# cuevhv/PMT_learning_for_semantic_segmentation_and_disparity

Measured on AMD Instinct MI355X. Metric: stereo-pairs/sec (train fwd+bwd) 512x256, higher is better.
Workload: dtype bf16; 1 GPU; minidsnetExt (densenet121, 1dcorr, aspp 0; the live PyTorch form of baseline_SDnet*) train step fwd+loss(CE+CE+Lovasz+L1)+bwd+Adam, 512x256 (WxH), batch 8 per GPU, hipGraph; global_batch=8, parallelism=dp1, world_size=1

## Files before the change

pmt_learning_for_semantic_segmentation_and_disparity_amd/_lib.py:

```python
import ctypes
import os
import re

import torch

_HERE = os.path.dirname(os.path.abspath(__file__))
LIB_PATH = os.path.join(_HERE, "libsdhip.so")
HEADER_PATH = os.path.join(_HERE, "..", "include", "sdhip.h")

NREP = int(os.environ.get("SDHIP_TUNE_NREP", "32"))


class SdhipError(RuntimeError):
    pass


_ARG_TYPES = {"*": ctypes.c_void_p, "int": ctypes.c_int, "long": ctypes.c_long, "int64_t": ctypes.c_long, "float": ctypes.c_float, "double": ctypes.c_double}
_RET_TYPES = {"int": ctypes.c_int, "long": ctypes.c_long, "void": None, "const char*": ctypes.c_char_p}


def parse_header(text):
    text = re.sub(r"/\*.*?\*/", " ", text, flags=re.S)
    consts = {n: int(v) for n, v in re.findall(r"^[ \t]*#define[ \t]+(SDHIP_\w+)[ \t]+\(?(-?\d+)\)?[ \t]*$", text, flags=re.M)}
    sigs = {}
    for ret, name, params in re.findall(r"^([\w \t*]+?)\s*\b(sdhip_\w+)\s*\(([^()]*)\)\s*;", text, flags=re.M):
        ret = re.sub(r"\s*\*\s*", "*", " ".join(ret.split()))
        if ret not in _RET_TYPES:
            raise SdhipError("sdhip.h: %s has return type '%s', which the binding cannot classify" % (name, ret))
        args = []
        for par in ([] if params.strip() == "void" else params.split(",")):
            ctype = "*" if "*" in par else " ".join(w for w in par.split()[:-1] if w != "const")
            if ctype not in _ARG_TYPES:
                raise SdhipError("sdhip.h: %s has parameter '%s', which the binding cannot classify" % (name, " ".join(par.split())))
            args.append(_ARG_TYPES[ctype])
        sigs[name] = (_RET_TYPES[ret], args)
    return sigs, consts


if not os.path.exists(LIB_PATH):
    raise ImportError(
        "libsdhip.so not found at %s — run `python -c 'import __graft_entry__ as g; g.build()'` "
        "(hipcc, gfx950). This package has no fallback path." % LIB_PATH)
if not os.path.exists(HEADER_PATH):
    raise ImportError(
        "sdhip.h not found at %s — the binding reads every signature and constant of libsdhip.so from it. "
        "This package has no fallback path." % HEADER_PATH)

_lib = ctypes.CDLL(LIB_PATH, mode=ctypes.RTLD_GLOBAL)

with open(HEADER_PATH) as _f:
    _SIGS, CONSTANTS = parse_header(_f.read())
SIGNATURES = {_name: _args for _name, (_ret, _args) in _SIGS.items()}
for _name, (_ret, _args) in _SIGS.items():
    _fn = getattr(_lib, _name)
    _fn.argtypes = _args
    _fn.restype = _ret

F32, BF16 = CONSTANTS["SDHIP_F32"], CONSTANTS["SDHIP_BF16"]
ERR_ARG, ERR_LAUNCH, ERR_UNSUPPORTED = CONSTANTS["SDHIP_ERR_ARG"], CONSTANTS["SDHIP_ERR_LAUNCH"], CONSTANTS["SDHIP_ERR_UNSUPPORTED"]
ACT_HSWISH, ACT_HSIGMOID = CONSTANTS["SDHIP_ACT_HSWISH"], CONSTANTS["SDHIP_ACT_HSIGMOID"]
SEG_TVERSKY, SEG_DICE, SEG_DICE_ENTROPY = CONSTANTS["SDHIP_SEG_TVERSKY"], CONSTANTS["SDHIP_SEG_DICE"], CONSTANTS["SDHIP_SEG_DICE_ENTROPY"]


class WgradItem(ctypes.Structure):
    _fields_ = [(n, ctypes.c_void_p) for n in ("x", "dy", "dw_packed", "dbias", "in_scale", "in_shift")] + \
               [(n, ctypes.c_int) for n in ("B", "H", "W", "Cin", "ldx", "Ho", "Wo", "Cout", "lddy", "kh", "kw", "stride", "dil", "pad_t",
                                            "pad_l", "D", "Do", "kd", "sd", "pad_d", "in_relu", "groups")]


class PyrMap(ctypes.Structure):
    _fields_ = [("p", ctypes.c_void_p)] + [(n, ctypes.c_int) for n in ("h", "w", "ld", "reserved")]


def pyr_maps(entries):
    t = (PyrMap * len(entries))()
    for e, (m, h, w, ld) in zip(t, entries):
        e.p, e.h, e.w, e.ld = m.data_ptr(), h, w, ld
    return ctypes.cast(t, ctypes.c_void_p), t


def lovasz_workspace_bytes(npix, C):
    return _lib.sdhip_lovasz_workspace_bytes(npix, C)


def seg_terms_workspace_bytes(B, hw, C):
    n = _lib.sdhip_seg_terms_workspace_bytes(B, hw, C)
    if n <= 0:
        raise SdhipError("sdhip_seg_terms_workspace_bytes: unsupported shape (B %d, %d pixels, C %d; C <= 32)" % (B, hw, C))
    return n


def disp_smooth_workspace_bytes(B, H, W):
    n = _lib.sdhip_disp_smooth_workspace_bytes(B, H, W)
    if n <= 0:
        raise SdhipError("sdhip_disp_smooth_workspace_bytes: unsupported shape (B %d, H %d, W %d)" % (B, H, W))
    return n


def edge_bce_workspace_bytes(n):
    nbytes = _lib.sdhip_edge_bce_workspace_bytes(n)
    if nbytes <= 0:
        raise SdhipError("sdhip_edge_bce_workspace_bytes: unsupported element count %d" % n)
    return nbytes


def photo_mse_workspace_bytes(npix):
    nbytes = _lib.sdhip_photo_mse_workspace_bytes(npix)
    if nbytes <= 0:
        raise SdhipError("sdhip_photo_mse_workspace_bytes: unsupported pixel count %d" % npix)
    return nbytes


def dw_pool_parts(H, W, C, k, stride, dt):
    n = _lib.sdhip_dw_pool_parts(H, W, C, k, stride, dt)
    if n <= 0:
        raise SdhipError("sdhip_dw_pool_parts: unsupported depthwise shape")
    return n


def dw_wgrad_parts(B, H, W, C, k, stride):
    n = _lib.sdhip_dw_wgrad_parts(B, H, W, C, k, stride)
    if n <= 0:
        raise SdhipError("sdhip_dw_wgrad_parts: unsupported depthwise shape")
    return n


def packed_elems(M, K, T, dt):
    return _lib.sdhip_conv_packed_elems(M, K, T, dt)


def graph_node_counts(graph):
    c = (ctypes.c_int * 4)()
    n = _lib.sdhip_graph_node_counts(ctypes.c_void_p(graph.raw_cuda_graph()), c)
    if n < 0:
        raise SdhipError("sdhip_graph_node_counts failed: %s" % _lib.sdhip_last_error().decode())
    return {"kernel": c[0], "memset": c[1], "memcpy": c[2], "other": c[3], "total": n}


def abort_capture(stream):
    rc = _lib.sdhip_abort_capture(ctypes.c_void_p(stream.cuda_stream))
    if rc < 0:
        raise SdhipError("sdhip_abort_capture failed: %s" % _lib.sdhip_last_error().decode())
    return rc


def reload_diag():
    _lib.sdhip_diag_reload()


def _diag_switch(name):
    v = os.environ.get(name)
    if v:
        import sys
        sys.stderr.write("[sdhip] diagnostic switch %s=%s is set: this is not the production path\n" % (name, v))
    return v


DIAG_NO_FUSED_BN = bool(_diag_switch("SDHIP_DIAG_NO_FUSED_BN"))
DIAG_NO_SIDE = bool(_diag_switch("SDHIP_DIAG_NO_SIDE"))
DIAG_NO_GRAD_SLOTS = bool(_diag_switch("SDHIP_DIAG_NO_GRAD_SLOTS"))
DIAG_NO_WGRAD_GROUP = bool(_diag_switch("SDHIP_DIAG_NO_WGRAD_GROUP"))
DIAG_NO_PHASE_DGRAD = bool(_diag_switch("SDHIP_DIAG_NO_PHASE_DGRAD"))
TUNE_WGRAD_OVERLAP = bool(_diag_switch("SDHIP_TUNE_WGRAD_OVERLAP"))
TUNE_OVERLAP_WG = int(_diag_switch("SDHIP_TUNE_OVERLAP_WG") or 128)
DIAG_NO_BN_SLOTS = bool(_diag_switch("SDHIP_DIAG_NO_BN_SLOTS"))
TUNE_FUSE1_MAX_PIX = int(_diag_switch("SDHIP_TUNE_FUSE1_MAX_PIX") or 32768)
TUNE_PRO_MAX_PIX = int(_diag_switch("SDHIP_TUNE_PRO_MAX_PIX") or 32768)
TUNE_BN_SLOT_MAX_MB = int(_diag_switch("SDHIP_TUNE_BN_SLOT_MAX_MB") or 40)
DIAG_NO_BNPRO = bool(_diag_switch("SDHIP_DIAG_NO_BNPRO"))
DIAG_NO_BNBWD_EPILOGUE = bool(_diag_switch("SDHIP_DIAG_NO_BNBWD_EPILOGUE"))
DIAG_STEM_S2D = _diag_switch("SDHIP_STEM_S2D")
DIAG_NO_PYRAMID_FUSE = bool(_diag_switch("SDHIP_DIAG_NO_PYRAMID_FUSE"))


def abi_version():
    return _lib.sdhip_abi_version()


def call(name, *args, unsupported_ok=False):
    if name not in SIGNATURES:
        raise SdhipError("%s is not declared in include/sdhip.h" % name)
    rc = getattr(_lib, name)(*args)
    if rc != 0 and not (unsupported_ok and rc == ERR_UNSUPPORTED):
        raise SdhipError("%s failed (%d): %s" % (name, rc, _lib.sdhip_last_error().decode()))
    return rc == 0


def try_call(name, *args):
    return call(name, *args, unsupported_ok=True)


def dtype_code(t):
    if t.dtype == torch.float32:
        return F32
    if t.dtype == torch.bfloat16:
        return BF16
    raise SdhipError("unsupported dtype %s (f32 and bf16 only)" % t.dtype)


def code_of(dtype):
    return BF16 if dtype == torch.bfloat16 else F32


def stream_ptr():
    return ctypes.c_void_p(torch.cuda.current_stream().cuda_stream)


def ptr(t):
    return ctypes.c_void_p(t.data_ptr()) if t is not None else ctypes.c_void_p(0)
```

pmt_learning_for_semantic_segmentation_and_disparity_amd/csrc/conv_band.h:

```cpp
#pragma once
#include <type_traits>
#include "conv_fast.h"

namespace {

struct BandArgs {
  const void* x; const void* wp; void* y;
  const float* bias; double* stats;
  int B, H, W, Ho, Wo, pad_t, pad_l;
  int Cin, ldx, Cout, Mpad, ldy;
  int bpg, act, stats_ld, nrep;
  const void* res; int ldres;
  long rep_stride;
  int tiles_w, tiles_hw, ntiles, tpw;
  unsigned magic_hw, magic_tw;
  int D, Do, pad_d;
  unsigned magic_do;
  int dbg;
};

template <int I, int N, typename F> __device__ __forceinline__ void band_static_for(F&& f) {
  if constexpr (I < N) { f(std::integral_constant<int, I>{}); band_static_for<I + 1, N>(f); }
}
template <int N> __device__ __forceinline__ void band_wait() { asm volatile("s_waitcnt vmcnt(%0) lgkmcnt(0)" ::"n"(N) : "memory"); }

template <int K, int BN, int NW = 8, int KD = 1>
struct BandCfg {
  static constexpr int RPR = NW * 16;
  static constexpr int RPW = 16 / NW;
  static constexpr int TH = 16, TW = 32;
  static constexpr int IH = TH + K - 1, IW = TW + K - 1, IWp = (IW + 7) & ~7;
  static constexpr int HROWS = IH * IWp;
  static constexpr int HR = (HROWS + RPR - 1) / RPR;
  static constexpr int HB = HROWS * 64;
  static constexpr int RS = K == 3 ? 3 : 1;
  static constexpr int NSTG = K / RS;
  static constexpr bool WRES = NSTG == 1 && KD == 1;
  static constexpr int TPS = RS * K;
  static constexpr int WROWS = TPS * BN;
  static constexpr int WR = (WROWS + RPR - 1) / RPR;
  static constexpr int WB = WROWS * 64;
  static constexpr int NWB = WRES ? 1 : 2;
  static constexpr int WRS = WRES ? 0 : WR;
  static constexpr int HPS = NSTG == 1 ? HR : (HR + NSTG - 2) / (NSTG - 1);
  static constexpr int RED = NW * 2 * BN * 4;
  static constexpr int SPT = (WRS + HPS + TPS - 1) / TPS;
  static constexpr size_t LDS = 2 * HB + NWB * WB + RED;
  static_assert(HROWS % 16 == 0 && WROWS % 16 == 0, "a wave's 16 rows of a DMA round are either all inside or all outside the image");
  static_assert(NSTG == 1 || HPS * (NSTG - 1) >= HR, "halo rounds must fit the stages of one chunk");
  static_assert(LDS <= 160 * 1024, "LDS budget");
};

typedef __attribute__((ext_vector_type(4))) int band_rsrc_t;
constexpr int kBandOob = 0x7fffff00;
#pragma clang diagnostic push
#pragma clang diagnostic ignored "-Winline-asm"
__device__ __forceinline__ void band_dma(int voff, band_rsrc_t rsrc, unsigned lds_wave_base, int soff) {
  asm volatile("s_mov_b32 m0, %2\n\ts_nop 0\n\tbuffer_load_dwordx4 %0, %1, %3 offen lds"
               : : "v"(voff), "s"(rsrc), "s"(lds_wave_base), "s"(soff) : "memory", "m0");
}
#pragma clang diagnostic pop
__device__ __forceinline__ band_rsrc_t band_rsrc(const void* base) {
  const unsigned long long a = (unsigned long long)base;
  band_rsrc_t r;
  r[0] = __builtin_amdgcn_readfirstlane((int)(a & 0xffffffffu));
  r[1] = __builtin_amdgcn_readfirstlane((int)((a >> 32) & 0xffffu));
  r[2] = kBandOob;
  r[3] = 0x00020000;
  return r;
}

template <int K, int BN, int VAR, int NW, int KD = 1>
__global__ __launch_bounds__(NW * 64) void conv_band_kernel(const BandArgs p) {
  constexpr bool DBG = (VAR & 128) != 0;
  const int dbg = DBG ? p.dbg : 0;
  using C = BandCfg<K, BN, NW, KD>;
  using T = bf16_t;
  constexpr int IWp = C::IWp, IW = C::IW, HB = C::HB, WB = C::WB, RPR = C::RPR, RPW = C::RPW;
  constexpr int NT_CO = BN / 16, NT_PIX = 2 * RPW;
  constexpr int NSTORE = NT_CO * NT_PIX / 2;
  extern __shared__ __attribute__((aligned(16))) unsigned char smem[];

  const int tid = threadIdx.x, lane = tid & 63;
  const int wave = __builtin_amdgcn_readfirstlane(tid >> 6);
  const int l15 = lane & 15, lg = lane >> 4;

  const int t_begin = blockIdx.x * p.tpw;
  const int t_end = min(p.ntiles, t_begin + p.tpw);
  if (t_begin >= t_end) return;
  const int nhalf = KD > 1 ? KD : (p.Cin > 32 ? 2 : 1);
  const int nchunks = (t_end - t_begin) * nhalf;

  const int rsub = tid >> 2;
  const int c_l = (tid & 3) ^ ((rsub >> 1) & 2);
  const unsigned wave_lds = __builtin_amdgcn_readfirstlane(lds_addr(smem) + wave * 1024);
  const band_rsrc_t xr = band_rsrc(p.x), wr = band_rsrc(p.wp);
  const int img_bytes = p.H * p.W * p.ldx * 2;

  int czt = 0;
  auto tile_of = [&](int t, int& b, int& oh0, int& ow0) {
    if constexpr (KD > 1) { const int q = fast_div(t, p.Do, p.magic_do); czt = t - q * p.Do; t = q; }
    b = fast_div(t, p.tiles_hw, p.magic_hw);
    const int r = t - b * p.tiles_hw;
    const int ty = fast_div(r, p.tiles_w, p.magic_tw);
    oh0 = ty * C::TH;
    ow0 = (r - ty * p.tiles_w) * C::TW;
  };
  int hv[C::HR];
  auto halo_offsets = [&](int oh0, int ow0) {
    const int ih0 = oh0 - p.pad_t, iw0 = ow0 - p.pad_l;
#pragma unroll
    for (int r = 0; r < C::HR; ++r) {
      const int row = r * RPR + rsub;
      const int ih = row / IWp, iw = row - ih * IWp;
      const int gh = ih0 + ih, gw = iw0 + iw;
      const bool in = iw < IW && (unsigned)gh < (unsigned)p.H && (unsigned)gw < (unsigned)p.W && c_l * 8 < p.Cin;
      hv[r] = in ? ((gh * p.W + gw) * p.ldx + c_l * 8) * 2 : kBandOob;
    }
  };
  auto halo_dma = [&](int r, int soff, int hsel) {
    if (r < C::HR && r * RPR + wave * 16 < C::HROWS) band_dma(soff >= 0 ? hv[r] : kBandOob, xr, hsel * HB + r * (RPR * 64) + wave_lds, soff >= 0 ? soff : 0);
  };
  auto chunk_src = [&](int b, int zt, int h) -> int {
    if constexpr (KD > 1) {
      const int zin = zt + h - p.pad_d;
      return (zin >= 0 && zin < p.D) ? (b * p.D + zin) * img_bytes : -1;
    } else {
      return b * img_bytes + h * 64;
    }
  };
  int wv[C::WR];
#pragma unroll
  for (int r = 0; r < C::WR; ++r) {
    const int row = r * RPR + rsub;
    const int tap = row / BN, m = min(row % BN, p.Mpad - 1);
    wv[r] = (tap * p.Mpad + m) * 128 + c_l * 16;
  }
  const int wrow_bytes = C::TPS * p.Mpad * 128;
  auto w_dma = [&](int r, int j, int h, int wsel) {
    if (r < C::WR && r * RPR + wave * 16 < C::WROWS)
      band_dma(wv[r], wr, 2 * HB + wsel * WB + r * (RPR * 64) + wave_lds, j * wrow_bytes + (KD > 1 ? h * wrow_bytes : h * 64));
  };

  int b_k[K];
#pragma unroll
  for (int kw = 0; kw < K; ++kw) b_k[kw] = LdsRow<1>::off(kw + l15, lg);
  const int a_base = LdsRow<1>::off(l15, lg);
  const int wave_row = wave * (RPW * IWp * 64);

  float bv[NT_CO][4];
#pragma unroll
  for (int mi = 0; mi < NT_CO; ++mi)
#pragma unroll
    for (int r = 0; r < 4; ++r) {
      const int co = mi * 16 + 4 * lg + r;
      bv[mi][r] = (p.bias && co < p.Cout) ? p.bias[co] : 0.f;
    }

  f32x4 acc[NT_CO][NT_PIX];
  float s1[NT_CO][4], s2[NT_CO][4];
#pragma unroll
  for (int mi = 0; mi < NT_CO; ++mi)
#pragma unroll
    for (int r = 0; r < 4; ++r) { s1[mi][r] = 0.f; s2[mi][r] = 0.f; }

  float* const red = reinterpret_cast<float*>(smem + 2 * HB + C::NWB * WB);
  auto flush_stats = [&](int grp) {
#pragma unroll
    for (int mi = 0; mi < NT_CO; ++mi) {
#pragma unroll
      for (int r = 0; r < 4; ++r) {
        const float a = row16_sum(s1[mi][r]), c2 = row16_sum(s2[mi][r]);
        if (l15 == 0) {
          const int m = mi * 16 + 4 * lg + r;
          red[(wave * 2 + 0) * BN + m] = a;
          red[(wave * 2 + 1) * BN + m] = c2;
        }
        s1[mi][r] = 0.f; s2[mi][r] = 0.f;
      }
    }
    asm volatile("s_waitcnt lgkmcnt(0)" ::: "memory");
    __builtin_amdgcn_s_barrier();
    if (tid < 2 * BN) {
      const int which = tid / BN, m = tid - which * BN;
      if (m < p.Cout) {
        float tot = 0.f;
#pragma unroll
        for (int w = 0; w < NW; ++w) tot += red[(w * 2 + which) * BN + m];
        atomicAdd(p.stats + (long)(blockIdx.x % p.nrep) * p.rep_stride + ((long)grp * 2 + which) * p.stats_ld + m, (double)tot);
      }
    }
  };

  if constexpr ((VAR & 2) != 0) { if (wave >= 4) __builtin_amdgcn_s_setprio(1); }
  int cb, coh0, cow0, ch_half = 0, ct = t_begin;
  tile_of(ct, cb, coh0, cow0);
  halo_offsets(coh0, cow0);
#pragma unroll
  for (int r = 0; r < C::WR; ++r) w_dma(r, 0, 0, 0);
#pragma unroll
  for (int r = 0; r < C::HR; ++r) halo_dma(r, chunk_src(cb, czt, 0), 0);
  int cz = czt;
  int wsel = 0;
  bool epi_counted = false;

  constexpr bool WREG = C::WRES && BN <= 32;
  u32x4 wreg[WREG ? C::TPS : 1][NT_CO];

  for (int c = 0; c < nchunks; ++c) {
    const int hsel = c & 1;
    const bool has_next = c + 1 < nchunks;
    int nb = cb, noh0 = coh0, now0 = cow0, nh = ch_half + 1, nt = ct, nz = cz;
    if (nh == nhalf) {
      nh = 0; nt = ct + 1;
      if (has_next) { tile_of(nt, nb, noh0, now0); halo_offsets(noh0, now0); nz = czt; }
    }
    const int nsoff = chunk_src(nb, nz, nh);
    if (ch_half == 0) {
#pragma unroll
      for (int mi = 0; mi < NT_CO; ++mi)
#pragma unroll
        for (int ni = 0; ni < NT_PIX; ++ni) acc[mi][ni] = f32x4{0.f, 0.f, 0.f, 0.f};
    }
    const unsigned char* const hb = smem + hsel * HB + wave_row;

    band_static_for<0, C::NSTG>([&](auto jc) {
      constexpr int j = decltype(jc)::value;
      constexpr int r_lo = (j - 1) * C::HPS, r_hi = j * C::HPS < C::HR ? j * C::HPS : C::HR;
      constexpr bool counted = j >= 1 && r_hi > r_lo && r_hi * RPR <= C::HROWS;
      if (j == 0 && epi_counted) band_wait<NSTORE>();
      else if (counted && has_next) band_wait<counted ? r_hi - r_lo : 0>();
      else band_wait<0>();
      if (!(dbg & 16)) __builtin_amdgcn_s_barrier();

      const unsigned char* const wl = smem + 2 * HB + wsel * WB + a_base;
      const unsigned char* const hj = hb + j * C::RS * (IWp * 64);
      if constexpr (WREG) {
        if (c == 0) {
#pragma unroll
          for (int t = 0; t < C::TPS; ++t)
#pragma unroll
            for (int mi = 0; mi < NT_CO; ++mi) wreg[t][mi] = *reinterpret_cast<const u32x4*>(wl + t * (BN * 64) + mi * 1024);
        }
      }
      u32x4 af[2][NT_CO], bf[2][NT_PIX];
      if constexpr (DBG) if (dbg & 32) {
#pragma unroll
        for (int i = 0; i < 2; ++i)
#pragma unroll
          for (int q = 0; q < 4; ++q) { if (q < NT_CO) af[i][q] = u32x4{0x3f803f80u, (unsigned)tid, 0x3f803f80u, 0x3f803f80u}; bf[i][q] = u32x4{0x3f803f80u, 0x3f803f80u, (unsigned)lane, 0x3f803f80u}; }
      }
      auto load = [&](int set, int t) {
        if (dbg & 32) return;
#pragma unroll
        for (int mi = 0; mi < NT_CO; ++mi) {
          if constexpr (WREG) af[set][mi] = wreg[t][mi];
          else af[set][mi] = *reinterpret_cast<const u32x4*>(wl + t * (BN * 64) + mi * 1024);
        }
#pragma unroll
        for (int ni = 0; ni < NT_PIX; ++ni)
          bf[set][ni] = *reinterpret_cast<const u32x4*>(hj + b_k[t % K] + ((t / K + (ni >> 1)) * IWp + (ni & 1) * 16) * 64);
      };
      auto dma_slot = [&](int sl) {
        if (sl < C::WRS) {
          if (dbg & 2) return;
          if (j + 1 < C::NSTG) w_dma(sl, j + 1, ch_half, wsel ^ 1);
          else if (has_next) w_dma(sl, 0, nh, wsel ^ 1);
        } else if (sl < C::WRS + C::HPS) {
          if (dbg & 1) return;
          if (has_next && (C::NSTG == 1 || j < C::NSTG - 1)) halo_dma(j * C::HPS + sl - C::WRS, nsoff, hsel ^ 1);
        }
      };
      load(0, 0);
#pragma unroll
      for (int kw = 0; kw < C::TPS; ++kw) {
        if constexpr ((VAR & 1) != 0) {
#pragma unroll
          for (int sl = kw * C::SPT; sl < (kw + 1) * C::SPT; ++sl) dma_slot(sl);
        }
        if (kw + 1 < C::TPS) load((kw + 1) & 1, kw + 1);
        if constexpr ((VAR & 1) == 0) {
#pragma unroll
          for (int sl = kw * C::SPT; sl < (kw + 1) * C::SPT; ++sl) dma_slot(sl);
        }
        if (!(dbg & 4)) {
#pragma unroll
          for (int mi = 0; mi < NT_CO; ++mi)
#pragma unroll
            for (int ni = 0; ni < NT_PIX; ++ni) Mma<T>::run(acc[mi][ni], af[kw & 1][mi], bf[kw & 1][ni]);
        }
        if constexpr ((VAR & 4) != 0) {
#pragma unroll
          for (int g = 0; g < NT_CO + NT_PIX; ++g) {
            __builtin_amdgcn_sched_group_barrier(0x100, 1, 0);
            __builtin_amdgcn_sched_group_barrier(0x008, (NT_CO * NT_PIX) / (NT_CO + NT_PIX), 0);
          }
        }
      }
      if constexpr (!C::WRES) wsel ^= 1;
    });

    epi_counted = false;
    if (ch_half == nhalf - 1) {
      const int oimg = KD > 1 ? cb * p.Do + cz : cb;
      const int grp = oimg < p.bpg ? 0 : oimg / p.bpg;
      if (p.bias) {
#pragma unroll
        for (int mi = 0; mi < NT_CO; ++mi)
#pragma unroll
          for (int ni = 0; ni < NT_PIX; ++ni)
#pragma unroll
            for (int r = 0; r < 4; ++r) acc[mi][ni][r] += bv[mi][r];
      }
      if (p.act == 1) {
#pragma unroll
        for (int mi = 0; mi < NT_CO; ++mi)
#pragma unroll
          for (int ni = 0; ni < NT_PIX; ++ni)
#pragma unroll
            for (int r = 0; r < 4; ++r) acc[mi][ni][r] = fmaxf(acc[mi][ni][r], 0.f);
      } else if (p.act == 2) {
#pragma unroll
        for (int mi = 0; mi < NT_CO; ++mi)
#pragma unroll
          for (int ni = 0; ni < NT_PIX; ++ni)
#pragma unroll
            for (int r = 0; r < 4; ++r) acc[mi][ni][r] = 1.f / (1.f + __expf(-acc[mi][ni][r]));
      }
      T* const yb = (T*)p.y + (long)oimg * p.Ho * p.Wo * p.ldy;
      const T* const rb = (const T*)p.res + (long)oimg * p.Ho * p.Wo * p.ldres;
      const bool interior = coh0 + C::TH <= p.Ho && cow0 + C::TW <= p.Wo && BN <= p.Cout;
      if (interior) {
        const long pix0 = (long)(coh0 + RPW * wave) * p.Wo + cow0 + (lg & 1) * 16 + l15;
        T* const d0 = yb + pix0 * p.ldy + 8 * (lg >> 1);
        const T* const r0 = rb + pix0 * p.ldres + 8 * (lg >> 1);
#pragma unroll
        for (int q = 0; q < NT_PIX / 2; ++q) {
          T* dst = d0 + (long)q * p.Wo * p.ldy;
          const T* rsrc = r0 + (long)q * p.Wo * p.ldres;
          u32x4 ov[NT_CO];
#pragma unroll
          for (int mi = 0; mi < NT_CO; ++mi) {
            const f32x4 v0 = acc[mi][2 * q], v1 = acc[mi][2 * q + 1];
            const u32x2 o0 = u32x2{pack2bf(v0[0], v0[1]), pack2bf(v0[2], v0[3])};
            const u32x2 o1 = u32x2{pack2bf(v1[0], v1[1]), pack2bf(v1[2], v1[3])};
            if (p.stats) {
              const f32x4 w0 = f32x4{bflo(o0[0]), bfhi(o0[0]), bflo(o0[1]), bfhi(o0[1])};
              const f32x4 w1 = f32x4{bflo(o1[0]), bfhi(o1[0]), bflo(o1[1]), bfhi(o1[1])};
#pragma unroll
              for (int r = 0; r < 4; ++r) {
                s1[mi][r] += w0[r] + w1[r];
                s2[mi][r] = fmaf(w1[r], w1[r], fmaf(w0[r], w0[r], s2[mi][r]));
              }
            }
            u32x4 o;
            if (p.res) {
              float f[8];
#pragma unroll
              for (int r = 0; r < 4; ++r) {
                const float a0 = v0[r], a1 = v1[r];
                const u32x2 e = __builtin_amdgcn_permlane16_swap(__float_as_uint(a0), __float_as_uint(a1), false, false);
                const unsigned e0 = e[0], e1 = e[1];
                f[r] = __uint_as_float(e0); f[4 + r] = __uint_as_float(e1);
              }
              const u32x4 old = *reinterpret_cast<const u32x4*>(rsrc + mi * 16);
#pragma unroll
              for (int e = 0; e < 4; ++e) o[e] = pack2bf(f[2 * e] + bflo(old[e]), f[2 * e + 1] + bfhi(old[e]));
            } else {
              const u32x2 e0 = __builtin_amdgcn_permlane16_swap(o0[0], o1[0], false, false);
              const u32x2 e1 = __builtin_amdgcn_permlane16_swap(o0[1], o1[1], false, false);
              o = u32x4{e0[0], e1[0], e0[1], e1[1]};
            }
            ov[mi] = o;
          }
          if (!(dbg & 8)) {
#pragma unroll
            for (int mi = 0; mi < NT_CO; ++mi) *reinterpret_cast<u32x4*>(dst + mi * 16) = ov[mi];
          }
        }
        epi_counted = !(dbg & 8) && !p.res;
      } else {
#pragma unroll
        for (int ni = 0; ni < NT_PIX; ++ni) {
          const int oh = coh0 + RPW * wave + (ni >> 1), ow = cow0 + (ni & 1) * 16 + l15;
          const bool valid = oh < p.Ho && ow < p.Wo;
          T* dst = yb + ((long)oh * p.Wo + ow) * p.ldy;
          const T* rsrc = rb + ((long)oh * p.Wo + ow) * p.ldres;
#pragma unroll
          for (int mi = 0; mi < NT_CO; ++mi) {
            const int co = mi * 16 + 4 * lg;
            float v[4];
#pragma unroll
            for (int r = 0; r < 4; ++r) v[r] = acc[mi][ni][r];
            if (valid && co + 3 < p.Cout) {
              if (p.res) {
                const u32x2 old = *reinterpret_cast<const u32x2*>(rsrc + co);
                v[0] += bflo(old[0]); v[1] += bfhi(old[0]); v[2] += bflo(old[1]); v[3] += bfhi(old[1]);
              }
              const u32x2 o = u32x2{pack2bf(v[0], v[1]), pack2bf(v[2], v[3])};
              *reinterpret_cast<u32x2*>(dst + co) = o;
              v[0] = bflo(o[0]); v[1] = bfhi(o[0]); v[2] = bflo(o[1]); v[3] = bfhi(o[1]);
            } else if (valid && co < p.Cout) {
#pragma unroll
              for (int r = 0; r < 4; ++r) {
                if (co + r < p.Cout) {
                  if (p.res) v[r] += Elem<T>::ld(rsrc + co + r);
                  Elem<T>::st(dst + co + r, v[r]); v[r] = Elem<T>::rnd(v[r]);
                }
                else v[r] = 0.f;
              }
            } else {
#pragma unroll
              for (int r = 0; r < 4; ++r) v[r] = 0.f;
            }
            if (p.stats) {
#pragma unroll
              for (int r = 0; r < 4; ++r) { s1[mi][r] += v[r]; s2[mi][r] = fmaf(v[r], v[r], s2[mi][r]); }
            }
          }
        }
      }
      if (p.stats) {
        const int nimg = KD > 1 ? nb * p.Do + nz : nb;
        const int ngrp = nimg < p.bpg ? 0 : nimg / p.bpg;
        if (!has_next || ngrp != grp) { flush_stats(grp); epi_counted = false; }
      }
    }
    cb = nb; coh0 = noh0; cow0 = now0; ch_half = nh; ct = nt; cz = nz;
  }
}

inline bool band_ok(int ntiles) { return ntiles >= 192 && ntiles < 65536; }

template <int K, int BN, int VAR, int NW = 8, int KD = 1>
int launch_band_bn(const BandArgs& a, int grid, hipStream_t s) {
  auto kern = conv_band_kernel<K, BN, VAR, NW, KD>;
  static bool attr_set = false;
  if (!attr_set) {
    if (hipFuncSetAttribute((const void*)kern, hipFuncAttributeMaxDynamicSharedMemorySize, 160 * 1024) != hipSuccess)
      SDHIP_FAIL(SDHIP_ERR_LAUNCH, "conv_band: cannot raise dynamic LDS limit");
    attr_set = true;
  }
  const size_t lds = BandCfg<K, BN, NW, KD>::LDS;
  hipLaunchKernelGGL(kern, dim3(grid), dim3(NW * 64), lds, s, a);
  SDHIP_LAUNCH_CHECK();
  return SDHIP_OK;
}

template <int K, int KD = 1>
int launch_band(BandArgs& a, hipStream_t s) {
  const int tiles_h = sdhip_cdiv(a.Ho, 16);
  a.tiles_w = sdhip_cdiv(a.Wo, 32);
  a.tiles_hw = tiles_h * a.tiles_w;
  a.ntiles = a.tiles_hw * a.B * (KD > 1 ? a.Do : 1);
  a.magic_do = (KD > 1 && a.Do > 1) ? (unsigned)(0x100000000ULL / (unsigned)a.Do) + 1u : 0u;
  a.magic_hw = a.tiles_hw > 1 ? (unsigned)(0x100000000ULL / (unsigned)a.tiles_hw) + 1u : 0u;
  a.magic_tw = a.tiles_w > 1 ? (unsigned)(0x100000000ULL / (unsigned)a.tiles_w) + 1u : 0u;
  a.tpw = sdhip_cdiv(a.ntiles, 256);
  a.dbg = sdhip_diag().tune_band_dbg;
  const int grid = sdhip_cdiv(a.ntiles, a.tpw);
  a.dbg &= 0xff;
  if constexpr (K == 5) {
    if (a.Mpad > 32) return a.dbg ? launch_band_bn<K, 64, 128 + 5>(a, grid, s) : launch_band_bn<K, 64, 5>(a, grid, s);
  } else if constexpr (KD > 1) {
    return launch_band_bn<K, 32, 5, 8, KD>(a, grid, s);
  } else {
    if (a.Mpad > 32) return launch_band_bn<K, 64, 5>(a, grid, s);
  }
  return launch_band_bn<K, 32, 5>(a, grid, s);
}

}
```

pmt_learning_for_semantic_segmentation_and_disparity_amd/csrc/conv_fwd.hip:

```cpp
#include "conv_common.h"
#include "conv_fast.h"
#include "conv_point.h"
#include "conv_grow.h"
#include "conv_mid.h"
#include "conv_band.h"
#include "conv_gemm.h"
#include "conv_thin.h"

namespace {

struct FwdArgs {
  const void* x; const void* wp; void* y;
  const float* bias; const float* in_scale; const float* in_shift; double* stats;
  ConvGeom g;
  int Cin, ldx, Cout, Mpad, ldy;
  int in_relu, groups, act, accumulate;
  int tg, vec_in, vec_out, stats_ld, nrep, pf_halo, sh, per_tap;
  long rep_stride;
};

template <typename T, int TH, int TW, int BN>
__global__ __launch_bounds__(256) void conv_fwd_kernel(const FwdArgs p) {
  constexpr int V = Chunk<T>::N;
  constexpr int CK = 8 * V;
// ... 209 lines not shown
      w_issue(q, t);
      w_commit(q, t, wl0);
      __syncthreads();
      compute(q, t, halo0, wl0);
    }
  } else {
  if (pf_halo) halo_issue(0); else halo_sync_stage(0, halo0);
  w_issue(0, 0);
  for (int st = 0; st < S; ++st) {
    const int q = st / ntg, t0 = (st - q * ntg) * p.tg;
    unsigned char* halo = halo0 + ((pf_halo && (q & 1)) ? halo_bytes : 0);
    unsigned char* wl = wl0 + (st & 1) * wbuf_bytes;
    if (pf_halo && t0 == 0) halo_commit(q, halo);
    w_commit(q, t0, wl);
    __syncthreads();
    const int sn = st + 1;
    int qn = 0, t0n = 0;
    if (sn < S) {
      qn = sn / ntg; t0n = (sn - qn * ntg) * p.tg;
      if (pf_halo && t0n == 0) halo_issue(qn);
      w_issue(qn, t0n);
    }
    compute(q, t0, halo, wl);
    if (!pf_halo && sn < S && t0n == 0) {
      __syncthreads();
      halo_sync_stage(qn, halo0);
    }
  }
  }

  float s1[NT_CO][4], s2[NT_CO][4];
#pragma unroll
  for (int mi = 0; mi < NT_CO; ++mi)
#pragma unroll
    for (int r = 0; r < 4; ++r) { s1[mi][r] = 0.f; s2[mi][r] = 0.f; }

  T* yb = (T*)p.y + (long)blockIdx.z * g.Ho * g.Wo * p.ldy;
#pragma unroll
  for (int ni = 0; ni < NT_PIX; ++ni) {
    const int pt = wave * NT_PIX + ni;
    const int oh = oh0 + pt / TWT, ow = ow0 + (pt % TWT) * 16 + l15;
    const bool valid = oh < g.Ho && ow < g.Wo;
    T* dst = yb + ((long)oh * g.Wo + ow) * p.ldy;
#pragma unroll
    for (int mi = 0; mi < NT_CO; ++mi) {
      if (mi * 16 >= mvalid) continue;
      const int co = n0 + mi * 16 + 4 * lg;
      float v[4];
#pragma unroll
      for (int r = 0; r < 4; ++r) {
        float x = acc[mi][ni][r];
        if (p.bias && co + r < p.Cout) x += p.bias[co + r];
        if (p.act == 1) x = fmaxf(x, 0.f);
        else if (p.act == 2) x = 1.f / (1.f + __expf(-x));
        v[r] = x;
      }
      if (!valid) continue;
      if (p.vec_out && co + 3 < p.Cout) {
        if constexpr (sizeof(T) == 4) {
          f32x4* d4 = reinterpret_cast<f32x4*>(dst + co);
          f32x4 o = f32x4{v[0], v[1], v[2], v[3]};
          if (p.accumulate) o += *d4;
          *d4 = o;
#pragma unroll
          for (int r = 0; r < 4; ++r) v[r] = o[r];
        } else {
          u32x2* d2 = reinterpret_cast<u32x2*>(dst + co);
          if (p.accumulate) {
            const u32x2 old = *d2;
            v[0] += bflo(old[0]); v[1] += bfhi(old[0]); v[2] += bflo(old[1]); v[3] += bfhi(old[1]);
          }
          const u32x2 o = u32x2{pack2bf(v[0], v[1]), pack2bf(v[2], v[3])};
          *d2 = o;
          v[0] = bflo(o[0]); v[1] = bfhi(o[0]); v[2] = bflo(o[1]); v[3] = bfhi(o[1]);
        }
      } else {
#pragma unroll
        for (int r = 0; r < 4; ++r) {
          if (co + r < p.Cout) {
            if (p.accumulate) v[r] += Elem<T>::ld(dst + co + r);
            Elem<T>::st(dst + co + r, v[r]);
            v[r] = Elem<T>::rnd(v[r]);
          } else {
            v[r] = 0.f;
          }
        }
      }
#pragma unroll
      for (int r = 0; r < 4; ++r) { s1[mi][r] += v[r]; s2[mi][r] = fmaf(v[r], v[r], s2[mi][r]); }
    }
  }

  if (p.stats) {
    __syncthreads();
    float* red = reinterpret_cast<float*>(smem);
#pragma unroll
    for (int mi = 0; mi < NT_CO; ++mi) {
#pragma unroll
      for (int r = 0; r < 4; ++r) {
        float a = s1[mi][r], c2 = s2[mi][r];
#pragma unroll
        for (int o = 8; o > 0; o >>= 1) { a += __shfl_xor(a, o, 64); c2 += __shfl_xor(c2, o, 64); }
        if (l15 == 0) {
          const int m = mi * 16 + 4 * lg + r;
          red[(wave * 2 + 0) * BN + m] = a;
          red[(wave * 2 + 1) * BN + m] = c2;
        }
      }
    }
    __syncthreads();
    if (tid < 2 * BN) {
      const int which = tid / BN, m = tid - which * BN;
      if (n0 + m < p.Cout) {
        const float tot = red[(0 * 2 + which) * BN + m] + red[(1 * 2 + which) * BN + m] +
                          red[(2 * 2 + which) * BN + m] + red[(3 * 2 + which) * BN + m];
        atomicAdd(p.stats + (long)((blockIdx.x + blockIdx.z) % p.nrep) * p.rep_stride + ((long)grp * 2 + which) * p.stats_ld + n0 + m, (double)tot);
      }
    }
  }
}

template <typename T, int TH, int TW, int BN>
int launch(const FwdArgs& a, size_t lds, hipStream_t s) {
  auto kern = conv_fwd_kernel<T, TH, TW, BN>;
  static size_t attr_set = 0;
  if (lds > 64 * 1024 && lds > attr_set) {
    if (hipFuncSetAttribute((const void*)kern, hipFuncAttributeMaxDynamicSharedMemorySize, 160 * 1024) != hipSuccess)
      SDHIP_FAIL(SDHIP_ERR_LAUNCH, "conv_fwd: cannot raise dynamic LDS limit");
    attr_set = 160 * 1024;
  }
  const ConvGeom& g = a.g;
  dim3 grid(sdhip_cdiv(g.Ho, TH) * sdhip_cdiv(g.Wo, TW), sdhip_cdiv(a.Mpad, BN), g.B * g.Do);
  hipLaunchKernelGGL(kern, grid, dim3(256), lds, s, a);
  SDHIP_LAUNCH_CHECK();
  return SDHIP_OK;
}

template <typename T, int TH, int TW>
int launch_bn(const FwdArgs& a, int bn, size_t lds, hipStream_t s) {
  switch (bn) {
    case 16: return launch<T, TH, TW, 16>(a, lds, s);
    case 32: return launch<T, TH, TW, 32>(a, lds, s);
    case 64: return launch<T, TH, TW, 64>(a, lds, s);
    default: return launch<T, TH, TW, 128>(a, lds, s);
  }
}

size_t halo_bytes_of(const ConvGeom& g, int th, int tw, int per_tap) {
  const int eh = per_tap ? 0 : (g.kh - 1) * g.dil, ew = per_tap ? 0 : (g.kw - 1) * g.dil;
  const int IH = (th - 1) * g.stride + eh + 1, IW = (tw - 1) * g.stride + ew + 1;
  return ((size_t)IH * IW * 128 + 15) & ~(size_t)15;
}


struct ProStats {
  const double* stats; int ld, nrep;
  const float* gamma; const float* beta;
  float* scale; float* shift; float* mean; float* invstd; float* rmean; float* rvar;
  float eps, momentum; double count;
  const double* pend; double* fold; int pend_ld, pend_nrep, pend_c0, pend_n;
};

struct ConvCall {
  const void* x = nullptr; const void* wp = nullptr; void* y = nullptr;
  const float* bias = nullptr; const float* in_scale = nullptr; const float* in_shift = nullptr;
  double* stats = nullptr; int stats_ld = 0, stats_nrep = 1;
  ConvGeom g{};
  int Cin = 0, ldx = 0, Cout = 0, ldy = 0;
  int in_relu = 0, groups = 1, act = 0, accumulate = 0;
  int dtype = SDHIP_F32;
  hipStream_t stream = nullptr;
  int omul = 1, ooz = 0, ooy = 0, oox = 0;
  const void* bx = nullptr; int ldbx = 0;
  const float* bsc = nullptr; const float* bsh = nullptr; int bx_mode = 0;
  const void* addend = nullptr; int ldadd = 0;
  const ProStats* ps = nullptr;
  bool plain() const { return !ps && !bx && !addend && omul == 1; }
  bool flat() const { return g.kd == 1 && g.D == 1 && g.Do == 1; }
};

ConvGeom geom2d(int B, int H, int W, int Ho, int Wo, int kh, int kw, int stride, int dil, int pad_t, int pad_l) {
  return ConvGeom{B, H, W, Ho, Wo, kh, kw, stride, dil, pad_t, pad_l, 1, 1, 1, 1, 0};
}

ConvCall conv_call(const void* x, const void* wpacked, void* y, const ConvGeom& g, int Cin, int ldx, int Cout, int ldy, int dtype, void* stream) {
  ConvCall c;
  c.x = x; c.wp = wpacked; c.y = y; c.g = g;
  c.Cin = Cin; c.ldx = ldx; c.Cout = Cout; c.ldy = ldy;
  c.dtype = dtype; c.stream = (hipStream_t)stream;
  return c;
}

struct ConvPlan {
  int V, es, Mpad;
  int stats_ld, nrep; long rep_stride;
  int vec_in, vec_out;
  int T, bn; bool big;
  int rows, chunks_per_row, per_tap_any;
};

constexpr size_t kLdsMax = 160 * 1024, kLdsSoft = 80 * 1024;

ConvPlan conv_plan(const ConvCall& c) {
  const ConvGeom& g = c.g;
  const SdhipDiag& dg = sdhip_diag();
  ConvPlan d;
  d.V = c.dtype == SDHIP_BF16 ? 8 : 4;
  d.es = conv_esize(c.dtype);
  d.Mpad = (c.Cout + 15) & ~15;
  d.stats_ld = c.stats_ld > 0 ? c.stats_ld : c.Cout;
  d.nrep = c.stats_nrep > 0 ? c.stats_nrep : 1;
  d.rep_stride = (long)c.groups * 2 * d.stats_ld;
  d.vec_in = (c.ldx % d.V == 0) && (((uintptr_t)c.x & 15) == 0);
  d.vec_out = (c.ldy % 4 == 0) && (((uintptr_t)c.y % (4 * d.es)) == 0);
  int bn = 16;
  for (int cand = 128; cand >= 32; cand >>= 1)
    if ((long)sdhip_cdiv(d.Mpad, cand) * cand * 4 <= (long)d.Mpad * 5) { bn = cand; break; }
  if ((long)g.kh * g.kw * g.kd * c.Cin <= 128 && d.Mpad <= 128) bn = d.Mpad > 64 ? 128 : (d.Mpad > 32 ? 64 : (d.Mpad > 16 ? 32 : 16));
  d.T = g.kh * g.kw;
  const long blocks_big = (long)sdhip_cdiv(g.Ho, 8) * sdhip_cdiv(g.Wo, 32) * g.B * g.Do * sdhip_cdiv(d.Mpad, bn);
  d.big = (blocks_big >= dg.tune_big && g.Wo >= 24) || dg.conv_big;
  if (g.stride == 2 && g.kd > 1 && !dg.conv_big && dg.tune_s2_small) d.big = false;
  if (!d.big) {
    const long px_blocks = (long)sdhip_cdiv(g.Ho, 4) * sdhip_cdiv(g.Wo, 16) * g.B * g.Do;
    while (bn > 32 && px_blocks * sdhip_cdiv(d.Mpad, bn) < dg.tune_split) bn >>= 1;
  }
  d.bn = bn;
  d.rows = d.Mpad < bn ? d.Mpad : bn;
  d.chunks_per_row = c.Cin <= 8 * d.V / 2 ? 4 : 8;
  d.per_tap_any = (g.kh > 1 || g.kw > 1) && g.dil >= 4 && g.kd == 1;
  return d;
}


int path_thin(const ConvCall& c, const ConvPlan& d) {
  const ConvGeom& g = c.g;
  if (!(c.plain() && c.Cout == 1 && c.Cin <= d.V && d.vec_in && g.stride == 1 && c.flat() && !c.in_scale && !c.accumulate &&
        d.T <= kThinMaxT && g.Ho == g.H + 2 * g.pad_t - g.dil * (g.kh - 1) && g.Wo == g.W + 2 * g.pad_l - g.dil * (g.kw - 1) &&
        g.pad_t >= 0 && g.pad_l >= 0 && !sdhip_diag().conv_no_thin))
    return kNotTaken;
  ThinArgs t{};
  t.x = c.x; t.wp = c.wp; t.y = c.y; t.bias = c.bias; t.stats = c.stats;
  set_extent(t, g);
  t.kh = g.kh; t.kw = g.kw; t.dil = g.dil;
  t.Cin = c.Cin; t.ldx = c.ldx; t.ldy = c.ldy; t.Mpad = d.Mpad; t.act = c.act; t.bpg = g.B / c.groups;
  t.stats_ld = d.stats_ld; t.nrep = d.nrep; t.rep_stride = d.rep_stride;
  dim3 grid(sdhip_cdiv(g.Wo, 256), g.Ho, g.B);
  if (c.dtype == SDHIP_BF16) hipLaunchKernelGGL(conv_thin_fwd_kernel<bf16_t>, grid, dim3(256), 0, c.stream, t);
  else hipLaunchKernelGGL(conv_thin_fwd_kernel<float>, grid, dim3(256), 0, c.stream, t);
  SDHIP_LAUNCH_CHECK_AS("conv2d_fwd_impl");
  return SDHIP_OK;
}

int path_fanin(const ConvCall& c, const ConvPlan& d) {
  const ConvGeom& g = c.g;
  if (!(c.plain() && c.dtype == SDHIP_BF16 && fanin_ok(c.Cin, c.Cout, g.kh, g.kw, g.stride, g.dil, g.kd, g.sd, c.ldx, c.x) && !c.in_scale &&
        !c.accumulate && !c.stats && (long)g.H * g.W * c.ldx < (1L << 31) && !sdhip_diag().conv_no_thin))
    return kNotTaken;
  FaninArgs t{};
  t.x = c.x; t.wp = c.wp; t.y = c.y; t.bias = c.bias;
  set_extent(t, g);
  t.kh = g.kh; t.kw = g.kw;
  t.D = g.D; t.Do = g.Do; t.pad_d = g.pad_d;
  t.Cin = c.Cin; t.ldx = c.ldx; t.ldy = c.ldy; t.Mpad = d.Mpad; t.act = c.act;
  t.dpw = 1; t.zsegs = g.Do; t.npxp = 0; t.pitch = 0;
  return launch_fanin(t, g.kd, c.stream);
}

int path_fanout(const ConvCall& c, const ConvPlan& d) {
  const ConvGeom& g = c.g;
  if (!(c.plain() && c.dtype == SDHIP_BF16 && fanout_ok(c.Cin, c.Cout, d.T, g.stride, g.kd, g.sd, c.ldy, c.y) && !c.in_scale &&
        !c.accumulate && !c.stats && !c.bias && c.act == 0 && (g.kh - 1) * g.dil <= 31 && (g.kw - 1) * g.dil <= 31 &&
        (long)sdhip_cdiv(g.Ho, 8) * sdhip_cdiv(g.Wo, 32) < (1L << 31) && g.B <= 65535 && !sdhip_diag().conv_no_thin))
    return kNotTaken;
  FanArgs t{};
  t.x = c.x; t.wp = c.wp; t.y = c.y;
  set_extent(t, g);
  t.kh = g.kh; t.kw = g.kw; t.dil = g.dil;
  t.ldx = c.ldx; t.Cout = c.Cout; t.Mpad = d.Mpad; t.ldy = c.ldy;
  t.D = g.D; t.Do = g.Do; t.kd = g.kd; t.pad_d = g.pad_d; t.dpw = 1; t.zsegs = g.Do;
  return launch_fanout(t, c.stream);
}

int path_gemm(const ConvCall& c, const ConvPlan& d) {
  const ConvGeom& g = c.g;
  const SdhipDiag& dg = sdhip_diag();
  if (!(c.plain() && c.dtype == SDHIP_BF16 && g.kh == 1 && g.kw == 1 && c.flat() && g.stride == 1 && g.pad_t == 0 && g.pad_l == 0 &&
        g.Ho == g.H && g.Wo == g.W && !c.accumulate && !dg.conv_generic && !dg.conv_no_gemm))
    return kNotTaken;
  GemmArgs a{};
  a.seg[0] = GemmSeg{c.x, c.ldx, c.Cin, 0};
  a.seg[1] = GemmSeg{nullptr, 0, 0, 0};
  a.nseg = 1;
  a.wp = c.wp; a.y = c.y; a.bias = c.bias; a.in_scale = c.in_scale; a.in_shift = c.in_shift; a.stats = c.stats;
  a.ldy = c.ldy; a.Cout = c.Cout; a.Mpad = d.Mpad; a.K = c.Cin; a.in_relu = c.in_relu; a.act = c.act;
  a.M = (long)g.B * g.H * g.W; a.H = g.H; a.W = g.W; a.ppg = a.M / c.groups;
  a.stats_ld = d.stats_ld; a.nrep = d.nrep; a.rep_stride = d.rep_stride;
  if (!gemm1x1_ok(a, (c.in_scale || c.stats) ? c.groups : 1)) return kNotTaken;
  return launch_gemm_any(a, c.stream);
}

bool band_common_ok(const ConvCall& c) {
  const ConvGeom& g = c.g;
  return !c.ps && !c.bx && c.omul == 1 && c.dtype == SDHIP_BF16 && g.stride == 1 && g.dil == 1 && !c.in_scale &&
         !((c.accumulate || c.addend) && c.stats) && !(c.accumulate && c.addend) &&
         (!c.addend || (c.ldadd % 8 == 0 && ((uintptr_t)c.addend & 15) == 0)) && c.Cin % 8 == 0 &&
         c.ldx % 8 == 0 && ((uintptr_t)c.x & 15) == 0 && c.ldy % 8 == 0 && ((uintptr_t)c.y & 15) == 0 &&
         (long)g.B * g.D * g.H * g.W * c.ldx * 2 < (long)kBandOob && band_ok(sdhip_cdiv(g.Ho, 16) * sdhip_cdiv(g.Wo, 32) * g.B * g.Do) &&
         !sdhip_diag().conv_generic && !sdhip_diag().conv_no_band;
}

BandArgs band_args(const ConvCall& c, const ConvPlan& d) {
  const ConvGeom& g = c.g;
  BandArgs f{};
  f.x = c.x; f.wp = c.wp; f.y = c.y; f.bias = c.bias; f.stats = c.stats;
  set_extent(f, g);
  f.D = g.D; f.Do = g.Do; f.pad_d = g.pad_d;
  f.Cin = c.Cin; f.ldx = c.ldx; f.Cout = c.Cout; f.Mpad = d.Mpad; f.ldy = c.ldy;
  f.bpg = (g.B / c.groups) * g.Do; f.act = c.act; f.stats_ld = d.stats_ld; f.nrep = d.nrep; f.rep_stride = d.rep_stride;
  f.res = c.addend ? c.addend : (c.accumulate ? c.y : nullptr); f.ldres = c.addend ? c.ldadd : c.ldy;
  return f;
}

int path_band2d(const ConvCall& c, const ConvPlan& d) {
  const ConvGeom& g = c.g;
  const bool band5 = g.kh == 5 && g.kw == 5 && (c.Cin <= 32 || c.Cin == 64);
  const bool band3 = g.kh == 3 && g.kw == 3 && c.Cin <= 32 && !sdhip_diag().conv_no_band3;
  if (!((band5 || band3) && c.flat() && d.Mpad <= 64 && d.Mpad >= 32 && band_common_ok(c))) return kNotTaken;
  BandArgs f = band_args(c, d);
  f.pad_d = 0;
  return band5 ? launch_band<5>(f, c.stream) : launch_band<3>(f, c.stream);
}

int path_band3d(const ConvCall& c, const ConvPlan& d) {
  const ConvGeom& g = c.g;
  if (!(g.kh == 3 && g.kw == 3 && g.kd == 3 && g.sd == 1 && c.Cin <= 32 && d.Mpad == 32 && band_common_ok(c) && !sdhip_diag().conv_no_band3))
    return kNotTaken;
  BandArgs f = band_args(c, d);
  return launch_band<3, 3>(f, c.stream);
}

int path_point(const ConvCall& c, const ConvPlan& d) {
  const ConvGeom& g = c.g;
  const SdhipDiag& dg = sdhip_diag();
  if (!(c.dtype == SDHIP_BF16 && !c.bx && !c.addend && c.omul == 1 && (c.ps || (c.in_scale && c.stats)) && !c.bias && c.act == 0 && !c.accumulate &&
        g.kh == 1 && g.kw == 1 && c.flat() && g.stride == 1 && g.pad_t == 0 && g.pad_l == 0 && g.Ho == g.H && g.Wo == g.W &&
        c.Cin >= 128 && c.Cin <= kPinMaxC && c.Cin % 8 == 0 && c.Cout % kPointBN == 0 && c.Cout <= 256 && (long)g.B * g.H * g.W <= 32768 && (long)g.H * g.W <= kPointMaxMap &&
        (long)g.B * sdhip_cdiv((long)g.H * g.W, kPointPix) * (c.Cout / kPointBN) <= kPointMaxWG &&
        d.vec_in && d.vec_out && (long)g.H * g.W * c.ldx < (1L << 31) && !dg.conv_generic && !dg.conv_no_point))
    return kNotTaken;
  const ProStats* ps = c.ps;
  PointArgs f{};
  f.x = c.x; f.wp = c.wp; f.y = c.y; f.in_scale = c.in_scale; f.in_shift = c.in_shift; f.stats = c.stats;
  f.HW = g.H * g.W; f.Cin = c.Cin; f.ldx = c.ldx; f.Cout = c.Cout; f.Mpad = d.Mpad; f.ldy = c.ldy;
  f.in_relu = c.in_relu; f.bpg = g.B / c.groups;
  f.stats_ld = d.stats_ld; f.nrep = d.nrep; f.rep_stride = d.rep_stride;
  if (ps) {
    f.pin_stats = ps->stats; f.pin_ld = ps->ld; f.pin_nrep = ps->nrep; f.pin_groups = c.groups; f.pin_gamma = ps->gamma; f.pin_beta = ps->beta;
    f.pin_scale = ps->scale; f.pin_shift = ps->shift; f.pin_mean = ps->mean; f.pin_invstd = ps->invstd; f.pin_rmean = ps->rmean; f.pin_rvar = ps->rvar;
    f.pin_eps = ps->eps; f.pin_momentum = ps->momentum; f.pin_count = ps->count;
    f.pend_stats = ps->pend; f.pin_fold = ps->fold; f.pend_ld = ps->pend_ld; f.pend_nrep = ps->pend_nrep; f.pend_c0 = ps->pend_c0; f.pend_n = ps->pend ? ps->pend_n : 0;
  }
  return launch_point(f, g.B, c.stream);
}

int path_grow(const ConvCall& c, const ConvPlan& d) {
  const ConvGeom& g = c.g;
  const SdhipDiag& dg = sdhip_diag();
  if (!(c.dtype == SDHIP_BF16 && !c.bx && !c.addend && c.omul == 1 && (c.ps || (c.in_scale && c.stats)) && !c.bias && c.act == 0 && !c.accumulate &&
        g.kh == 3 && g.kw == 3 && c.flat() && g.stride == 1 && g.dil == 1 && g.pad_t == 1 && g.pad_l == 1 && g.Ho == g.H && g.Wo == g.W &&
        c.Cin % 32 == 0 && c.Cin >= 64 && c.Cin <= 256 && c.Cout == kGrowBN && (long)g.H * g.W <= kGrowMaxMap &&
        (long)g.B * sdhip_cdiv(g.H, kGrowTH) * sdhip_cdiv(g.W, kGrowTW) <= kGrowMaxWG &&
        d.vec_in && d.vec_out && (long)g.H * g.W * c.ldx < (1L << 31) && !dg.conv_generic && !dg.conv_no_grow))
    return kNotTaken;
  const ProStats* ps = c.ps;
  GrowArgs f{};
  f.x = c.x; f.wp = c.wp; f.y = c.y; f.in_scale = c.in_scale; f.in_shift = c.in_shift; f.stats = c.stats;
  f.H = g.H; f.W = g.W; f.Cin = c.Cin; f.ldx = c.ldx; f.ldy = c.ldy; f.tiles_w = sdhip_cdiv(g.W, kGrowTW);
  f.in_relu = c.in_relu; f.bpg = g.B / c.groups;
  f.stats_ld = d.stats_ld; f.nrep = d.nrep; f.rep_stride = d.rep_stride;
  if (ps) {
    f.pin_stats = ps->stats; f.pin_ld = ps->ld; f.pin_nrep = ps->nrep; f.pin_groups = c.groups; f.pin_gamma = ps->gamma; f.pin_beta = ps->beta;
    f.pin_scale = ps->scale; f.pin_shift = ps->shift; f.pin_mean = ps->mean; f.pin_invstd = ps->invstd; f.pin_rmean = ps->rmean; f.pin_rvar = ps->rvar;
    f.pin_eps = ps->eps; f.pin_momentum = ps->momentum; f.pin_count = ps->count;
    f.pend_stats = ps->pend; f.pin_fold = ps->fold; f.pend_ld = ps->pend_ld; f.pend_nrep = ps->pend_nrep; f.pend_c0 = ps->pend_c0; f.pend_n = ps->pend ? ps->pend_n : 0;
  }
  return launch_grow(f, g.B, c.stream);
}

int path_mid(const ConvCall& c, const ConvPlan& d) {
  const ConvGeom& g = c.g;
  const SdhipDiag& dg = sdhip_diag();
  const long min_map = dg.tune_mid_min_map > 0 ? dg.tune_mid_min_map : kMidMinMap, max_map = dg.tune_mid_max_map > 0 ? dg.tune_mid_max_map : kMidMaxMap;
  const long max_wg = dg.tune_mid_max_wg > 0 ? dg.tune_mid_max_wg : kMidMaxWG;
  if (!(c.dtype == SDHIP_BF16 && g.kh == 3 && g.kw == 3 && c.flat() && g.stride == 1 && g.dil == 1 && g.pad_t == 1 && g.pad_l == 1 &&
        g.Ho == g.H && g.Wo == g.W && c.Cin == kMidBN && c.Cout == kMidBN && !c.in_scale && !c.ps && !c.bias && c.act == 0 && !c.accumulate &&
        c.omul == 1 && (c.bx ? c.bx_mode == 0 : !c.addend) && (long)g.H * g.W >= min_map && (long)g.H * g.W <= max_map &&
        (long)g.B * sdhip_cdiv(g.H, kMidTH) * sdhip_cdiv(g.W, kMidTW) <= max_wg &&
        d.vec_in && d.vec_out && (long)g.H * g.W * c.ldx < (1L << 31) && !dg.conv_generic && !dg.conv_no_mid))
    return kNotTaken;
  MidArgs f{};
  f.x = c.x; f.wp = c.wp; f.y = c.y; f.stats = c.stats;
  f.H = g.H; f.W = g.W; f.ldx = c.ldx; f.ldy = c.ldy; f.tiles_w = sdhip_cdiv(g.W, kMidTW);
  f.bpg = g.B / c.groups;
  f.stats_ld = d.stats_ld; f.nrep = d.nrep; f.rep_stride = d.rep_stride;
  f.bx = c.bx; f.bsc = c.bsc; f.bsh = c.bsh; f.ldbx = c.ldbx;
  f.res = c.bx ? c.addend : nullptr; f.ldres = c.ldadd;
  return launch_mid(f, g.B, c.stream);
}

int path_fast(const ConvCall& c, const ConvPlan& d) {
  const ConvGeom& g = c.g;
  if (!(!d.per_tap_any && d.vec_in && d.vec_out && (long)g.H * g.W * c.ldx < (1L << 31) && !sdhip_diag().conv_generic)) return kNotTaken;
  const int tune_ksoft_small = 80, tune_ksoft_big = 80;
  const int CKh = 8 * d.V, T = d.T, bn = d.bn;
  const int ks = d.chunks_per_row == 4 ? 1 : 2;
  const int rb = 64 * ks, px_per_round = 256 / (4 * ks);
  const ProStats* ps = c.ps;
  FastArgs f{};
  f.x = c.x; f.wp = c.wp; f.y = c.y; f.bias = c.bias; f.in_scale = c.in_scale; f.in_shift = c.in_shift; f.stats = c.stats;
  set_extent(f, g);
  f.kh = g.kh; f.kw = g.kw; f.stride = g.stride; f.dil = g.dil;
  f.D = g.D; f.Do = g.Do; f.kd = g.kd; f.sd = g.sd; f.pad_d = g.pad_d;
  f.Cin = c.Cin; f.ldx = c.ldx; f.Cout = c.Cout; f.Mpad = d.Mpad; f.ldy = c.ldy;
  f.in_relu = c.in_relu; f.bpg = g.B / c.groups; f.act = c.act; f.accumulate = c.accumulate;
  f.stats_ld = d.stats_ld; f.nrep = d.nrep; f.rep_stride = d.rep_stride; f.tail = (c.Cin % d.V) != 0;
  f.omul = c.omul; f.ooz = c.ooz; f.ooy = c.ooy; f.oox = c.oox;
  f.bx = c.bx; f.ldbx = c.ldbx; f.bsc = c.bsc; f.bsh = c.bsh;
  f.res = c.bx ? c.addend : nullptr; f.ldres = c.ldadd; f.bx_mode = c.bx_mode; f.bx_groups = c.groups;
  f.dma = !c.in_scale && !f.tail && !ps;
  if (ps) {
    f.pin_stats = ps->stats; f.pin_ld = ps->ld; f.pin_nrep = ps->nrep; f.pin_groups = c.groups; f.pin_gamma = ps->gamma; f.pin_beta = ps->beta;
    f.pin_scale = ps->scale; f.pin_shift = ps->shift; f.pin_mean = ps->mean; f.pin_invstd = ps->invstd; f.pin_rmean = ps->rmean; f.pin_rvar = ps->rvar;
    f.pin_eps = ps->eps; f.pin_momentum = ps->momentum; f.pin_count = ps->count;
    f.pend_stats = ps->pend; f.pin_fold = ps->fold; f.pend_ld = ps->pend_ld; f.pend_nrep = ps->pend_nrep; f.pend_c0 = ps->pend_c0; f.pend_n = ps->pend ? ps->pend_n : 0;
  }
  bool fbig = d.big;
  for (int attempt = 0; attempt < 2; ++attempt) {
    const int th = fbig ? 8 : 4, tw = fbig ? 32 : 16;
    const int IH = (th - 1) * g.stride + (g.kh - 1) * g.dil + 1, IW = (tw - 1) * g.stride + (g.kw - 1) * g.dil + 1;
    const int IWp = (IW + 7) & ~7;
    const int hrows = ((IH * IWp + px_per_round - 1) / px_per_round) * px_per_round;
    const int nqq_f = g.kd * (ks == 2 ? sdhip_cdiv(c.Cin, CKh) : 1);
    const size_t hb = (size_t)hrows * rb * ((fbig || nqq_f == 1) ? 1 : 2);
    if (!fbig && hrows > ((f.dma && ks == 1) ? 6 : 5) * px_per_round) { fbig = true; continue; }
    auto wbuf = [&](int tgv) { return (size_t)(((tgv * bn + px_per_round - 1) / px_per_round) * px_per_round) * rb; };
    int tg = T;
    const size_t ksoft_f = (size_t)(fbig ? tune_ksoft_big : tune_ksoft_small) * 1024;
    size_t lds;
    if (nqq_f == 1 && hb + wbuf(T) <= ksoft_f) {
      lds = hb + wbuf(T);
    } else {
      while (tg > 1 && hb + 2 * wbuf(tg) > ksoft_f) --tg;
      lds = hb + 2 * wbuf(tg);
    }
    if (lds < 4096) lds = 4096;
    f.pin_off = 0; f.pin_cs = 0;
    if (ps) { f.pin_off = (int)lds; f.pin_cs = (c.Cin + 63) & ~63; lds += 2 * (size_t)f.pin_cs * sizeof(float); }
    if (lds > kLdsMax) { if (!fbig) break; fbig = false; continue; }
    f.tg = tg;
    f.magic_iwp = IWp > 1 ? (unsigned)(0x100000000ULL / (unsigned)IWp) + 1u : 0u;
    f.tiles_w = sdhip_cdiv(g.Wo, tw);
    f.magic_tw = f.tiles_w > 1 ? (unsigned)(0x100000000ULL / (unsigned)f.tiles_w) + 1u : 0u;
    f.ntg = sdhip_cdiv(T, tg);
    if ((long)f.tiles_w * sdhip_cdiv(g.Ho, th) >= 65536) break;
    return c.dtype == SDHIP_BF16 ? launch_fast_any<bf16_t>(f, fbig, ks, bn, lds, c.stream) : launch_fast_any<float>(f, fbig, ks, bn, lds, c.stream);
  }
  return kNotTaken;
}

int path_generic(const ConvCall& c, const ConvPlan& d) {
  const ConvGeom& g = c.g;
  const int bn = d.bn;
  FwdArgs a{};
  a.x = c.x; a.wp = c.wp; a.y = c.y; a.bias = c.bias; a.in_scale = c.in_scale; a.in_shift = c.in_shift; a.stats = c.stats;
  a.g = g;
  a.Cin = c.Cin; a.ldx = c.ldx; a.Cout = c.Cout; a.Mpad = d.Mpad; a.ldy = c.ldy;
  a.in_relu = c.in_relu; a.groups = c.groups; a.act = c.act; a.accumulate = c.accumulate;
  a.vec_in = d.vec_in; a.vec_out = d.vec_out;
  a.stats_ld = d.stats_ld; a.nrep = d.nrep; a.rep_stride = d.rep_stride;
  bool big = d.big;
  for (int attempt = 0; attempt < 2; ++attempt) {
    const int th = big ? 8 : 4, tw = big ? 32 : 16;
    const int per_tap = d.per_tap_any;
    const size_t halo = halo_bytes_of(g, th, tw, per_tap);
    const long halo_loads = (long)(halo / 128) * d.chunks_per_row;
    const int pf = !per_tap && !big && d.vec_in && (c.Cin % d.V == 0) && halo_loads <= 4 * 256 && 2 * halo + 2 * (size_t)bn * 128 <= kLdsSoft;
    int tg = per_tap ? 1 : 1024 / (d.rows * d.chunks_per_row);
    if (tg < 1) tg = 1;
    if (tg > d.T) tg = d.T;
    const size_t hb = halo * (pf ? 2 : 1);
    while (tg > 1 && hb + 2 * (size_t)tg * bn * 128 > kLdsSoft) --tg;
    size_t lds = hb + 2 * (size_t)tg * bn * 128;
    if (lds < 4096) lds = 4096;
    if (lds > kLdsMax) {
      if (big) { big = false; continue; }
      SDHIP_FAIL(SDHIP_ERR_UNSUPPORTED, "conv2d_fwd: halo tile of a %dx%d kernel with dilation %d does not fit LDS", g.kh, g.kw, g.dil);
    }
    a.tg = tg; a.pf_halo = pf; a.sh = d.chunks_per_row == 4 ? 2 : 3; a.per_tap = per_tap;
    if (c.dtype == SDHIP_BF16)
      return big ? launch_bn<bf16_t, 8, 32>(a, bn, lds, c.stream) : launch_bn<bf16_t, 4, 16>(a, bn, lds, c.stream);
    return big ? launch_bn<float, 8, 32>(a, bn, lds, c.stream) : launch_bn<float, 4, 16>(a, bn, lds, c.stream);
  }
  SDHIP_FAIL(SDHIP_ERR_UNSUPPORTED, "conv2d_fwd: no tile configuration fits");
}

int conv2d_fwd_impl(const ConvCall& c) {
  const ConvGeom& g = c.g;
  SDHIP_CHECK_ARG(c.x && c.wp && c.y, "conv2d_fwd: null pointer");
  SDHIP_CHECK_ARG(c.dtype == SDHIP_F32 || c.dtype == SDHIP_BF16, "conv2d_fwd: unknown dtype %d", c.dtype);
  SDHIP_CHECK_ARG(g.B > 0 && g.H > 0 && g.W > 0 && c.Cin > 0 && c.Cout > 0 && g.Ho > 0 && g.Wo > 0, "conv2d_fwd: empty tensor");
  SDHIP_CHECK_ARG(c.ldx >= c.Cin && c.ldy >= c.Cout, "conv2d_fwd: pixel stride smaller than channel count");
  SDHIP_CHECK_ARG(g.kh >= 1 && g.kw >= 1 && g.stride >= 1 && g.dil >= 1, "conv2d_fwd: bad kernel geometry");
  SDHIP_CHECK_ARG(c.groups >= 1 && g.B % c.groups == 0, "conv2d_fwd: batch %d not divisible by %d stat groups", g.B, c.groups);
  SDHIP_CHECK_ARG((c.in_scale == nullptr) == (c.in_shift == nullptr), "conv2d_fwd: in_scale/in_shift must come together");
  SDHIP_CHECK_ARG(((uintptr_t)c.wp & 15) == 0, "conv2d_fwd: packed weights must be 16-byte aligned");
  SDHIP_CHECK_ARG(g.D >= 1 && g.Do >= 1 && g.kd >= 1 && g.sd >= 1 && (long)g.B * g.Do <= 65535, "conv2d_fwd: bad depth geometry");
  const ConvPlan d = conv_plan(c);
  int rc;
  for (auto path : {path_thin, path_fanin, path_fanout, path_gemm, path_band2d, path_band3d})
    if ((rc = path(c, d)) != kNotTaken) return rc;
  if (c.addend && !c.bx) SDHIP_FAIL(SDHIP_ERR_UNSUPPORTED, "conv2d_fwd_add: only the persistent 5x5 kernel adds a second tensor in its epilogue (bf16, <= 64 channels, >= 192 tiles of 16x32)");
  if ((rc = path_point(c, d)) != kNotTaken) return rc;
  if ((rc = path_grow(c, d)) != kNotTaken) return rc;
  if ((rc = path_mid(c, d)) != kNotTaken) return rc;
  if ((rc = path_fast(c, d)) != kNotTaken) return rc;
  if (c.omul != 1) SDHIP_FAIL(SDHIP_ERR_UNSUPPORTED, "conv2d_fwd_phase: interleaved output needs the aligned fast path (ldx %% 8, ldy %% 4)");
  if (c.ps) SDHIP_FAIL(SDHIP_ERR_UNSUPPORTED, "conv2d_fwd_bnpro: needs the aligned fast path (ldx %% 8, ldy %% 4, halo tile within LDS)");
  if (c.bx) SDHIP_FAIL(SDHIP_ERR_UNSUPPORTED, "conv2d_fwd_bnbwd: needs the aligned fast path (ldx %% 8, ldy %% 4, halo tile within LDS)");
  return path_generic(c, d);
}

}

extern "C" int sdhip_conv1x1_cat_fwd(const void* x0, int ld0, int c0, int us0, const void* x1, int ld1, int c1, int us1,
                                     const void* wpacked, void* y, int ldy, const float* bias,
                                     int B, int H, int W, int Cout, int act, int dtype, void* stream) {
  SDHIP_CHECK_ARG(x0 && wpacked && y && c0 > 0 && B > 0 && H > 0 && W > 0 && Cout > 0, "conv1x1_cat_fwd: bad arguments");
  SDHIP_CHECK_ARG(dtype == SDHIP_BF16, "conv1x1_cat_fwd: bf16 only");
  SDHIP_CHECK_ARG((x1 == nullptr) == (c1 == 0) && us0 >= 0 && us1 >= 0 && us0 < 8 && us1 < 8, "conv1x1_cat_fwd: bad second segment");
  GemmArgs g{};
  g.seg[0] = GemmSeg{x0, ld0, c0, us0};
  g.seg[1] = GemmSeg{x1, ld1, c1, us1};
  g.nseg = x1 ? 2 : 1;
  g.wp = wpacked; g.y = y; g.bias = bias;
  g.ldy = ldy; g.Cout = Cout; g.Mpad = (Cout + 15) & ~15; g.K = c0 + c1; g.act = act;
  g.M = (long)B * H * W; g.H = H; g.W = W; g.ppg = g.M;
  g.stats_ld = Cout; g.nrep = 1; g.rep_stride = 0;
  if (!gemm1x1_ok(g, 1, true)) SDHIP_FAIL(SDHIP_ERR_UNSUPPORTED, "conv1x1_cat_fwd: operands not 16-byte aligned / grid not divisible by the upsampling factor");
  return launch_gemm_any(g, (hipStream_t)stream);
}

extern "C" int sdhip_conv2d_fwd(const void* x, const void* wpacked, void* y,
                                const float* bias, const float* in_scale, const float* in_shift,
                                double* stats, int stats_ld, int stats_nrep,
                                int B, int H, int W, int Cin, int ldx,
                                int Ho, int Wo, int Cout, int ldy,
                                int kh, int kw, int stride, int dil, int pad_t, int pad_l,
                                int D, int Do, int kd, int sd, int pad_d,
                                int in_relu, int groups, int act, int accumulate,
                                int dtype, void* stream) {
  ConvCall c = conv_call(x, wpacked, y, ConvGeom{B, H, W, Ho, Wo, kh, kw, stride, dil, pad_t, pad_l, D, Do, kd, sd, pad_d},
                         Cin, ldx, Cout, ldy, dtype, stream);
  c.bias = bias; c.in_scale = in_scale; c.in_shift = in_shift;
  c.stats = stats; c.stats_ld = stats_ld; c.stats_nrep = stats_nrep;
  c.in_relu = in_relu; c.groups = groups; c.act = act; c.accumulate = accumulate;
  return conv2d_fwd_impl(c);
}

extern "C" int sdhip_conv2d_fwd_bnpro(const void* x, const void* wpacked, void* y, double* out_stats, int out_stats_ld, int out_stats_nrep,
                                      double* in_stats, int in_stats_ld, int in_stats_nrep,
                                      const double* pend_stats, int pend_ld, int pend_nrep, int pend_c0, int pend_n,
                                      const float* gamma, const float* beta,
                                      float* running_mean, float* running_var, float* scale_out, float* shift_out, float* mean_out,
                                      float* invstd_out, double count, float eps, float momentum,
                                      int B, int H, int W, int Cin, int ldx, int Ho, int Wo, int Cout, int ldy,
                                      int kh, int kw, int pad_t, int pad_l, int groups, int dtype, void* stream) {
  SDHIP_CHECK_ARG(in_stats && scale_out && shift_out && mean_out && invstd_out && count >= 1. && in_stats_nrep >= 1 && in_stats_ld >= Cin,
                  "conv2d_fwd_bnpro: statistics / output vectors missing");
  SDHIP_CHECK_ARG((running_mean == nullptr) == (running_var == nullptr), "conv2d_fwd_bnpro: running_mean / running_var come together");
  if (Cin > kPinMaxC || in_stats_nrep > 4 || (pend_stats && pend_nrep > 4))
    SDHIP_FAIL(SDHIP_ERR_UNSUPPORTED, "conv2d_fwd_bnpro: at most %d input channels and 4 statistics replicas", kPinMaxC);
  SDHIP_CHECK_ARG(!pend_stats || (pend_n > 0 && pend_c0 >= 0 && pend_c0 + pend_n <= Cin && pend_ld >= pend_n && pend_nrep >= 1 && in_stats_nrep == 1),
                  "conv2d_fwd_bnpro: bad pending-statistics slice (folding needs single-replica slab statistics)");
  ProStats ps{in_stats, in_stats_ld, in_stats_nrep, gamma, beta, scale_out, shift_out, mean_out, invstd_out, running_mean, running_var,
              eps, momentum, count, pend_stats, in_stats, pend_ld, pend_nrep, pend_c0, pend_n};
  ConvCall c = conv_call(x, wpacked, y, geom2d(B, H, W, Ho, Wo, kh, kw, 1, 1, pad_t, pad_l), Cin, ldx, Cout, ldy, dtype, stream);
  c.stats = out_stats; c.stats_ld = out_stats_ld; c.stats_nrep = out_stats_nrep;
  c.in_relu = 1; c.groups = groups;
  c.ps = &ps;
  return conv2d_fwd_impl(c);
}

extern "C" int sdhip_conv2d_fwd_add(const void* x, const void* wpacked, void* y, const void* addend, int ldadd,
                                    int B, int H, int W, int Cin, int ldx, int Ho, int Wo, int Cout, int ldy,
                                    int kh, int kw, int pad_t, int pad_l, int dtype, void* stream) {
  SDHIP_CHECK_ARG(addend && ldadd >= Cout, "conv2d_fwd_add: addend missing / pixel stride smaller than Cout");
  ConvCall c = conv_call(x, wpacked, y, geom2d(B, H, W, Ho, Wo, kh, kw, 1, 1, pad_t, pad_l), Cin, ldx, Cout, ldy, dtype, stream);
  c.addend = addend; c.ldadd = ldadd;
  return conv2d_fwd_impl(c);
}

extern "C" int sdhip_conv2d_fwd_bnbwd(const void* x, const void* wpacked, void* y, double* sums, int sums_ld, int sums_nrep,
                                      const void* u, int ldu, const float* scale, const float* shift, const void* addend, int ldadd,
                                      int B, int H, int W, int Cin, int ldx, int Ho, int Wo, int Cout, int ldy,
                                      int kh, int kw, int dil, int pad_t, int pad_l, int groups, int mode, int dtype, void* stream) {
  SDHIP_CHECK_ARG(mode == 0 || (mode == 1 && addend), "conv2d_fwd_bnbwd: mode 1 (apply) needs the tensor the result is added to");
  SDHIP_CHECK_ARG(dtype == SDHIP_BF16, "conv2d_fwd_bnbwd: bf16 only");
  SDHIP_CHECK_ARG(sums && u && scale && shift && ldu >= Cout && Cout % 4 == 0 && ldu % 4 == 0 && ((uintptr_t)u & 7) == 0 &&
                  ((uintptr_t)scale & 15) == 0 && ((uintptr_t)shift & 15) == 0,
                  "conv2d_fwd_bnbwd: sums / u / scale / shift missing or misaligned (Cout %% 4, ldu %% 4)");
  SDHIP_CHECK_ARG(!addend || (ldadd >= Cout && ldadd % 4 == 0 && ((uintptr_t)addend & 7) == 0), "conv2d_fwd_bnbwd: addend misaligned");
  ConvCall c = conv_call(x, wpacked, y, geom2d(B, H, W, Ho, Wo, kh, kw, 1, dil, pad_t, pad_l), Cin, ldx, Cout, ldy, dtype, stream);
  c.stats = sums; c.stats_ld = sums_ld; c.stats_nrep = sums_nrep;
  c.groups = groups;
  c.bx = u; c.ldbx = ldu; c.bsc = scale; c.bsh = shift; c.bx_mode = mode;
  c.addend = addend; c.ldadd = ldadd;
  return conv2d_fwd_impl(c);
}

extern "C" int sdhip_conv2d_fwd_phase(const void* x, const void* wpacked, void* y, double* stats, int stats_ld, int stats_nrep,
                                      int B, int H, int W, int Cin, int ldx, int Cout, int ldy, int kh, int kw,
                                      int D, int kd, int groups, int off_d, int off_h, int off_w, int dtype, void* stream) {
  SDHIP_CHECK_ARG(off_d >= 0 && off_d < 2 && off_h >= 0 && off_h < 2 && off_w >= 0 && off_w < 2, "conv2d_fwd_phase: phase offsets are 0 or 1");
  ConvCall c = conv_call(x, wpacked, y, ConvGeom{B, H, W, H, W, kh, kw, 1, 1, 0, 0, D, D, kd, 1, 0}, Cin, ldx, Cout, ldy, dtype, stream);
  c.stats = stats; c.stats_ld = stats_ld; c.stats_nrep = stats_nrep;
  c.groups = groups;
  c.omul = 2; c.ooz = off_d; c.ooy = off_h; c.oox = off_w;
  return conv2d_fwd_impl(c);
}
```

pmt_learning_for_semantic_segmentation_and_disparity_amd/csrc/runtime.hip:

```cpp
#include "sdhip_common.h"
#include <vector>

#define SDHIP_ABI_VERSION 2

static thread_local char g_err[512] = "";

void sdhip_set_error(const char* fmt, ...) {
  va_list ap;
  va_start(ap, fmt);
  vsnprintf(g_err, sizeof(g_err), fmt, ap);
  va_end(ap);
}

extern "C" int sdhip_abi_version(void) { return SDHIP_ABI_VERSION; }
extern "C" const char* sdhip_last_error(void) { return g_err; }

static SdhipDiag g_diag;
static bool g_diag_init = false;

static int env_int(const char* name, int dflt) { const char* v = getenv(name); return v ? atoi(v) : dflt; }
static bool env_set(const char* name) {
  const char* v = getenv(name);
  if (v && *v) { fprintf(stderr, "[libsdhip] diagnostic switch %s=%s is set: kernels / launch heuristics differ from production\n", name, v); return true; }
  return false;
}
static void diag_fill() {
  g_diag.conv_generic = env_set("SDHIP_CONV_GENERIC");
  g_diag.conv_big = env_set("SDHIP_CONV_BIG");
  g_diag.conv_no_thin = env_set("SDHIP_CONV_NO_THIN");
  g_diag.conv_no_gemm = env_set("SDHIP_CONV_NO_GEMM");
  g_diag.conv_no_band = env_set("SDHIP_CONV_NO_BAND");
  g_diag.conv_no_band3 = env_set("SDHIP_CONV_NO_BAND3");
  g_diag.conv_no_point = env_set("SDHIP_CONV_NO_POINT");
  g_diag.conv_no_grow = env_set("SDHIP_CONV_NO_GROW");
  g_diag.conv_no_mid = env_set("SDHIP_CONV_NO_MID");
  g_diag.wgrad_generic = env_set("SDHIP_WGRAD_GENERIC");
  g_diag.wgrad_no_pack = env_set("SDHIP_WGRAD_NO_PACK");
  g_diag.wgrad_force_pack = env_set("SDHIP_WGRAD_FORCE_PACK");
  g_diag.wgrad_no_gemm = env_set("SDHIP_WGRAD_NO_GEMM");
  g_diag.wgrad_no_half = env_set("SDHIP_WGRAD_NO_HALF");
  g_diag.thin_wgrad_reg = env_set("SDHIP_THIN_WGRAD_REG");
  g_diag.corr_no_tiled = env_set("SDHIP_CORR_NO_TILED");
  g_diag.wgrad_no_half32 = env_set("SDHIP_WGRAD_NO_HALF32");
  g_diag.wgrad_split2d = env_set("SDHIP_WGRAD_SPLIT2D");
  g_diag.tune_s2_small = env_int("SDHIP_TUNE_S2_SMALL", 1);
  g_diag.tune_big = env_int("SDHIP_TUNE_BIG", 512);
  g_diag.tune_split = env_int("SDHIP_TUNE_SPLIT", 1024);
  g_diag.tune_thin_blocks = env_int("SDHIP_TUNE_THIN_BLOCKS", 1024);
  g_diag.tune_fused_blocks = env_int("SDHIP_TUNE_FUSED_BLOCKS", 768);
  g_diag.tune_gemm_dbg = env_int("SDHIP_TUNE_GEMM_DBG", 0);
  g_diag.tune_band_dbg = env_int("SDHIP_TUNE_BAND_DBG", 0);
  g_diag.tune_mid_min_map = env_int("SDHIP_TUNE_MID_MIN_MAP", 0);
  g_diag.tune_mid_max_map = env_int("SDHIP_TUNE_MID_MAX_MAP", 0);
  g_diag.tune_mid_max_wg = env_int("SDHIP_TUNE_MID_MAX_WG", 0);
  g_diag.tune_atomic_tbs = getenv("SDHIP_TUNE_ATOMIC_TBS") ? atof(getenv("SDHIP_TUNE_ATOMIC_TBS")) : 1.3;
  g_diag.tune_wg1_tile = getenv("SDHIP_TUNE_WG1_TILE") ? atof(getenv("SDHIP_TUNE_WG1_TILE")) : 1.0;
  g_diag_init = true;
}
const SdhipDiag& sdhip_diag() {
  if (!g_diag_init) diag_fill();
  return g_diag;
}
__attribute__((constructor)) static void diag_at_load() { diag_fill(); }
extern "C" void sdhip_diag_reload(void) { diag_fill(); }

extern "C" int sdhip_abort_capture(void* stream) {
  hipStream_t s = (hipStream_t)stream;
  hipStreamCaptureStatus st = hipStreamCaptureStatusNone;
  hipError_t e = hipStreamIsCapturing(s, &st);
  (void)hipGetLastError();
  int was_open = 0;
  if (e != hipSuccess || st != hipStreamCaptureStatusNone) {
    hipGraph_t g = nullptr;
    (void)hipStreamEndCapture(s, &g);
    (void)hipGetLastError();
    if (g) (void)hipGraphDestroy(g);
    was_open = 1;
  }
  st = hipStreamCaptureStatusNone;
  e = hipStreamIsCapturing(s, &st);
  (void)hipGetLastError();
  if (e == hipSuccess && st == hipStreamCaptureStatusActive) SDHIP_FAIL(SDHIP_ERR_LAUNCH, "abort_capture: the stream is still capturing");
  return was_open;
}

extern "C" int sdhip_graph_node_counts(void* graph, int* counts) {
  SDHIP_CHECK_ARG(graph && counts, "graph_node_counts: null pointer");
  size_t n = 0;
  if (hipGraphGetNodes((hipGraph_t)graph, nullptr, &n) != hipSuccess) SDHIP_FAIL(SDHIP_ERR_LAUNCH, "graph_node_counts: hipGraphGetNodes failed");
  std::vector<hipGraphNode_t> nodes(n);
  if (n && hipGraphGetNodes((hipGraph_t)graph, nodes.data(), &n) != hipSuccess) SDHIP_FAIL(SDHIP_ERR_LAUNCH, "graph_node_counts: hipGraphGetNodes failed");
  counts[0] = counts[1] = counts[2] = counts[3] = 0;
  for (size_t i = 0; i < n; ++i) {
    hipGraphNodeType t;
    if (hipGraphNodeGetType(nodes[i], &t) != hipSuccess) SDHIP_FAIL(SDHIP_ERR_LAUNCH, "graph_node_counts: hipGraphNodeGetType failed");
    if (t == hipGraphNodeTypeKernel) ++counts[0];
    else if (t == hipGraphNodeTypeMemset) ++counts[1];
    else if (t == hipGraphNodeTypeMemcpy) ++counts[2];
    else ++counts[3];
  }
  return (int)n;
}
```

pmt_learning_for_semantic_segmentation_and_disparity_amd/csrc/sdhip_common.h:

```cpp
#pragma once
#include <hip/hip_runtime.h>
#include <stdint.h>
#include <stdio.h>
#include <stdarg.h>
#include <stdlib.h>
#include <initializer_list>
#include <type_traits>

#include "../../include/sdhip.h"

#define SDHIP_WAVE 64

typedef unsigned short bf16_t;

typedef __attribute__((ext_vector_type(4))) float f32x4;
typedef __attribute__((ext_vector_type(2))) float f32x2;
typedef __attribute__((ext_vector_type(8))) __bf16 bf16x8_t;
typedef __attribute__((ext_vector_type(4))) __bf16 bf16x4_t;
typedef __attribute__((ext_vector_type(4))) unsigned int u32x4;
typedef __attribute__((ext_vector_type(2))) unsigned int u32x2;

void sdhip_set_error(const char* fmt, ...);
#define SDHIP_FAIL(code, ...) do { sdhip_set_error(__VA_ARGS__); return (code); } while (0)
#define SDHIP_CHECK_ARG(cond, ...) do { if (!(cond)) SDHIP_FAIL(SDHIP_ERR_ARG, __VA_ARGS__); } while (0)
#define SDHIP_LAUNCH_CHECK_AS(who) do { hipError_t e__ = hipGetLastError(); \
    if (e__ != hipSuccess) SDHIP_FAIL(SDHIP_ERR_LAUNCH, "%s: launch failed: %s", (who), hipGetErrorString(e__)); } while (0)
#define SDHIP_LAUNCH_CHECK() SDHIP_LAUNCH_CHECK_AS(__func__)

struct SdhipDiag {
  bool conv_generic, conv_big, conv_no_thin, conv_no_gemm, conv_no_band, conv_no_band3, wgrad_generic, wgrad_no_pack, wgrad_force_pack, wgrad_no_half, thin_wgrad_reg, corr_no_tiled, wgrad_no_half32, wgrad_split2d, wgrad_no_gemm, conv_no_point, conv_no_grow, conv_no_mid;
  int tune_s2_small;
  int tune_big, tune_split, tune_thin_blocks, tune_fused_blocks, tune_gemm_dbg, tune_band_dbg;
  int tune_mid_min_map, tune_mid_max_map, tune_mid_max_wg;
  double tune_atomic_tbs, tune_wg1_tile;
};
const SdhipDiag& sdhip_diag();

__device__ __forceinline__ float bf2f(bf16_t v) { return __builtin_bit_cast(float, ((unsigned int)v) << 16); }
__device__ __forceinline__ bf16_t f2bf(float f) { return __builtin_bit_cast(bf16_t, (__bf16)f); }
__device__ __forceinline__ unsigned int pack2bf(float lo, float hi) {
  return (unsigned int)f2bf(lo) | ((unsigned int)f2bf(hi) << 16);
}
__device__ __forceinline__ float bflo(unsigned int u) { return __builtin_bit_cast(float, u << 16); }
__device__ __forceinline__ float bfhi(unsigned int u) { return __builtin_bit_cast(float, u & 0xffff0000u); }

template <typename T> struct Elem;
template <> struct Elem<float> {
  static constexpr int kPer16B = 4;
  static __device__ __forceinline__ float ld(const float* p) { return *p; }
  static __device__ __forceinline__ void st(float* p, float v) { *p = v; }
  static __device__ __forceinline__ float rnd(float v) { return v; }
};
template <> struct Elem<bf16_t> {
  static constexpr int kPer16B = 8;
  static __device__ __forceinline__ float ld(const bf16_t* p) { return bf2f(*p); }
  static __device__ __forceinline__ void st(bf16_t* p, float v) { *p = f2bf(v); }
  static __device__ __forceinline__ float rnd(float v) { return bf2f(f2bf(v)); }
};

template <typename T> struct Chunk;
template <> struct Chunk<float> {
  static constexpr int N = 4;
  static __device__ __forceinline__ void unpack(const u32x4& u, float* f) {
    const f32x4 v = __builtin_bit_cast(f32x4, u);
#pragma unroll
    for (int i = 0; i < 4; ++i) f[i] = v[i];
  }
  static __device__ __forceinline__ u32x4 pack(const float* f) {
    f32x4 v;
#pragma unroll
    for (int i = 0; i < 4; ++i) v[i] = f[i];
    return __builtin_bit_cast(u32x4, v);
  }
};
template <> struct Chunk<bf16_t> {
  static constexpr int N = 8;
  static __device__ __forceinline__ void unpack(const u32x4& u, float* f) {
#pragma unroll
    for (int i = 0; i < 4; ++i) { f[2 * i] = bflo(u[i]); f[2 * i + 1] = bfhi(u[i]); }
  }
  static __device__ __forceinline__ u32x4 pack(const float* f) {
    u32x4 u;
#pragma unroll
    for (int i = 0; i < 4; ++i) u[i] = pack2bf(f[2 * i], f[2 * i + 1]);
    return u;
  }
};

template <typename T> __device__ __forceinline__ T wave_sum(T v) {
#pragma unroll
  for (int o = 32; o > 0; o >>= 1) v += __shfl_xor(v, o, 64);
  return v;
}
__device__ __forceinline__ float wave_max(float v) {
#pragma unroll
  for (int o = 32; o > 0; o >>= 1) v = fmaxf(v, __shfl_xor(v, o, 64));
  return v;
}

__device__ __forceinline__ float block_sum(float v, float* sh) {
  v = wave_sum(v);
  if ((threadIdx.x & 63) == 0) sh[threadIdx.x >> 6] = v;
  __syncthreads();
  float r = 0.f;
  if (threadIdx.x == 0) for (int i = 0; i < (int)(blockDim.x >> 6); ++i) r += sh[i];
  return r;
}
template <typename T> __device__ __forceinline__ T block_tail(T v, T* red) {
  const int tid = threadIdx.x;
#pragma unroll
  for (int o = 32; o > 0; o >>= 1) v += __shfl_xor(v, o, 64);
  if ((tid & 63) == 0) red[tid >> 6] = v;
  __syncthreads();
  return ((red[0] + red[1]) + red[2]) + red[3];
}

template <typename T, bool VEC> struct Unit {
  static constexpr int N = VEC ? Chunk<T>::N : 1;
  static __device__ __forceinline__ void load(const T* p, float* f) {
    if constexpr (VEC) Chunk<T>::unpack(*reinterpret_cast<const u32x4*>(p), f);
    else f[0] = Elem<T>::ld(p);
  }
  static __device__ __forceinline__ void store(T* p, const float* f) {
    if constexpr (VEC) *reinterpret_cast<u32x4*>(p) = Chunk<T>::pack(f);
    else Elem<T>::st(p, f[0]);
  }
  using Raw = std::conditional_t<VEC, u32x4, T>;
  static __device__ __forceinline__ Raw raw(const T* p) {
    if constexpr (VEC) return *reinterpret_cast<const u32x4*>(p);
    else return *p;
  }
  static __device__ __forceinline__ void unpack(const Raw& r, float* f) {
    if constexpr (VEC) Chunk<T>::unpack(r, f);
    else f[0] = Elem<T>::ld(&r);
  }
};

__device__ __forceinline__ float hsig_f(float v) { return fminf(fmaxf(v + 3.f, 0.f), 6.f) / 6.f; }
__device__ __forceinline__ float act_hs(float v, int act) { return act == SDHIP_ACT_HSWISH ? v * hsig_f(v) : hsig_f(v); }
__device__ __forceinline__ float act_hs_d(float v, int act) {
  const float t = v + 3.f;
  const float m = (t > 0.f && t < 6.f) ? 1.f / 6.f : 0.f;
  return act == SDHIP_ACT_HSWISH ? hsig_f(v) + v * m : m;
}

static inline int sdhip_cdiv(long a, long b) { return (int)((a + b - 1) / b); }

template <typename T> struct SdhipType { using type = T; };
template <typename F> inline auto sdhip_by_dtype(int dtype, F&& f) {
  return dtype == SDHIP_F32 ? f(SdhipType<float>{}) : f(SdhipType<bf16_t>{});
}
template <typename F> inline auto sdhip_by_flag(bool b, F&& f) { return b ? f(std::true_type{}) : f(std::false_type{}); }

#define SDHIP_CHECK_DTYPE(who, dtype) \
  SDHIP_CHECK_ARG((dtype) == SDHIP_F32 || (dtype) == SDHIP_BF16, "%s: unknown dtype %d", who, (int)(dtype))

template <typename T>
inline bool sdhip_vec_ok(int C, std::initializer_list<int> lds, std::initializer_list<const void*> ptrs) {
  const int n = Chunk<T>::N;
  if (C % n) return false;
  for (int l : lds) if (l % n) return false;
  for (const void* p : ptrs) if (p && ((uintptr_t)p & 15)) return false;
  return true;
}

namespace {
__global__ __launch_bounds__(256) void sdhip_zero_kernel(unsigned char* __restrict__ p, size_t bytes) {
  const size_t stride = (size_t)gridDim.x * 256;
  const size_t i = (size_t)blockIdx.x * 256 + threadIdx.x;
  size_t head = (size_t)((16 - (((uintptr_t)p) & 15)) & 15);
  if (head > bytes) head = bytes;
  const size_t n16 = (bytes - head) >> 4;
  const size_t tail0 = head + (n16 << 4);
  u32x4* p16 = reinterpret_cast<u32x4*>(p + head);
  for (size_t j = i; j < n16; j += stride) p16[j] = u32x4{0u, 0u, 0u, 0u};
  if (i < head) p[i] = 0;
  if (tail0 + i < bytes && i < 16) p[tail0 + i] = 0;
}
inline hipError_t sdhip_zero_async(void* ptr, size_t bytes, hipStream_t s) {
  if (bytes == 0) return hipSuccess;
  size_t blocks = (bytes / 16 + 255) / 256;
  if (blocks > 2048) blocks = 2048;
  if (blocks < 1) blocks = 1;
  hipLaunchKernelGGL(sdhip_zero_kernel, dim3((unsigned)blocks), dim3(256), 0, s, (unsigned char*)ptr, bytes);
  return hipGetLastError();
}
}
```

pmt_learning_for_semantic_segmentation_and_disparity_amd/ops.py:

```python
import os
import torch

from . import _lib
from ._lib import call, dtype_code, ptr, stream_ptr, try_call


def _require_gpu(*ts):
    for t in ts:
        if t is not None and not t.is_cuda:
            raise _lib.SdhipError("sdhip ops need GPU tensors (got %s); there is no CPU path" % t.device)


def nhwc_view(x):
    B, C, H, W = x.shape
    sb, sc, sh, sw = x.stride()
    ld = sw
    ok = (sc == 1 or C == 1) and ld >= C and (sh == W * ld or H == 1) and (sb == H * W * ld or B == 1)
    if W == 1:
        ok = False if (sc != 1 and C != 1) else (sh >= C and (sb == H * sh or B == 1))
        ld = sh if ok else ld
    if not ok:
        x = x.contiguous(memory_format=torch.channels_last)
        if x.stride(1) != 1 and C != 1:
            x = x.permute(0, 2, 3, 1).contiguous().permute(0, 3, 1, 2)
# ... 384 lines not shown

    def finish(self):
        self.measuring = False
        slot = lambda bn, g: (g * bn.num_features + 3) & ~3
        n = sum(2 * slot(bn, g) for bn, g, _, _ in self.tables.values())
        self.table_buf = torch.empty(max(n, 4), dtype=torch.float32, device=self.device)
        off = 0
        for rec in self.tables.values():
            bn, g = rec[0], rec[1]
            k, step = g * bn.num_features, slot(bn, g)
            rec[2] = self.table_buf[off:off + k].view(g, bn.num_features)
            rec[3] = self.table_buf[off + step:off + step + k].view(g, bn.num_features)
            off += 2 * step

    def rows(self):
        rows = [fold_row(r.weight.detach(), r.kind, r.bn, None, r.pack, r.bias_out) for r in self.layers.values() if r.ok]
        rows += [table_row(bn, g, sc, sh) for bn, g, sc, sh in self.tables.values()]
        return rows


def bn_frozen(bn):
    return not bn.training and not _wants_grad(bn.weight, bn.bias)


def _wants_grad(gamma, beta):
    return (gamma is not None and gamma.requires_grad) or (beta is not None and beta.requires_grad)


def _fold_state(bn=None):
    c = _ctx[0]
    if c is None or c.fold is None or (bn is not None and bn.training):
        return None
    if c.fold.train:
        return c.fold if c.fold.live and bn is not None and bn_frozen(bn) else None
    return None if torch.is_grad_enabled() else c.fold


def _folded_conv_bn_act(fold, x, weight, bn, spec, act, residual, groups, views=None):
    if act not in FOLD_ACTS or spec.D != 1 or spec.Do != 1 or weight.dim() != 4 or bn.running_mean is None or x.dtype != fold.dtype:
        return None
    rec = fold.layer(weight, bn, spec.kind)
    if rec is None or not rec.ok:
        return None
    _require_gpu(x, weight)
    B, Cin, H, W = x.shape
    xv, ldx = aligned_view(x)
    Cout = spec.cout(weight)
    y, ldy = alloc_nhwc(B, Cout, spec.Ho, spec.Wo, x.dtype, x.device)
    if residual is not None:
        if residual.shape != y.shape or residual.dtype != y.dtype:
            raise _lib.SdhipError("conv_bn_act: residual does not match the output")
        rv, ldres = nhwc_view(residual)
        call("sdhip_affine_act", ptr(rv), ldres, ptr(y), ldy, None, 0, None, None, B * spec.Ho * spec.Wo, Cout, 1, 0, dtype_code(x),
             stream_ptr())
    ran = try_call("sdhip_conv2d_fwd", ptr(xv), ptr(rec.pack), ptr(y), ptr(rec.bias_out), None, None, None, 0, 1,
                   B, H, W, Cin, ldx, spec.Ho, spec.Wo, Cout, ldy, spec.kh, spec.kw, spec.stride, spec.dil, spec.pad_t, spec.pad_l,
                   *spec.depth(), 0, groups, act, int(residual is not None), dtype_code(x), stream_ptr())
    if not ran:
        rec.ok = False
        return None
    fold.calls += 1
    if views is not None:
        views.append((xv, ldx, ldy))
    return y


class _NoFold(Exception):
    """The folded kernel does not take this layer's shape: conv_bn_act runs the table form instead (once; the record remembers)."""


class _FoldedConvBNActFn(torch.autograd.Function):

    @staticmethod
    def forward(ctx, x, weight, fold, spec, bn, act, groups, in_slot, in_bn):
        views = []
        y = _folded_conv_bn_act(fold, x, weight, bn, spec, act, None, groups, views)
        if y is None:
            raise _NoFold()
        (xv, ldx, ldy), = views
        scale = _bn_finalize(None, 1, bn, 0, 1)[0]
        ctx.spec, ctx.act, ctx.ldx, ctx.ldy, ctx.in_slot, ctx.in_bn = spec, act, ldx, ldy, in_slot, in_bn
        ctx.save_for_backward(xv, weight, y, scale)
        return y

    @staticmethod
    def backward(ctx, gy):
        xv, weight, y, scale = ctx.saved_tensors
        spec = ctx.spec
        B, Cout = y.shape[0], y.shape[1]
        g, ldg = nhwc_view(gy)
        graw, ldgr = alloc_nhwc(B, Cout, spec.Ho, spec.Wo, y.dtype, y.device)
        call("sdhip_act_out_bwd", ptr(g), ldg, ptr(y), ctx.ldy, ptr(graw), ldgr, ptr(scale), B * spec.Ho * spec.Wo, Cout, 1, ctx.act,
             dtype_code(y), stream_ptr())
        acc, addend = _take_parked(ctx.in_slot, xv, ctx.needs_input_grad[0])
        gx, gw, _ = _conv_backward(spec, xv, ctx.ldx, weight, graw, ldgr, None, None, False, 1, ctx.needs_input_grad[0],
                                   ctx.needs_input_grad[1], acc_into=acc, addend=addend, bn_slot=ctx.in_bn)
        return gx, gw, None, None, None, None, None, None, None


class ConvSpec:
    __slots__ = ("kind", "kh", "kw", "stride", "dil", "pad_t", "pad_l", "Ho", "Wo", "D", "Do", "kd", "sd", "pad_d")

    def __init__(self, kind, kh, kw, stride, dil, pad_t, pad_l, Ho, Wo, D=1, Do=1, kd=1, sd=1, pad_d=0):
        self.kind, self.kh, self.kw, self.stride, self.dil = kind, kh, kw, stride, dil
        self.pad_t, self.pad_l, self.Ho, self.Wo = pad_t, pad_l, Ho, Wo
        self.D, self.Do, self.kd, self.sd, self.pad_d = D, Do, kd, sd, pad_d

    def depth(self):
        return (self.D, self.Do, self.kd, self.sd, self.pad_d)

    def cout(self, weight):
        return weight.shape[0 if self.kind == 'conv' else 1]


def _conv_launch(x, ldx, wp, y, ldy, bias, in_scale, in_shift, stats, B, H, W, Cin, Ho, Wo, Cout,
                 kh, kw, stride, dil, pad_t, pad_l, in_relu, groups, act, accumulate, nrep=1, depth=(1, 1, 1, 1, 0)):
    sld = stats.stride(-2) if stats is not None else 0
    call("sdhip_conv2d_fwd", ptr(x), ptr(wp), ptr(y), ptr(bias), ptr(in_scale), ptr(in_shift), ptr(stats), sld, nrep,
         B, H, W, Cin, ldx, Ho, Wo, Cout, ldy, kh, kw, stride, dil, pad_t, pad_l, *depth,
         int(in_relu), groups, act, int(accumulate), dtype_code(x), stream_ptr())


NREP = _lib.NREP

from . import parallel


def _sync_stats(stats, nrep):
    if stats is None or parallel.world_size() == 1:
        return stats, nrep
    if stats.is_contiguous():
        parallel.all_reduce_sum_(stats)
        return stats, nrep
    G, _, C = stats.shape[-3:]
    compact, pz = _zeros((G, 2, C), torch.float64, stats.device)
    if not pz:
        compact.zero_()
    call("sdhip_stats_replica_sum", ptr(stats), ptr(compact), nrep, G, C, stats.stride(-2), C, stream_ptr())
    parallel.all_reduce_sum_(compact)
    return compact, 1


def _bn_finalize(stats, nrep, bn, count, groups, synced=False):
    C = bn.num_features
    dev = bn.weight.device
    if stats is None:
        fold = _fold_state(bn)
        t = fold.table(bn, groups) if fold is not None else None
        if t is not None:
            return [t[0], t[1], None, None]
    if not synced:
        stats, nrep = _sync_stats(stats, nrep)
    count = parallel.global_count(count)
    out = [torch.empty((groups, C), dtype=torch.float32, device=dev) for _ in range(4)]
    if stats is not None:
        _bn_track(bn, groups)
        call("sdhip_bn_finalize", ptr(stats), stats.stride(-2), nrep, ptr(bn.weight), ptr(bn.bias), ptr(bn.running_mean),
             ptr(bn.running_var), ptr(out[0]), ptr(out[1]), ptr(out[2]), ptr(out[3]), C, groups, float(count),
             float(bn.eps), float(_bn_momentum(bn)), stream_ptr())
    else:
        call("sdhip_bn_finalize", None, 0, 1, ptr(bn.weight), ptr(bn.bias), ptr(bn.running_mean), ptr(bn.running_var),
             ptr(out[0]), ptr(out[1]), ptr(out[2]), ptr(out[3]), C, groups, float(count), float(bn.eps), 0.0, stream_ptr())
    return out


def _fused_bn():
    return not _lib.DIAG_NO_FUSED_BN


def _bn_momentum(bn):
    return 0.1 if bn.momentum is None else bn.momentum


def _bn_track(bn, groups):
    if bn.num_batches_tracked is None:
        return
    c = _ctx[0]
    if c is not None and c.nbt is not None and c.arena is not None:
        return
    if c is not None and c.nbt is not None:
        c.nbt.append((bn.num_batches_tracked, groups))
    bn.num_batches_tracked += groups


def _bn_param_grads(gamma, beta, C, device):
    tg, tb = _grad_target(gamma), _grad_target(beta)
    if tg is not None and tb is not None:
        return tg, tb, True, (None, None)
    dgamma, dbeta = (torch.empty(C, dtype=torch.float32, device=device) for _ in range(2))
    return dgamma, dbeta, False, (dgamma, dbeta)


def bn_backward_two_phase(gy, ldg, x, ldx, gx, ldgx, scale, shift, mean, invstd, gamma, beta, npix, C, groups, act, count, dt):
    dev = scale.device
    both, pz = _zeros((2, NREP, groups, C), torch.float32, dev)
    dsc, dsh = both[0], both[1]
    call("sdhip_affine_act_bwd", ptr(gy), ldg, ptr(x), ldx, None, 0, ptr(scale), ptr(shift), ptr(dsc), ptr(dsh), NREP,
         npix, C, groups, act, 0, int(pz), dt, stream_ptr())
    parallel.all_reduce_sum_(both)
    dgamma, dbeta, direct, returned = _bn_param_grads(gamma, beta, C, dev)
    call("sdhip_bn_bwd_apply_fin", ptr(gy), ldg, ptr(x), ldx, ptr(gx), ldgx, ptr(scale), ptr(shift), ptr(dsc), ptr(dsh), NREP,
         ptr(gamma), ptr(mean), ptr(invstd), ptr(dgamma), ptr(dbeta), int(direct), parallel.param_scale(), npix, C, groups,
         float(count), act, dt, stream_ptr())
    return returned


def _bn_backward(gy, ldg, x, ldx, gx, ldgx, scale, shift, mean, invstd, gamma, npix, C, groups, act, count, train,
                 dt, accumulate_gx=False, dstats=None, accumulate_dstats=False, beta=None):
    dev = scale.device
    if not train and not _wants_grad(gamma, beta):
        call("sdhip_affine_act_bwd", ptr(gy), ldg, ptr(x), ldx, ptr(gx), ldgx, ptr(scale), ptr(shift), None, None, 1,
             npix, C, groups, act, int(accumulate_gx), 0, dt, stream_ptr())
        return None, None, None
    both, pz = _zeros((2, NREP, groups, C), torch.float32, dev)
    dsc, dsh = both[0], both[1]
    call("sdhip_affine_act_bwd", ptr(gy), ldg, ptr(x), ldx, ptr(gx), ldgx, ptr(scale), ptr(shift), ptr(dsc), ptr(dsh), NREP,
         npix, C, groups, act, int(accumulate_gx), int(pz), dt, stream_ptr())
    dgamma, dbeta, direct, returned = _bn_param_grads(gamma, beta, C, dev)
    par_flag = 2 if direct else 0
    if dstats is None:
        dstats = torch.empty((groups, 2, C), dtype=torch.float64, device=dev)
        accumulate_dstats = False
    if parallel.world_size() > 1 and train:
        call("sdhip_bn_finalize_bwd", ptr(dsc), ptr(dsh), NREP, ptr(gamma), ptr(mean), ptr(invstd), ptr(dgamma), ptr(dbeta),
             None, C, par_flag, C, groups, float(count), 1, stream_ptr())
        parallel.all_reduce_sum_(both)
        call("sdhip_bn_finalize_bwd", ptr(dsc), ptr(dsh), NREP, ptr(gamma), ptr(mean), ptr(invstd), None, None,
             ptr(dstats), dstats.stride(-2), int(accumulate_dstats), C, groups, float(parallel.global_count(count)), 1,
             stream_ptr())
    else:
        call("sdhip_bn_finalize_bwd", ptr(dsc), ptr(dsh), NREP, ptr(gamma), ptr(mean), ptr(invstd), ptr(dgamma), ptr(dbeta),
             ptr(dstats), dstats.stride(-2), int(accumulate_dstats) | par_flag, C, groups, float(count), int(train), stream_ptr())
    return (*returned, dstats)


_BN_ACTS = (0, 1, 2, _lib.ACT_HSWISH, _lib.ACT_HSIGMOID)


def _bn_act_forward(yraw, ldr, bn, ws, count, groups, act, residual=None):
    B, C, Ho, Wo = yraw.shape
    npix, dt = B * Ho * Wo, dtype_code(yraw)
    rv, ldres = nhwc_view(residual) if residual is not None else (None, 0)
    y, ldy = alloc_nhwc(B, C, Ho, Wo, yraw.dtype, yraw.device)
    if ws is not None and _fused_bn():
        scale, shift, mean, invstd = [torch.empty((groups, C), dtype=torch.float32, device=yraw.device) for _ in range(4)]
        _bn_track(bn, groups)
        parallel.all_reduce_sum_(ws)
        call("sdhip_affine_act_bn", ptr(yraw), ldr, ptr(y), ldy, ptr(rv), ldres, ptr(ws), ws.stride(-2), NREP, ptr(bn.weight),
             ptr(bn.bias), ptr(bn.running_mean), ptr(bn.running_var), ptr(scale), ptr(shift), ptr(mean), ptr(invstd),
             npix, C, groups, float(parallel.global_count(count)), float(bn.eps), float(_bn_momentum(bn)), act, dt, stream_ptr())
    else:
        scale, shift, mean, invstd = _bn_finalize(ws, NREP, bn, count, groups)
        call("sdhip_affine_act", ptr(yraw), ldr, ptr(y), ldy, ptr(rv), ldres, ptr(scale), ptr(shift), npix, C, groups, act, dt,
             stream_ptr())
    return y, scale, shift, mean, invstd


def _bn_act_backward(g, ldg, yraw, ldraw, scale, shift, mean, invstd, gamma, beta, groups, act, count, train, presummed=None,
                     out=None):
    B, C, Ho, Wo = yraw.shape
    npix, dt = B * Ho * Wo, dtype_code(yraw)
    graw, ldgr = out if out is not None else alloc_nhwc(B, C, Ho, Wo, yraw.dtype, yraw.device)
    if presummed is not None:
        dgamma, dbeta, direct, returned = _bn_param_grads(gamma, beta, C, yraw.device)
        parallel.all_reduce_sum_(presummed)
        call("sdhip_bn_bwd_apply_fin_d", ptr(g), ldg, ptr(yraw), ldraw, ptr(graw), ldgr, ptr(scale), ptr(shift), ptr(presummed), NREP,
             ptr(gamma), ptr(mean), ptr(invstd), ptr(dgamma), ptr(dbeta), int(direct), parallel.param_scale(), npix, C, groups,
             float(parallel.global_count(count)), act, dt, stream_ptr())
        return graw, ldgr, *returned
    if train and act not in _BN_ACTS:
        raise _lib.SdhipError("train-mode BatchNorm backward: activation %d is not one the two-phase kernels take" % act)
    if train and _fused_bn():
        dgamma, dbeta = bn_backward_two_phase(g, ldg, yraw, ldraw, graw, ldgr, scale, shift, mean, invstd, gamma, beta, npix, C,
                                              groups, act, parallel.global_count(count), dt)
    elif train:
        dgamma, dbeta, dS = _bn_backward(g, ldg, yraw, ldraw, None, 0, scale, shift, mean, invstd, gamma, npix, C, groups, act,
                                         count, True, dt, beta=beta)
        call("sdhip_bn_bwd_apply", ptr(g), ldg, ptr(yraw), ldraw, ptr(graw), ldgr, ptr(scale), ptr(shift), ptr(dS), C, npix, C,
             groups, act, dt, stream_ptr())
    else:
        dgamma, dbeta, _ = _bn_backward(g, ldg, yraw, ldraw, graw, ldgr, scale, shift, mean, invstd, gamma, npix, C, groups, act,
                                        count, False, dt, beta=beta)
    return graw, ldgr, dgamma, dbeta


class GradSlot:
    __slots__ = ("g", "exclusive")

    def __init__(self, exclusive):
        self.g = None
        self.exclusive = exclusive


def _take_parked(slot, xv, need_x):
    if slot is None or slot.g is None or not need_x:
        return None, None
    parked, slot.g = slot.g, None
    if parked.shape != xv.shape or parked.dtype != xv.dtype:
        raise _lib.SdhipError("GradSlot: parked gradient does not match the input it belongs to")
    return (parked, None) if slot.exclusive else (None, parked)


BN_SLOT_MAX_BYTES = _lib.TUNE_BN_SLOT_MAX_MB << 20


class BNSlot:
    __slots__ = ("u", "ldu", "scale", "shift", "groups", "C", "sums", "gptr")

    def __init__(self):
        self.u = self.scale = self.shift = self.sums = None
        self.ldu = self.groups = self.C = 0
        self.gptr = 0


def _conv_backward(ctx_spec, xv, ldx, weight, g, ldg, in_scale, in_shift, in_relu, groups, need_x, need_w, bias=None, acc_into=None,
                   addend=None, bn_slot=None):
    spec = ctx_spec
    Bimg, Cin, H, W = xv.shape
    B = Bimg // spec.D
    Cout = spec.cout(weight)
    dt = dtype_code(xv)
    gpost = gw = gb = None
    if need_x:
        wd = packed_weight(weight, spec.kind, 'dgrad', xv.dtype)
        fused_bn = False
        if (bn_slot is not None and bn_slot.u is not None and bn_slot.C == Cin and xv.dtype == torch.bfloat16 and spec.stride == 1
                and spec.sd == 1 and spec.kd == 1 and spec.D == 1 and tuple(bn_slot.u.shape) == (Bimg, Cin, H, W)
                and spec.kh * spec.kw <= 9 and Bimg * H * W * Cin * 2 <= BN_SLOT_MAX_BYTES):
            other = acc_into if acc_into is not None else addend
            gpost, ldgp = alloc_nhwc(Bimg, Cin, H, W, xv.dtype, xv.device)
            sums = _zeros((NREP, bn_slot.groups, 2, Cin), torch.float64, xv.device)[0]
            ov, ldo = nhwc_view(other) if other is not None else (None, 0)
            fused_bn = try_call("sdhip_conv2d_fwd_bnbwd", ptr(g), ptr(wd), ptr(gpost), ptr(sums), Cin, NREP, ptr(bn_slot.u), bn_slot.ldu,
                                ptr(bn_slot.scale), ptr(bn_slot.shift), ptr(ov), ldo, B, spec.Ho, spec.Wo, Cout, ldg, H, W, Cin, ldgp,
                                spec.kh, spec.kw, spec.dil, spec.dil * (spec.kh - 1) - spec.pad_t,
                                spec.dil * (spec.kw - 1) - spec.pad_l, bn_slot.groups, 0, dt, stream_ptr())
            if fused_bn:
                bn_slot.sums, bn_slot.gptr = sums, gpost.data_ptr()
        if (not fused_bn and acc_into is None and addend is None and spec.kind == 'conv' and spec.stride == 2 and spec.sd == 2
                and spec.kd == 3 and spec.kh == 3 and spec.kw == 3 and spec.dil == 1 and spec.pad_t == 1 and spec.pad_l == 1
                and spec.pad_d == 1 and spec.D == 2 * spec.Do and H == 2 * spec.Ho and W == 2 * spec.Wo and not _lib.DIAG_NO_PHASE_DGRAD):
            gpost, ldgp = alloc_nhwc(Bimg, Cin, H, W, xv.dtype, xv.device)
            packs, _keep = _phase_packs(weight, xv.dtype)
            for (pd, ph, pw), wpk in zip(_PHASES, packs):
                call("sdhip_conv2d_fwd_phase", ptr(g), ptr(wpk), ptr(gpost), None, 0, 1, B, spec.Ho, spec.Wo, Cout, ldg, Cin, ldgp,
                     1 + ph, 1 + pw, spec.Do, 1 + pd, 1, pd, ph, pw, dt, stream_ptr())
            if need_w:
                gw, gb = wgrad(xv, ldx, g, ldg, weight, bias, spec, in_scale, in_shift, in_relu, groups)
            return gpost, gw, gb
        if fused_bn:
            pass
        elif acc_into is not None:
            gpost, ldgp = nhwc_view(acc_into)
        else:
            gpost, ldgp = alloc_nhwc(Bimg, Cin, H, W, xv.dtype, xv.device)
        pt = spec.dil * (spec.kh - 1) - spec.pad_t
        pl = spec.dil * (spec.kw - 1) - spec.pad_l
        pd = (spec.kd - 1) - spec.pad_d
        gsrc, ldsrc, Dg, Hg, Wg = g, ldg, spec.Do, spec.Ho, spec.Wo
        if spec.stride != 1 or spec.sd != 1:
            Dg, Hg, Wg = (spec.Do - 1) * spec.sd + 1, (spec.Ho - 1) * spec.stride + 1, (spec.Wo - 1) * spec.stride + 1
            gsrc = empty_nhwc(B * Dg, Cout, Hg, Wg, xv.dtype, xv.device)
            call("sdhip_stuff", ptr(g), ldg, ptr(gsrc), Cout, B, spec.Do, spec.Ho, spec.Wo, Cout, spec.sd, spec.stride, 1, dt,
                 stream_ptr())
            ldsrc = Cout
        fused_add = fused_bn
        if not fused_bn and addend is not None and spec.kd == 1 and spec.D == 1 and spec.dil == 1 and gsrc is g:
            av, lda = nhwc_view(addend)
            fused_add = try_call("sdhip_conv2d_fwd_add", ptr(gsrc), ptr(wd), ptr(gpost), ptr(av), lda, B, Hg, Wg, Cout, ldsrc, H, W, Cin,
                                 ldgp, spec.kh, spec.kw, pt, pl, dt, stream_ptr())
        if not fused_add:
            _conv_launch(gsrc, ldsrc, wd, gpost, ldgp, None, None, None, None, B, Hg, Wg, Cout, H, W, Cin,
                         spec.kh, spec.kw, 1, spec.dil, pt, pl, False, 1, 0, acc_into is not None, 1, (Dg, spec.D, spec.kd, 1, pd))
            if addend is not None:
                gpost = add(gpost, addend)

    if need_w:
        gw, gb = wgrad(xv, ldx, g, ldg, weight, bias, spec, in_scale, in_shift, in_relu, groups)
    return gpost, gw, gb


def wgrad(xv, ldx, g, ldg, weight, bias, spec, in_scale=None, in_shift=None, in_relu=False, groups=1):
    c = _ctx[0]
    if c is not None and c.side is not None and c.direct_grads and not c.defer_wgrad:
        main = torch.cuda.current_stream()
        c.side.wait_stream(main)
        c.keep.append((xv, g, in_scale, in_shift))
        with torch.cuda.stream(c.side):
            return _wgrad_impl(xv, ldx, g, ldg, weight, bias, spec, in_scale, in_shift, in_relu, groups)
    return _wgrad_impl(xv, ldx, g, ldg, weight, bias, spec, in_scale, in_shift, in_relu, groups)


def _wgrad_impl(xv, ldx, g, ldg, weight, bias, spec, in_scale, in_shift, in_relu, groups):
    Bimg, Cin, H, W = xv.shape
    B = Bimg // spec.D
    Cout = spec.cout(weight)
    dt = dtype_code(xv)
    T = spec.kh * spec.kw
    per = _lib.packed_elems(Cout, Cin, T, dt)
    acc, pz = _zeros((per * spec.kd,), torch.float32, xv.device)
    tw = _grad_target(weight)
    tb = _grad_target(bias) if bias is not None else None
    gb = None
    if bias is not None:
        if tb is not None:
            dbias, dbias_pz = tb, True
        else:
            dbias, dbias_pz = _zeros((Cout,), torch.float32, xv.device)
            gb = dbias
    else:
        dbias, dbias_pz = None, True
    if bias is not None and pz != dbias_pz:
        if not pz:
            acc.zero_()
        elif tb is None:
            dbias.zero_()
        pz = True
    c = _ctx[0]
    if (c is not None and c.defer_wgrad and c.direct_grads and c.arena is not None and tw is not None and pz
            and (bias is None or tb is not None)):
        dpt = lambda t: t.data_ptr() if t is not None else None
        c.wq.append((dpt(xv), dpt(g), dpt(acc), dpt(dbias), dpt(in_scale), dpt(in_shift), B, H, W, Cin, ldx, spec.Ho, spec.Wo, Cout, ldg,
                     spec.kh, spec.kw, spec.stride, spec.dil, spec.pad_t, spec.pad_l) + tuple(spec.depth()) + (int(in_relu), groups))
        c.wq_keep.append((xv, g, in_scale, in_shift))
        c.wq_dt = dt
        if not c.overlap:
            c.flush_to_side()
    else:
        call("sdhip_conv2d_wgrad", ptr(xv), ptr(g), ptr(acc), ptr(dbias), ptr(in_scale), ptr(in_shift),
             B, H, W, Cin, ldx, spec.Ho, spec.Wo, Cout, ldg, spec.kh, spec.kw, spec.stride, spec.dil,
             spec.pad_t, spec.pad_l, *spec.depth(), int(in_relu), groups, int(pz), dt, stream_ptr())
    gw = None
    target = tw
    if target is None:
        gw = target = torch.empty_like(weight, memory_format=torch.contiguous_format)
    c = _ctx[0]
    defer = c is not None and c.direct_grads and tw is not None and pz and c.arena is not None
    for src_off, blk, M, K, T_, sm, sk, flip in _pack_rows(weight, spec.kind, 'fwd', dt):
        if defer:
            c.unpacks.append((acc.data_ptr() + 4 * per * blk, target.data_ptr() + 4 * src_off, M, K, T_, sm, sk, flip))
            c.unpack_dt = dt
        else:
            call("sdhip_conv_unpack_wgrad", ctypes_ptr(acc.data_ptr() + 4 * per * blk), ctypes_ptr(target.data_ptr() + 4 * src_off),
                 M, K, T_, sm, sk, flip, 1 if tw is not None else 0, dt, stream_ptr())
    return gw, gb


class _ConvFn(torch.autograd.Function):

    @staticmethod
    def forward(ctx, x, weight, bias, spec, act):
        _require_gpu(x, weight)
        Bimg, Cin, H, W = x.shape
        B = Bimg // spec.D
        xv, ldx = aligned_view(x)
        Cout = spec.cout(weight)
        wp = packed_weight(weight, spec.kind, 'fwd', x.dtype)
        y, ldy = alloc_nhwc(B * spec.Do, Cout, spec.Ho, spec.Wo, x.dtype, x.device)
        _conv_launch(xv, ldx, wp, y, ldy, bias.detach() if bias is not None else None, None, None, None, B, H, W, Cin,
                     spec.Ho, spec.Wo, Cout, spec.kh, spec.kw, spec.stride, spec.dil, spec.pad_t, spec.pad_l, False, 1, act, False,
                     1, spec.depth())
        ctx.spec, ctx.act, ctx.ldx = spec, act, ldx
        ctx.save_for_backward(xv, weight, bias, y if act else None)
        return y

    @staticmethod
    def backward(ctx, gy):
        xv, weight, bias, ysaved = ctx.saved_tensors
        spec, act = ctx.spec, ctx.act
        B = xv.shape[0] // spec.D * spec.Do
        Cout = spec.cout(weight)
        g, ldg = aligned_view(gy)
        if act:
            g2, ldg2 = alloc_nhwc(B, Cout, spec.Ho, spec.Wo, xv.dtype, xv.device)
            call("sdhip_affine_act_bwd", ptr(g), ldg, ptr(ysaved), nhwc_view(ysaved)[1], ptr(g2), ldg2, None, None, None, None, 1,
                 B * spec.Ho * spec.Wo, Cout, 1, 1 if act == 1 else 4, 0, 0, dtype_code(xv), stream_ptr())
            g, ldg = g2, ldg2
        gx, gw, gb = _conv_backward(spec, xv, ctx.ldx, weight, g, ldg, None, None, False, 1, ctx.needs_input_grad[0],
                                    ctx.needs_input_grad[1] or (bias is not None and ctx.needs_input_grad[2]), bias)
        return gx, gw, gb, None, None


class _ConvBNActFn(torch.autograd.Function):

    @staticmethod
    def forward(ctx, x, weight, gamma, beta, residual, spec, bn, act, groups, in_slot=None, res_slot=None, in_bn=None, out_bn=None):
        _require_gpu(x, weight)
        ctx.in_slot, ctx.res_slot, ctx.in_bn, ctx.out_bn = in_slot, res_slot, in_bn, out_bn
        Bimg, Cin, H, W = x.shape
        Btrue = Bimg // spec.D
        B = Btrue * spec.Do
        xv, ldx = aligned_view(x)
        Cout = spec.cout(weight)
        wp = packed_weight(weight, spec.kind, 'fwd', x.dtype)
        yraw, ldr_ = alloc_nhwc(B, Cout, spec.Ho, spec.Wo, x.dtype, x.device)
        train = bn.training
        ws = _zeros((NREP, groups, 2, Cout), torch.float64, x.device)[0] if train else None
        _conv_launch(xv, ldx, wp, yraw, ldr_, None, None, None, ws, Btrue, H, W, Cin, spec.Ho, spec.Wo, Cout,
                     spec.kh, spec.kw, spec.stride, spec.dil, spec.pad_t, spec.pad_l, False, groups, 0, False, NREP, spec.depth())
        count = (B // groups) * spec.Ho * spec.Wo
        y, scale, shift, mean, invstd = _bn_act_forward(yraw, ldr_, bn, ws, count, groups, act, residual)
        ctx.spec, ctx.act, ctx.groups, ctx.ldx, ctx.count, ctx.train = spec, act, groups, ldx, count, train
        ctx.ldraw = ldr_
        ctx.has_res = residual is not None
        if out_bn is not None and train and act == 1 and _fused_bn() and spec.D == 1 and spec.Do == 1:
            out_bn.u, out_bn.ldu, out_bn.scale, out_bn.shift, out_bn.groups, out_bn.C = yraw, ldr_, scale, shift, groups, Cout
        ctx.save_for_backward(xv, weight, gamma, beta, yraw, scale, shift, mean, invstd)
        return y

    @staticmethod
    def backward(ctx, gy):
        xv, weight, gamma, beta, yraw, scale, shift, mean, invstd = ctx.saved_tensors
        spec, groups = ctx.spec, ctx.groups
        g, ldg = nhwc_view(gy)
        ob, sums = ctx.out_bn, None
        if ob is not None and ob.sums is not None and ob.gptr == g.data_ptr() and ctx.train and _fused_bn():
            sums, ob.sums, ob.gptr = ob.sums, None, 0
        graw, ldgr, dgamma, dbeta = _bn_act_backward(g, ldg, yraw, ctx.ldraw, scale, shift, mean, invstd, gamma, beta, groups,
                                                     ctx.act, ctx.count, ctx.train, presummed=sums)
        acc, addend = _take_parked(ctx.in_slot, xv, ctx.needs_input_grad[0])
        gx, gw, _ = _conv_backward(spec, xv, ctx.ldx, weight, graw, ldgr, None, None, False, 1, ctx.needs_input_grad[0],
                                   ctx.needs_input_grad[1], acc_into=acc, addend=addend, bn_slot=ctx.in_bn)
        gres = gy if ctx.has_res else None
        if gres is not None and ctx.res_slot is not None:
            ctx.res_slot.g, gres = gy, None
        return gx, gw, dgamma, dbeta, gres, None, None, None, None, None, None, None, None


class _BNConvFn(torch.autograd.Function):

    @staticmethod
    def forward(ctx, x, stats, weight, gamma, beta, spec, bn, groups):
        _require_gpu(x, weight)
        B, Cin, H, W = x.shape
        xv, ldx = nhwc_view(x)
        Cout = weight.shape[0]
        train = bn.training
        count = (B // groups) * H * W
        scale, shift, mean, invstd = _bn_finalize(stats if train else None, 1, bn, count, groups, synced=True)
        wp = packed_weight(weight, spec.kind, 'fwd', x.dtype)
        y = empty_nhwc(B, Cout, spec.Ho, spec.Wo, x.dtype, x.device)
        _conv_launch(xv, ldx, wp, y, Cout, None, scale, shift, None, B, H, W, Cin, spec.Ho, spec.Wo, Cout,
                     spec.kh, spec.kw, spec.stride, spec.dil, spec.pad_t, spec.pad_l, True, groups, 0, False)
        ctx.spec, ctx.groups, ctx.ldx, ctx.count, ctx.train = spec, groups, ldx, count, train
        ctx.save_for_backward(xv, weight, gamma, beta, scale, shift, mean, invstd)
        return y

    @staticmethod
    def backward(ctx, gy):
        xv, weight, gamma, beta, scale, shift, mean, invstd = ctx.saved_tensors
        spec, groups = ctx.spec, ctx.groups
        B, Cin, H, W = xv.shape
        dt = dtype_code(xv)
        g, ldg = nhwc_view(gy)
        gpost, gw, _ = _conv_backward(spec, xv, ctx.ldx, weight, g, ldg, scale, shift, True, groups, True, True)
        gx = empty_nhwc(B, Cin, H, W, xv.dtype, xv.device)
        dgamma, dbeta, dS = _bn_backward(gpost, nhwc_view(gpost)[1], xv, ctx.ldx, gx, Cin, scale, shift, mean, invstd, gamma,
                                         B * H * W, Cin, groups, 1, ctx.count, ctx.train, dt, beta=beta)
        return gx, (dS if ctx.train else None), gw, dgamma, dbeta, None, None, None


class _BNActFn(torch.autograd.Function):

    @staticmethod
    def forward(ctx, x, stats, gamma, beta, bn, act, groups):
        _require_gpu(x)
        B, C, H, W = x.shape
        xv, ldx = nhwc_view(x)
        train = bn.training
        count = (B // groups) * H * W
        scale, shift, mean, invstd = _bn_finalize(stats if train else None, 1, bn, count, groups, synced=True)
        y = empty_nhwc(B, C, H, W, x.dtype, x.device)
        call("sdhip_affine_act", ptr(xv), ldx, ptr(y), C, None, 0, ptr(scale), ptr(shift), B * H * W, C, groups, act,
             dtype_code(x), stream_ptr())
        ctx.cfg = (ldx, act, groups, count, train)
        ctx.save_for_backward(xv, gamma, beta, scale, shift, mean, invstd)
        return y

    @staticmethod
    def backward(ctx, gy):
        xv, gamma, beta, scale, shift, mean, invstd = ctx.saved_tensors
        ldx, act, groups, count, train = ctx.cfg
        B, C, H, W = xv.shape
        g, ldg = nhwc_view(gy)
        gx = empty_nhwc(B, C, H, W, xv.dtype, xv.device)
        dgamma, dbeta, dS = _bn_backward(g, ldg, xv, ldx, gx, C, scale, shift, mean, invstd, gamma, B * H * W, C, groups, act,
                                         count, train, dtype_code(xv), beta=beta)
        return gx, (dS if train else None), dgamma, dbeta, None, None, None


def conv1x1_cat_forward(segs, weight, bias, act):
    (x0, us0) = segs[0]
    x1, us1 = segs[1] if len(segs) > 1 else (None, 0)
    B, c0 = x0.shape[0], x0.shape[1]
    H, W = x0.shape[2] << us0, x0.shape[3] << us0
    v0, ld0 = aligned_view(x0)
    v1, ld1 = aligned_view(x1) if x1 is not None else (None, 0)
    c1 = x1.shape[1] if x1 is not None else 0
    Cout = weight.shape[0]
    wp = packed_weight(weight, 'conv', 'fwd', x0.dtype)
    y, ldy = alloc_nhwc(B, Cout, H, W, x0.dtype, x0.device)
    call("sdhip_conv1x1_cat_fwd", ptr(v0), ld0, c0, us0, ptr(v1), ld1, c1, us1, ptr(wp), ptr(y), ldy,
         ptr(bias.detach()) if bias is not None else None, B, H, W, Cout, act, dtype_code(x0), stream_ptr())
    return y


class _UpCatConv1x1Fn(torch.autograd.Function):

    @staticmethod
    def forward(ctx, xs, xf, weight, us, act):
        _require_gpu(xs, xf, weight)
        y = conv1x1_cat_forward([(xs, us), (xf, 0)], weight, None, act)
        ctx.save_for_backward(xs, xf, weight, y if act else None)
        ctx.cfg = (us, act)
        return y

    @staticmethod
    def backward(ctx, gy):
        xs, xf, weight, ysaved = ctx.saved_tensors
        us, act = ctx.cfg
        B, Cout, H, W = gy.shape
        c0, c1 = xs.shape[1], xf.shape[1]
        h, w = xs.shape[2], xs.shape[3]
        dt = dtype_code(gy)
        g, ldg = aligned_view(gy)
        if act:
            g2, ldg2 = alloc_nhwc(B, Cout, H, W, gy.dtype, gy.device)
            call("sdhip_affine_act_bwd", ptr(g), ldg, ptr(ysaved), nhwc_view(ysaved)[1], ptr(g2), ldg2, None, None, None, None, 1,
                 B * H * W, Cout, 1, 1 if act == 1 else 4, 0, 0, dt, stream_ptr())
            g, ldg = g2, ldg2
        k = 1 << us
# ... 1688 lines not shown
```

Before: 434.6 stereo-pairs/s.

## Fuse BatchNorm-backward epilogue into band conv dgrad kernel for 3x3/5x5

Adds a band-convolution kernel variant whose epilogue computes the BatchNorm-backward reductions (ReLU mask and per-channel sum of grad·u and grad) from the saved pre-activation. The kernel body moves into a shared include so the plain and BN-fused variants share one source. The Python side now routes 3x3 and 5x5 data-gradient convolutions with a BN slot onto the fused path, including 5x5 kernels and tensors above the old slot-size cap. The goal is to skip a separate pass that rereads the gradient and activation for BN statistics. The cost is more epilogue work and register pressure in the band kernel.

```diff
diff --git a/pmt_learning_for_semantic_segmentation_and_disparity_amd/_lib.py b/pmt_learning_for_semantic_segmentation_and_disparity_amd/_lib.py
--- a/pmt_learning_for_semantic_segmentation_and_disparity_amd/_lib.py
+++ b/pmt_learning_for_semantic_segmentation_and_disparity_amd/_lib.py
@@ -167,6 +167,9 @@
 TUNE_FUSE1_MAX_PIX = int(_diag_switch("SDHIP_TUNE_FUSE1_MAX_PIX") or 32768)
 TUNE_PRO_MAX_PIX = int(_diag_switch("SDHIP_TUNE_PRO_MAX_PIX") or 32768)
 TUNE_BN_SLOT_MAX_MB = int(_diag_switch("SDHIP_TUNE_BN_SLOT_MAX_MB") or 40)
+_forms = _diag_switch("SDHIP_TUNE_BAND_BX_FORMS")
+TUNE_BAND_BX_FORMS = "5x5,3x3" if _forms is None else ("" if _forms == "none" else _forms)
+del _forms
 DIAG_NO_BNPRO = bool(_diag_switch("SDHIP_DIAG_NO_BNPRO"))
 DIAG_NO_BNBWD_EPILOGUE = bool(_diag_switch("SDHIP_DIAG_NO_BNBWD_EPILOGUE"))
 DIAG_STEM_S2D = _diag_switch("SDHIP_STEM_S2D")
diff --git a/pmt_learning_for_semantic_segmentation_and_disparity_amd/csrc/conv_band.h b/pmt_learning_for_semantic_segmentation_and_disparity_amd/csrc/conv_band.h
--- a/pmt_learning_for_semantic_segmentation_and_disparity_amd/csrc/conv_band.h
+++ b/pmt_learning_for_semantic_segmentation_and_disparity_amd/csrc/conv_band.h
@@ -17,6 +17,9 @@
   int D, Do, pad_d;
   unsigned magic_do;
   int dbg;
+};
+struct BandBxArgs : BandArgs {
+  const void* bx; const float* bsc; const float* bsh; int ldbx;
 };
 
 template <int I, int N, typename F> __device__ __forceinline__ void band_static_for(F&& f) {
@@ -72,365 +75,17 @@
 
 template <int K, int BN, int VAR, int NW, int KD = 1>
 __global__ __launch_bounds__(NW * 64) void conv_band_kernel(const BandArgs p) {
-  constexpr bool DBG = (VAR & 128) != 0;
-  const int dbg = DBG ? p.dbg : 0;
-  using C = BandCfg<K, BN, NW, KD>;
-  using T = bf16_t;
-  constexpr int IWp = C::IWp, IW = C::IW, HB = C::HB, WB = C::WB, RPR = C::RPR, RPW = C::RPW;
-  constexpr int NT_CO = BN / 16, NT_PIX = 2 * RPW;
-  constexpr int NSTORE = NT_CO * NT_PIX / 2;
-  extern __shared__ __attribute__((aligned(16))) unsigned char smem[];
+#include "conv_band_body.h"
+}
 
-  const int tid = threadIdx.x, lane = tid & 63;
-  const int wave = __builtin_amdgcn_readfirstlane(tid >> 6);
-  const int l15 = lane & 15, lg = lane >> 4;
-
-  const int t_begin = blockIdx.x * p.tpw;
-  const int t_end = min(p.ntiles, t_begin + p.tpw);
-  if (t_begin >= t_end) return;
-  const int nhalf = KD > 1 ? KD : (p.Cin > 32 ? 2 : 1);
-  const int nchunks = (t_end - t_begin) * nhalf;
-
-  const int rsub = tid >> 2;
-  const int c_l = (tid & 3) ^ ((rsub >> 1) & 2);
-  const unsigned wave_lds = __builtin_amdgcn_readfirstlane(lds_addr(smem) + wave * 1024);
-  const band_rsrc_t xr = band_rsrc(p.x), wr = band_rsrc(p.wp);
-  const int img_bytes = p.H * p.W * p.ldx * 2;
-
-  int czt = 0;
-  auto tile_of = [&](int t, int& b, int& oh0, int& ow0) {
-    if constexpr (KD > 1) { const int q = fast_div(t, p.Do, p.magic_do); czt = t - q * p.Do; t = q; }
-    b = fast_div(t, p.tiles_hw, p.magic_hw);
-    const int r = t - b * p.tiles_hw;
-    const int ty = fast_div(r, p.tiles_w, p.magic_tw);
-    oh0 = ty * C::TH;
-    ow0 = (r - ty * p.tiles_w) * C::TW;
-  };
-  int hv[C::HR];
-  auto halo_offsets = [&](int oh0, int ow0) {
-    const int ih0 = oh0 - p.pad_t, iw0 = ow0 - p.pad_l;
-#pragma unroll
-    for (int r = 0; r < C::HR; ++r) {
-      const int row = r * RPR + rsub;
-      const int ih = row / IWp, iw = row - ih * IWp;
-      const int gh = ih0 + ih, gw = iw0 + iw;
-      const bool in = iw < IW && (unsigned)gh < (unsigned)p.H && (unsigned)gw < (unsigned)p.W && c_l * 8 < p.Cin;
-      hv[r] = in ? ((gh * p.W + gw) * p.ldx + c_l * 8) * 2 : kBandOob;
-    }
-  };
-  auto halo_dma = [&](int r, int soff, int hsel) {
-    if (r < C::HR && r * RPR + wave * 16 < C::HROWS) band_dma(soff >= 0 ? hv[r] : kBandOob, xr, hsel * HB + r * (RPR * 64) + wave_lds, soff >= 0 ? soff : 0);
-  };
-  auto chunk_src = [&](int b, int zt, int h) -> int {
-    if constexpr (KD > 1) {
-      const int zin = zt + h - p.pad_d;
-      return (zin >= 0 && zin < p.D) ? (b * p.D + zin) * img_bytes : -1;
-    } else {
-      return b * img_bytes + h * 64;
-    }
-  };
-  int wv[C::WR];
-#pragma unroll
-  for (int r = 0; r < C::WR; ++r) {
-    const int row = r * RPR + rsub;
-    const int tap = row / BN, m = min(row % BN, p.Mpad - 1);
-    wv[r] = (tap * p.Mpad + m) * 128 + c_l * 16;
-  }
-  const int wrow_bytes = C::TPS * p.Mpad * 128;
-  auto w_dma = [&](int r, int j, int h, int wsel) {
-    if (r < C::WR && r * RPR + wave * 16 < C::WROWS)
-      band_dma(wv[r], wr, 2 * HB + wsel * WB + r * (RPR * 64) + wave_lds, j * wrow_bytes + (KD > 1 ? h * wrow_bytes : h * 64));
-  };
-
-  int b_k[K];
-#pragma unroll
-  for (int kw = 0; kw < K; ++kw) b_k[kw] = LdsRow<1>::off(kw + l15, lg);
-  const int a_base = LdsRow<1>::off(l15, lg);
-  const int wave_row = wave * (RPW * IWp * 64);
-
-  float bv[NT_CO][4];
-#pragma unroll
-  for (int mi = 0; mi < NT_CO; ++mi)
-#pragma unroll
-    for (int r = 0; r < 4; ++r) {
-      const int co = mi * 16 + 4 * lg + r;
-      bv[mi][r] = (p.bias && co < p.Cout) ? p.bias[co] : 0.f;
-    }
-
-  f32x4 acc[NT_CO][NT_PIX];
-  float s1[NT_CO][4], s2[NT_CO][4];
-#pragma unroll
-  for (int mi = 0; mi < NT_CO; ++mi)
-#pragma unroll
-    for (int r = 0; r < 4; ++r) { s1[mi][r] = 0.f; s2[mi][r] = 0.f; }
-
-  float* const red = reinterpret_cast<float*>(smem + 2 * HB + C::NWB * WB);
-  auto flush_stats = [&](int grp) {
-#pragma unroll
-    for (int mi = 0; mi < NT_CO; ++mi) {
-#pragma unroll
-      for (int r = 0; r < 4; ++r) {
-        const float a = row16_sum(s1[mi][r]), c2 = row16_sum(s2[mi][r]);
-        if (l15 == 0) {
-          const int m = mi * 16 + 4 * lg + r;
-          red[(wave * 2 + 0) * BN + m] = a;
-          red[(wave * 2 + 1) * BN + m] = c2;
-        }
-        s1[mi][r] = 0.f; s2[mi][r] = 0.f;
-      }
-    }
-    asm volatile("s_waitcnt lgkmcnt(0)" ::: "memory");
-    __builtin_amdgcn_s_barrier();
-    if (tid < 2 * BN) {
-      const int which = tid / BN, m = tid - which * BN;
-      if (m < p.Cout) {
-        float tot = 0.f;
-#pragma unroll
-        for (int w = 0; w < NW; ++w) tot += red[(w * 2 + which) * BN + m];
-        atomicAdd(p.stats + (long)(blockIdx.x % p.nrep) * p.rep_stride + ((long)grp * 2 + which) * p.stats_ld + m, (double)tot);
-      }
-    }
-  };
-
-  if constexpr ((VAR & 2) != 0) { if (wave >= 4) __builtin_amdgcn_s_setprio(1); }
-  int cb, coh0, cow0, ch_half = 0, ct = t_begin;
-  tile_of(ct, cb, coh0, cow0);
-  halo_offsets(coh0, cow0);
-#pragma unroll
-  for (int r = 0; r < C::WR; ++r) w_dma(r, 0, 0, 0);
-#pragma unroll
-  for (int r = 0; r < C::HR; ++r) halo_dma(r, chunk_src(cb, czt, 0), 0);
-  int cz = czt;
-  int wsel = 0;
-  bool epi_counted = false;
-
-  constexpr bool WREG = C::WRES && BN <= 32;
-  u32x4 wreg[WREG ? C::TPS : 1][NT_CO];
-
-  for (int c = 0; c < nchunks; ++c) {
-    const int hsel = c & 1;
-    const bool has_next = c + 1 < nchunks;
-    int nb = cb, noh0 = coh0, now0 = cow0, nh = ch_half + 1, nt = ct, nz = cz;
-    if (nh == nhalf) {
-      nh = 0; nt = ct + 1;
-      if (has_next) { tile_of(nt, nb, noh0, now0); halo_offsets(noh0, now0); nz = czt; }
-    }
-    const int nsoff = chunk_src(nb, nz, nh);
-    if (ch_half == 0) {
-#pragma unroll
-      for (int mi = 0; mi < NT_CO; ++mi)
-#pragma unroll
-        for (int ni = 0; ni < NT_PIX; ++ni) acc[mi][ni] = f32x4{0.f, 0.f, 0.f, 0.f};
-    }
-    const unsigned char* const hb = smem + hsel * HB + wave_row;
-
-    band_static_for<0, C::NSTG>([&](auto jc) {
-      constexpr int j = decltype(jc)::value;
-      constexpr int r_lo = (j - 1) * C::HPS, r_hi = j * C::HPS < C::HR ? j * C::HPS : C::HR;
-      constexpr bool counted = j >= 1 && r_hi > r_lo && r_hi * RPR <= C::HROWS;
-      if (j == 0 && epi_counted) band_wait<NSTORE>();
-      else if (counted && has_next) band_wait<counted ? r_hi - r_lo : 0>();
-      else band_wait<0>();
-      if (!(dbg & 16)) __builtin_amdgcn_s_barrier();
-
-      const unsigned char* const wl = smem + 2 * HB + wsel * WB + a_base;
-      const unsigned char* const hj = hb + j * C::RS * (IWp * 64);
-      if constexpr (WREG) {
-        if (c == 0) {
-#pragma unroll
-          for (int t = 0; t < C::TPS; ++t)
-#pragma unroll
-            for (int mi = 0; mi < NT_CO; ++mi) wreg[t][mi] = *reinterpret_cast<const u32x4*>(wl + t * (BN * 64) + mi * 1024);
-        }
-      }
-      u32x4 af[2][NT_CO], bf[2][NT_PIX];
-      if constexpr (DBG) if (dbg & 32) {
-#pragma unroll
-        for (int i = 0; i < 2; ++i)
-#pragma unroll
-          for (int q = 0; q < 4; ++q) { if (q < NT_CO) af[i][q] = u32x4{0x3f803f80u, (unsigned)tid, 0x3f803f80u, 0x3f803f80u}; bf[i][q] = u32x4{0x3f803f80u, 0x3f803f80u, (unsigned)lane, 0x3f803f80u}; }
-      }
-      auto load = [&](int set, int t) {
-        if (dbg & 32) return;
-#pragma unroll
-        for (int mi = 0; mi < NT_CO; ++mi) {
-          if constexpr (WREG) af[set][mi] = wreg[t][mi];
-          else af[set][mi] = *reinterpret_cast<const u32x4*>(wl + t * (BN * 64) + mi * 1024);
-        }
-#pragma unroll
-        for (int ni = 0; ni < NT_PIX; ++ni)
-          bf[set][ni] = *reinterpret_cast<const u32x4*>(hj + b_k[t % K] + ((t / K + (ni >> 1)) * IWp + (ni & 1) * 16) * 64);
-      };
-      auto dma_slot = [&](int sl) {
-        if (sl < C::WRS) {
-          if (dbg & 2) return;
-          if (j + 1 < C::NSTG) w_dma(sl, j + 1, ch_half, wsel ^ 1);
-          else if (has_next) w_dma(sl, 0, nh, wsel ^ 1);
-        } else if (sl < C::WRS + C::HPS) {
-          if (dbg & 1) return;
-          if (has_next && (C::NSTG == 1 || j < C::NSTG - 1)) halo_dma(j * C::HPS + sl - C::WRS, nsoff, hsel ^ 1);
-        }
-      };
-      load(0, 0);
-#pragma unroll
-      for (int kw = 0; kw < C::TPS; ++kw) {
-        if constexpr ((VAR & 1) != 0) {
-#pragma unroll
-          for (int sl = kw * C::SPT; sl < (kw + 1) * C::SPT; ++sl) dma_slot(sl);
-        }
-        if (kw + 1 < C::TPS) load((kw + 1) & 1, kw + 1);
-        if constexpr ((VAR & 1) == 0) {
-#pragma unroll
-          for (int sl = kw * C::SPT; sl < (kw + 1) * C::SPT; ++sl) dma_slot(sl);
-        }
-        if (!(dbg & 4)) {
-#pragma unroll
-          for (int mi = 0; mi < NT_CO; ++mi)
-#pragma unroll
-            for (int ni = 0; ni < NT_PIX; ++ni) Mma<T>::run(acc[mi][ni], af[kw & 1][mi], bf[kw & 1][ni]);
-        }
-        if constexpr ((VAR & 4) != 0) {
-#pragma unroll
-          for (int g = 0; g < NT_CO + NT_PIX; ++g) {
-            __builtin_amdgcn_sched_group_barrier(0x100, 1, 0);
-            __builtin_amdgcn_sched_group_barrier(0x008, (NT_CO * NT_PIX) / (NT_CO + NT_PIX), 0);
-          }
-        }
-      }
-      if constexpr (!C::WRES) wsel ^= 1;
-    });
-
-    epi_counted = false;
-    if (ch_half == nhalf - 1) {
-      const int oimg = KD > 1 ? cb * p.Do + cz : cb;
-      const int grp = oimg < p.bpg ? 0 : oimg / p.bpg;
-      if (p.bias) {
-#pragma unroll
-        for (int mi = 0; mi < NT_CO; ++mi)
-#pragma unroll
-          for (int ni = 0; ni < NT_PIX; ++ni)
-#pragma unroll
-            for (int r = 0; r < 4; ++r) acc[mi][ni][r] += bv[mi][r];
-      }
-      if (p.act == 1) {
-#pragma unroll
-        for (int mi = 0; mi < NT_CO; ++mi)
-#pragma unroll
-          for (int ni = 0; ni < NT_PIX; ++ni)
-#pragma unroll
-            for (int r = 0; r < 4; ++r) acc[mi][ni][r] = fmaxf(acc[mi][ni][r], 0.f);
-      } else if (p.act == 2) {
-#pragma unroll
-        for (int mi = 0; mi < NT_CO; ++mi)
-#pragma unroll
-          for (int ni = 0; ni < NT_PIX; ++ni)
-#pragma unroll
-            for (int r = 0; r < 4; ++r) acc[mi][ni][r] = 1.f / (1.f + __expf(-acc[mi][ni][r]));
-      }
-      T* const yb = (T*)p.y + (long)oimg * p.Ho * p.Wo * p.ldy;
-      const T* const rb = (const T*)p.res + (long)oimg * p.Ho * p.Wo * p.ldres;
-      const bool interior = coh0 + C::TH <= p.Ho && cow0 + C::TW <= p.Wo && BN <= p.Cout;
-      if (interior) {
-        const long pix0 = (long)(coh0 + RPW * wave) * p.Wo + cow0 + (lg & 1) * 16 + l15;
-        T* const d0 = yb + pix0 * p.ldy + 8 * (lg >> 1);
-        const T* const r0 = rb + pix0 * p.ldres + 8 * (lg >> 1);
-#pragma unroll
-        for (int q = 0; q < NT_PIX / 2; ++q) {
-          T* dst = d0 + (long)q * p.Wo * p.ldy;
-          const T* rsrc = r0 + (long)q * p.Wo * p.ldres;
-          u32x4 ov[NT_CO];
-#pragma unroll
-          for (int mi = 0; mi < NT_CO; ++mi) {
-            const f32x4 v0 = acc[mi][2 * q], v1 = acc[mi][2 * q + 1];
-            const u32x2 o0 = u32x2{pack2bf(v0[0], v0[1]), pack2bf(v0[2], v0[3])};
-            const u32x2 o1 = u32x2{pack2bf(v1[0], v1[1]), pack2bf(v1[2], v1[3])};
-            if (p.stats) {
-              const f32x4 w0 = f32x4{bflo(o0[0]), bfhi(o0[0]), bflo(o0[1]), bfhi(o0[1])};
-              const f32x4 w1 = f32x4{bflo(o1[0]), bfhi(o1[0]), bflo(o1[1]), bfhi(o1[1])};
-#pragma unroll
-              for (int r = 0; r < 4; ++r) {
-                s1[mi][r] += w0[r] + w1[r];
-                s2[mi][r] = fmaf(w1[r], w1[r], fmaf(w0[r], w0[r], s2[mi][r]));
-              }
-            }
-            u32x4 o;
-            if (p.res) {
-              float f[8];
-#pragma unroll
-              for (int r = 0; r < 4; ++r) {
-                const float a0 = v0[r], a1 = v1[r];
-                const u32x2 e = __builtin_amdgcn_permlane16_swap(__float_as_uint(a0), __float_as_uint(a1), false, false);
-                const unsigned e0 = e[0], e1 = e[1];
-                f[r] = __uint_as_float(e0); f[4 + r] = __uint_as_float(e1);
-              }
-              const u32x4 old = *reinterpret_cast<const u32x4*>(rsrc + mi * 16);
-#pragma unroll
-              for (int e = 0; e < 4; ++e) o[e] = pack2bf(f[2 * e] + bflo(old[e]), f[2 * e + 1] + bfhi(old[e]));
-            } else {
-              const u32x2 e0 = __builtin_amdgcn_permlane16_swap(o0[0], o1[0], false, false);
-              const u32x2 e1 = __builtin_amdgcn_permlane16_swap(o0[1], o1[1], false, false);
-              o = u32x4{e0[0], e1[0], e0[1], e1[1]};
-            }
-            ov[mi] = o;
-          }
-          if (!(dbg & 8)) {
-#pragma unroll
-            for (int mi = 0; mi < NT_CO; ++mi) *reinterpret_cast<u32x4*>(dst + mi * 16) = ov[mi];
-          }
-        }
-        epi_counted = !(dbg & 8) && !p.res;
-      } else {
-#pragma unroll
-        for (int ni = 0; ni < NT_PIX; ++ni) {
-          const int oh = coh0 + RPW * wave + (ni >> 1), ow = cow0 + (ni & 1) * 16 + l15;
-          const bool valid = oh < p.Ho && ow < p.Wo;
-          T* dst = yb + ((long)oh * p.Wo + ow) * p.ldy;
-          const T* rsrc = rb + ((long)oh * p.Wo + ow) * p.ldres;
-#pragma unroll
-          for (int mi = 0; mi < NT_CO; ++mi) {
-            const int co = mi * 16 + 4 * lg;
-            float v[4];
-#pragma unroll
-            for (int r = 0; r < 4; ++r) v[r] = acc[mi][ni][r];
-            if (valid && co + 3 < p.Cout) {
-              if (p.res) {
-                const u32x2 old = *reinterpret_cast<const u32x2*>(rsrc + co);
-                v[0] += bflo(old[0]); v[1] += bfhi(old[0]); v[2] += bflo(old[1]); v[3] += bfhi(old[1]);
-              }
-              const u32x2 o = u32x2{pack2bf(v[0], v[1]), pack2bf(v[2], v[3])};
-              *reinterpret_cast<u32x2*>(dst + co) = o;
-              v[0] = bflo(o[0]); v[1] = bfhi(o[0]); v[2] = bflo(o[1]); v[3] = bfhi(o[1]);
-            } else if (valid && co < p.Cout) {
-#pragma unroll
-              for (int r = 0; r < 4; ++r) {
-                if (co + r < p.Cout) {
-                  if (p.res) v[r] += Elem<T>::ld(rsrc + co + r);
-                  Elem<T>::st(dst + co + r, v[r]); v[r] = Elem<T>::rnd(v[r]);
-                }
-                else v[r] = 0.f;
-              }
-            } else {
-#pragma unroll
-              for (int r = 0; r < 4; ++r) v[r] = 0.f;
-            }
-            if (p.stats) {
-#pragma unroll
-              for (int r = 0; r < 4; ++r) { s1[mi][r] += v[r]; s2[mi][r] = fmaf(v[r], v[r], s2[mi][r]); }
-            }
-          }
-        }
-      }
-      if (p.stats) {
-        const int nimg = KD > 1 ? nb * p.Do + nz : nb;
-        const int ngrp = nimg < p.bpg ? 0 : nimg / p.bpg;
-        if (!has_next || ngrp != grp) { flush_stats(grp); epi_counted = false; }
-      }
-    }
-    cb = nb; coh0 = noh0; cow0 = now0; ch_half = nh; ct = nt; cz = nz;
-  }
+template <int K, int BN, int VAR, int NW, int KD = 1>
+__global__ __launch_bounds__(NW * 64) void conv_band_bx_kernel(const BandBxArgs p) {
+  static_assert((VAR & 8) != 0 && KD == 1, "the BatchNorm-backward epilogue: 2-D form only");
+#include "conv_band_body.h"
 }
 
 inline bool band_ok(int ntiles) { return ntiles >= 192 && ntiles < 65536; }
+inline bool band_bx_form_ok(int k, int Mpad, bool addend) { return !(k == 5 && Mpad > 32 && addend); }
 
 template <int K, int BN, int VAR, int NW = 8, int KD = 1>
 int launch_band_bn(const BandArgs& a, int grid, hipStream_t s) {
@@ -447,8 +102,24 @@
   return SDHIP_OK;
 }
 
-template <int K, int KD = 1>
-int launch_band(BandArgs& a, hipStream_t s) {
+template <int K, int BN, int VAR, int NW = 8>
+int launch_band_bx_bn(const BandBxArgs& a, int grid, hipStream_t s) {
+  auto kern = conv_band_bx_kernel<K, BN, VAR, NW>;
+  static bool attr_set = false;
+  if (!attr_set) {
+    if (hipFuncSetAttribute((const void*)kern, hipFuncAttributeMaxDynamicSharedMemorySize, 160 * 1024) != hipSuccess)
+      SDHIP_FAIL(SDHIP_ERR_LAUNCH, "conv_band: cannot raise dynamic LDS limit");
+    attr_set = true;
+  }
+  constexpr size_t lds = BandCfg<K, BN, NW, 1>::LDS + 2 * BN * sizeof(float);
+  static_assert(lds <= 160 * 1024, "LDS budget of the BatchNorm-backward form");
+  hipLaunchKernelGGL(kern, dim3(grid), dim3(NW * 64), lds, s, a);
+  SDHIP_LAUNCH_CHECK();
+  return SDHIP_OK;
+}
+
+template <int KD>
+int band_tiling(BandArgs& a) {
   const int tiles_h = sdhip_cdiv(a.Ho, 16);
   a.tiles_w = sdhip_cdiv(a.Wo, 32);
   a.tiles_hw = tiles_h * a.tiles_w;
@@ -457,8 +128,13 @@
   a.magic_hw = a.tiles_hw > 1 ? (unsigned)(0x100000000ULL / (unsigned)a.tiles_hw) + 1u : 0u;
   a.magic_tw = a.tiles_w > 1 ? (unsigned)(0x100000000ULL / (unsigned)a.tiles_w) + 1u : 0u;
   a.tpw = sdhip_cdiv(a.ntiles, 256);
+  return sdhip_cdiv(a.ntiles, a.tpw);
+}
+
+template <int K, int KD = 1>
+int launch_band(BandArgs& a, hipStream_t s) {
+  const int grid = band_tiling<KD>(a);
   a.dbg = sdhip_diag().tune_band_dbg;
-  const int grid = sdhip_cdiv(a.ntiles, a.tpw);
   a.dbg &= 0xff;
   if constexpr (K == 5) {
     if (a.Mpad > 32) return a.dbg ? launch_band_bn<K, 64, 128 + 5>(a, grid, s) : launch_band_bn<K, 64, 5>(a, grid, s);
@@ -470,4 +146,18 @@
   return launch_band_bn<K, 32, 5>(a, grid, s);
 }
 
+template <int K>
+int launch_band_bx(BandBxArgs& a, hipStream_t s) {
+  const int grid = band_tiling<1>(a);
+  a.dbg = 0;
+  if (!band_bx_form_ok(K, a.Mpad, a.res != nullptr))
+    SDHIP_FAIL(SDHIP_ERR_UNSUPPORTED, "conv_band: the BatchNorm-backward form with an addend is not built for %dx%d with more than 32 output channels", K, K);
+  if constexpr (K == 5) {
+    if (a.Mpad > 32) return launch_band_bx_bn<K, 64, 5 + 8>(a, grid, s);
+  } else {
+    if (a.Mpad > 32) return a.res ? launch_band_bx_bn<K, 64, 5 + 8 + 16>(a, grid, s) : launch_band_bx_bn<K, 64, 5 + 8>(a, grid, s);
+  }
+  return a.res ? launch_band_bx_bn<K, 32, 5 + 8 + 16>(a, grid, s) : launch_band_bx_bn<K, 32, 5 + 8>(a, grid, s);
 }
+
+}
diff --git a/pmt_learning_for_semantic_segmentation_and_disparity_amd/csrc/conv_band_body.h b/pmt_learning_for_semantic_segmentation_and_disparity_amd/csrc/conv_band_body.h
--- /dev/null
+++ b/pmt_learning_for_semantic_segmentation_and_disparity_amd/csrc/conv_band_body.h
@@ -0,0 +1,496 @@
+  constexpr bool DBG = (VAR & 128) != 0;
+  constexpr bool BX = (VAR & 8) != 0;
+  static_assert(!BX || (KD == 1 && !DBG), "the BatchNorm-backward epilogue: 2-D form only");
+  const std::conditional_t<BX, BandBxArgs, BandArgs>& pbx = p;
+  const int dbg = DBG ? p.dbg : 0;
+  using C = BandCfg<K, BN, NW, KD>;
+  using T = bf16_t;
+  constexpr int IWp = C::IWp, IW = C::IW, HB = C::HB, WB = C::WB, RPR = C::RPR, RPW = C::RPW;
+  constexpr int NT_CO = BN / 16, NT_PIX = 2 * RPW;
+  constexpr int NSTORE = NT_CO * NT_PIX / 2;
+  extern __shared__ __attribute__((aligned(16))) unsigned char smem[];
+
+  const int tid = threadIdx.x, lane = tid & 63;
+  const int wave = __builtin_amdgcn_readfirstlane(tid >> 6);
+  const int l15 = lane & 15, lg = lane >> 4;
+
+  const int t_begin = blockIdx.x * p.tpw;
+  const int t_end = min(p.ntiles, t_begin + p.tpw);
+  if (t_begin >= t_end) return;
+  const int nhalf = KD > 1 ? KD : (p.Cin > 32 ? 2 : 1);
+  const int nchunks = (t_end - t_begin) * nhalf;
+
+  const int rsub = tid >> 2;
+  const int c_l = (tid & 3) ^ ((rsub >> 1) & 2);
+  const unsigned wave_lds = __builtin_amdgcn_readfirstlane(lds_addr(smem) + wave * 1024);
+  const band_rsrc_t xr = band_rsrc(p.x), wr = band_rsrc(p.wp);
+  const int img_bytes = p.H * p.W * p.ldx * 2;
+
+  int czt = 0;
+  auto tile_of = [&](int t, int& b, int& oh0, int& ow0) {
+    if constexpr (KD > 1) { const int q = fast_div(t, p.Do, p.magic_do); czt = t - q * p.Do; t = q; }
+    b = fast_div(t, p.tiles_hw, p.magic_hw);
+    const int r = t - b * p.tiles_hw;
+    const int ty = fast_div(r, p.tiles_w, p.magic_tw);
+    oh0 = ty * C::TH;
+    ow0 = (r - ty * p.tiles_w) * C::TW;
+  };
+  int hv[C::HR];
+  auto halo_offsets = [&](int oh0, int ow0) {
+    const int ih0 = oh0 - p.pad_t, iw0 = ow0 - p.pad_l;
+#pragma unroll
+    for (int r = 0; r < C::HR; ++r) {
+      const int row = r * RPR + rsub;
+      const int ih = row / IWp, iw = row - ih * IWp;
+      const int gh = ih0 + ih, gw = iw0 + iw;
+      const bool in = iw < IW && (unsigned)gh < (unsigned)p.H && (unsigned)gw < (unsigned)p.W && c_l * 8 < p.Cin;
+      hv[r] = in ? ((gh * p.W + gw) * p.ldx + c_l * 8) * 2 : kBandOob;
+    }
+  };
+  auto halo_dma = [&](int r, int soff, int hsel) {
+    if (r < C::HR && r * RPR + wave * 16 < C::HROWS) band_dma(soff >= 0 ? hv[r] : kBandOob, xr, hsel * HB + r * (RPR * 64) + wave_lds, soff >= 0 ? soff : 0);
+  };
+  auto chunk_src = [&](int b, int zt, int h) -> int {
+    if constexpr (KD > 1) {
+      const int zin = zt + h - p.pad_d;
+      return (zin >= 0 && zin < p.D) ? (b * p.D + zin) * img_bytes : -1;
+    } else {
+      return b * img_bytes + h * 64;
+    }
+  };
+  int wv[C::WR];
+#pragma unroll
+  for (int r = 0; r < C::WR; ++r) {
+    const int row = r * RPR + rsub;
+    const int tap = row / BN, m = min(row % BN, p.Mpad - 1);
+    wv[r] = (tap * p.Mpad + m) * 128 + c_l * 16;
+  }
+  const int wrow_bytes = C::TPS * p.Mpad * 128;
+  auto w_dma = [&](int r, int j, int h, int wsel) {
+    if (r < C::WR && r * RPR + wave * 16 < C::WROWS)
+      band_dma(wv[r], wr, 2 * HB + wsel * WB + r * (RPR * 64) + wave_lds, j * wrow_bytes + (KD > 1 ? h * wrow_bytes : h * 64));
+  };
+
+  int b_k[K];
+#pragma unroll
+  for (int kw = 0; kw < K; ++kw) b_k[kw] = LdsRow<1>::off(kw + l15, lg);
+  const int a_base = LdsRow<1>::off(l15, lg);
+  const int wave_row = wave * (RPW * IWp * 64);
+
+  float bv[NT_CO][4];
+#pragma unroll
+  for (int mi = 0; mi < NT_CO; ++mi)
+#pragma unroll
+    for (int r = 0; r < 4; ++r) {
+      const int co = mi * 16 + 4 * lg + r;
+      bv[mi][r] = (!BX && p.bias && co < p.Cout) ? p.bias[co] : 0.f;
+    }
+
+  f32x4 acc[NT_CO][NT_PIX];
+  float s1[NT_CO][4], s2[NT_CO][4];
+#pragma unroll
+  for (int mi = 0; mi < NT_CO; ++mi)
+#pragma unroll
+    for (int r = 0; r < 4; ++r) { s1[mi][r] = 0.f; s2[mi][r] = 0.f; }
+
+  float* const red = reinterpret_cast<float*>(smem + 2 * HB + C::NWB * WB);
+  float* const bxs = red + NW * 2 * BN;
+  auto bx_scale = [&](int grp) {
+    if constexpr (BX) {
+      if (tid < 2 * BN) {
+        const int which = tid / BN, m = tid - which * BN;
+        bxs[tid] = m < p.Cout ? (which ? pbx.bsh : pbx.bsc)[(long)grp * p.Cout + m] : 0.f;
+      }
+    }
+  };
+  auto bx_fold = [&]() {
+#pragma unroll
+    for (int mi = 0; mi < NT_CO; ++mi)
+#pragma unroll
+      for (int r = 0; r < 4; ++r) {
+        const float a = row16_sum(s1[mi][r]), c2 = row16_sum(s2[mi][r]);
+        if (l15 == 0) {
+          const int m = mi * 16 + 4 * lg + r;
+          red[(wave * 2 + 0) * BN + m] += a;
+          red[(wave * 2 + 1) * BN + m] += c2;
+        }
+      }
+  };
+  auto flush_stats = [&](int grp) {
+    if constexpr (!BX) {
+#pragma unroll
+      for (int mi = 0; mi < NT_CO; ++mi) {
+#pragma unroll
+        for (int r = 0; r < 4; ++r) {
+          const float a = row16_sum(s1[mi][r]), c2 = row16_sum(s2[mi][r]);
+          if (l15 == 0) {
+            const int m = mi * 16 + 4 * lg + r;
+            red[(wave * 2 + 0) * BN + m] = a;
+            red[(wave * 2 + 1) * BN + m] = c2;
+          }
+          s1[mi][r] = 0.f; s2[mi][r] = 0.f;
+        }
+      }
+    }
+    asm volatile("s_waitcnt lgkmcnt(0)" ::: "memory");
+    __builtin_amdgcn_s_barrier();
+    if (tid < 2 * BN) {
+      const int which = tid / BN, m = tid - which * BN;
+      if (m < p.Cout) {
+        float tot = 0.f;
+#pragma unroll
+        for (int w = 0; w < NW; ++w) tot += red[(w * 2 + which) * BN + m];
+        if constexpr (BX) {
+#pragma unroll
+          for (int w = 0; w < NW; ++w) red[(w * 2 + which) * BN + m] = 0.f;
+        }
+        atomicAdd(p.stats + (long)(blockIdx.x % p.nrep) * p.rep_stride + ((long)grp * 2 + which) * p.stats_ld + m, (double)tot);
+      }
+    }
+  };
+
+  if constexpr ((VAR & 2) != 0) { if (wave >= 4) __builtin_amdgcn_s_setprio(1); }
+  int cb, coh0, cow0, ch_half = 0, ct = t_begin;
+  tile_of(ct, cb, coh0, cow0);
+  if constexpr (BX) {
+    for (int i = lane; i < 2 * BN; i += 64) red[wave * 2 * BN + i] = 0.f;
+    bx_scale(cb < p.bpg ? 0 : cb / p.bpg);
+  }
+  halo_offsets(coh0, cow0);
+#pragma unroll
+  for (int r = 0; r < C::WR; ++r) w_dma(r, 0, 0, 0);
+#pragma unroll
+  for (int r = 0; r < C::HR; ++r) halo_dma(r, chunk_src(cb, czt, 0), 0);
+  int cz = czt;
+  int wsel = 0;
+  bool epi_counted = false;
+
+  constexpr bool WREG = C::WRES && BN <= 32;
+  u32x4 wreg[WREG ? C::TPS : 1][NT_CO];
+  constexpr bool BXR = (VAR & 16) != 0;
+  constexpr int BXQA = BX && BN <= 32 ? NT_PIX / 2 : 0;
+  constexpr bool BXRA = BXR && K == 5 && BN <= 32;
+
+  for (int c = 0; c < nchunks; ++c) {
+    const int hsel = c & 1;
+    const bool has_next = c + 1 < nchunks;
+    int nb = cb, noh0 = coh0, now0 = cow0, nh = ch_half + 1, nt = ct, nz = cz;
+    if (nh == nhalf) {
+      nh = 0; nt = ct + 1;
+      if (has_next) { tile_of(nt, nb, noh0, now0); halo_offsets(noh0, now0); nz = czt; }
+    }
+    const int nsoff = chunk_src(nb, nz, nh);
+    if (ch_half == 0) {
+#pragma unroll
+      for (int mi = 0; mi < NT_CO; ++mi)
+#pragma unroll
+        for (int ni = 0; ni < NT_PIX; ++ni) acc[mi][ni] = f32x4{0.f, 0.f, 0.f, 0.f};
+    }
+    const unsigned char* const hb = smem + hsel * HB + wave_row;
+
+    u32x4 bxu[BX ? NT_PIX / 2 : 1][NT_CO], bxr[BXR ? NT_PIX / 2 : 1][NT_CO];
+    auto bx_issue = [&](bool with_u, bool with_res, int q0, int q1) {
+      if constexpr (BX) {
+        if (!(coh0 + C::TH <= p.Ho && cow0 + C::TW <= p.Wo && BN <= p.Cout)) return;
+        const long pix0 = ((long)cb * p.Ho + coh0 + RPW * wave) * p.Wo + cow0 + (lg & 1) * 16 + l15;
+        if (with_u) {
+          const T* const u0 = (const T*)pbx.bx + pix0 * pbx.ldbx + 8 * (lg >> 1);
+#pragma unroll
+          for (int q = 0; q < NT_PIX / 2; ++q)
+#pragma unroll
+            for (int mi = 0; mi < NT_CO; ++mi) if (q >= q0 && q < q1) bxu[q][mi] = *reinterpret_cast<const u32x4*>(u0 + (long)q * p.Wo * pbx.ldbx + mi * 16);
+        }
+        if constexpr (BXR) {
+          if (with_res) {
+            const T* const r0 = (const T*)p.res + pix0 * p.ldres + 8 * (lg >> 1);
+#pragma unroll
+            for (int q = 0; q < NT_PIX / 2; ++q)
+#pragma unroll
+              for (int mi = 0; mi < NT_CO; ++mi) if (q >= q0 && q < q1) bxr[q][mi] = *reinterpret_cast<const u32x4*>(r0 + (long)q * p.Wo * p.ldres + mi * 16);
+          }
+        }
+      }
+    };
+
+    band_static_for<0, C::NSTG>([&](auto jc) {
+      constexpr int j = decltype(jc)::value;
+      constexpr int r_lo = (j - 1) * C::HPS, r_hi = j * C::HPS < C::HR ? j * C::HPS : C::HR;
+      constexpr bool counted = j >= 1 && r_hi > r_lo && r_hi * RPR <= C::HROWS;
+      if (j == 0 && epi_counted) band_wait<NSTORE>();
+      else if (counted && has_next) band_wait<counted ? r_hi - r_lo : 0>();
+      else band_wait<0>();
+      if (!(dbg & 16)) __builtin_amdgcn_s_barrier();
+
+      const unsigned char* const wl = smem + 2 * HB + wsel * WB + a_base;
+      const unsigned char* const hj = hb + j * C::RS * (IWp * 64);
+      if constexpr (WREG) {
+        if (c == 0) {
+#pragma unroll
+          for (int t = 0; t < C::TPS; ++t)
+#pragma unroll
+            for (int mi = 0; mi < NT_CO; ++mi) wreg[t][mi] = *reinterpret_cast<const u32x4*>(wl + t * (BN * 64) + mi * 1024);
+        }
+      }
+      if constexpr (BXQA > 0 && j == C::NSTG - 1) { if (ch_half == nhalf - 1) bx_issue(true, BXRA, 0, BXQA); }
+      u32x4 af[2][NT_CO], bf[2][NT_PIX];
+      if constexpr (DBG) if (dbg & 32) {
+#pragma unroll
+        for (int i = 0; i < 2; ++i)
+#pragma unroll
+          for (int q = 0; q < 4; ++q) { if (q < NT_CO) af[i][q] = u32x4{0x3f803f80u, (unsigned)tid, 0x3f803f80u, 0x3f803f80u}; bf[i][q] = u32x4{0x3f803f80u, 0x3f803f80u, (unsigned)lane, 0x3f803f80u}; }
+      }
+      auto load = [&](int set, int t) {
+        if (dbg & 32) return;
+#pragma unroll
+        for (int mi = 0; mi < NT_CO; ++mi) {
+          if constexpr (WREG) af[set][mi] = wreg[t][mi];
+          else af[set][mi] = *reinterpret_cast<const u32x4*>(wl + t * (BN * 64) + mi * 1024);
+        }
+#pragma unroll
+        for (int ni = 0; ni < NT_PIX; ++ni)
+          bf[set][ni] = *reinterpret_cast<const u32x4*>(hj + b_k[t % K] + ((t / K + (ni >> 1)) * IWp + (ni & 1) * 16) * 64);
+      };
+      auto dma_slot = [&](int sl) {
+        if (sl < C::WRS) {
+          if (dbg & 2) return;
+          if (j + 1 < C::NSTG) w_dma(sl, j + 1, ch_half, wsel ^ 1);
+          else if (has_next) w_dma(sl, 0, nh, wsel ^ 1);
+        } else if (sl < C::WRS + C::HPS) {
+          if (dbg & 1) return;
+          if (has_next && (C::NSTG == 1 || j < C::NSTG - 1)) halo_dma(j * C::HPS + sl - C::WRS, nsoff, hsel ^ 1);
+        }
+      };
+      load(0, 0);
+#pragma unroll
+      for (int kw = 0; kw < C::TPS; ++kw) {
+        if constexpr ((VAR & 1) != 0) {
+#pragma unroll
+          for (int sl = kw * C::SPT; sl < (kw + 1) * C::SPT; ++sl) dma_slot(sl);
+        }
+        if (kw + 1 < C::TPS) load((kw + 1) & 1, kw + 1);
+        if constexpr ((VAR & 1) == 0) {
+#pragma unroll
+          for (int sl = kw * C::SPT; sl < (kw + 1) * C::SPT; ++sl) dma_slot(sl);
+        }
+        if (!(dbg & 4)) {
+#pragma unroll
+          for (int mi = 0; mi < NT_CO; ++mi)
+#pragma unroll
+            for (int ni = 0; ni < NT_PIX; ++ni) Mma<T>::run(acc[mi][ni], af[kw & 1][mi], bf[kw & 1][ni]);
+        }
+        if constexpr ((VAR & 4) != 0) {
+#pragma unroll
+          for (int g = 0; g < NT_CO + NT_PIX; ++g) {
+            __builtin_amdgcn_sched_group_barrier(0x100, 1, 0);
+            __builtin_amdgcn_sched_group_barrier(0x008, (NT_CO * NT_PIX) / (NT_CO + NT_PIX), 0);
+          }
+        }
+      }
+      if constexpr (!C::WRES) wsel ^= 1;
+    });
+
+    epi_counted = false;
+    if (ch_half == nhalf - 1) {
+      const int oimg = KD > 1 ? cb * p.Do + cz : cb;
+      const int grp = oimg < p.bpg ? 0 : oimg / p.bpg;
+      if constexpr (BX) {
+#pragma unroll
+        for (int mi = 0; mi < NT_CO; ++mi)
+#pragma unroll
+          for (int r = 0; r < 4; ++r) { s1[mi][r] = 0.f; s2[mi][r] = 0.f; }
+      }
+      if (!BX && p.bias) {
+#pragma unroll
+        for (int mi = 0; mi < NT_CO; ++mi)
+#pragma unroll
+          for (int ni = 0; ni < NT_PIX; ++ni)
+#pragma unroll
+            for (int r = 0; r < 4; ++r) acc[mi][ni][r] += bv[mi][r];
+      }
+      if (!BX && p.act == 1) {
+#pragma unroll
+        for (int mi = 0; mi < NT_CO; ++mi)
+#pragma unroll
+          for (int ni = 0; ni < NT_PIX; ++ni)
+#pragma unroll
+            for (int r = 0; r < 4; ++r) acc[mi][ni][r] = fmaxf(acc[mi][ni][r], 0.f);
+      } else if (!BX && p.act == 2) {
+#pragma unroll
+        for (int mi = 0; mi < NT_CO; ++mi)
+#pragma unroll
+          for (int ni = 0; ni < NT_PIX; ++ni)
+#pragma unroll
+            for (int r = 0; r < 4; ++r) acc[mi][ni][r] = 1.f / (1.f + __expf(-acc[mi][ni][r]));
+      }
+      T* const yb = (T*)p.y + (long)oimg * p.Ho * p.Wo * p.ldy;
+      const T* const rb = (const T*)p.res + (long)oimg * p.Ho * p.Wo * p.ldres;
+      const bool interior = coh0 + C::TH <= p.Ho && cow0 + C::TW <= p.Wo && BN <= p.Cout;
+      if (interior) {
+        const long pix0 = (long)(coh0 + RPW * wave) * p.Wo + cow0 + (lg & 1) * 16 + l15;
+        T* const d0 = yb + pix0 * p.ldy + 8 * (lg >> 1);
+        const T* const r0 = rb + pix0 * p.ldres + 8 * (lg >> 1);
+        if constexpr (BX) {
+          if constexpr (BXQA < NT_PIX / 2) bx_issue(true, false, BXQA, NT_PIX / 2);
+          if constexpr (BXR && !BXRA) bx_issue(false, true, 0, NT_PIX / 2);
+        }
+        if constexpr (BX) {
+#pragma unroll
+          for (int q = 0; q < NT_PIX / 2; ++q)
+#pragma unroll
+            for (int mi = 0; mi < NT_CO; ++mi) asm volatile("" : "+v"(bxu[q][mi]));
+        }
+#pragma unroll
+        for (int q = 0; q < NT_PIX / 2; ++q) {
+          T* dst = d0 + (long)q * p.Wo * p.ldy;
+          const T* rsrc = r0 + (long)q * p.Wo * p.ldres;
+          u32x4 ov[NT_CO];
+#pragma unroll
+          for (int mi = 0; mi < NT_CO; ++mi) {
+            const f32x4 v0 = acc[mi][2 * q], v1 = acc[mi][2 * q + 1];
+            if constexpr (BX) {
+              const u32x4 ub = bxu[q][mi];
+              const u32x2 ua = __builtin_amdgcn_permlane16_swap(ub[0], ub[2], false, false);
+              const u32x2 uc = __builtin_amdgcn_permlane16_swap(ub[1], ub[3], false, false);
+              const unsigned ua0 = ua[0], ua1 = ua[1], uc0 = uc[0], uc1 = uc[1];
+              float f0[4], f1[4];
+#pragma unroll
+              for (int r = 0; r < 4; ++r) { f0[r] = v0[r]; f1[r] = v1[r]; }
+              if constexpr (BXR) {
+                const u32x4 rb4 = bxr[q][mi];
+                const u32x2 ra = __builtin_amdgcn_permlane16_swap(rb4[0], rb4[2], false, false);
+                const u32x2 rc = __builtin_amdgcn_permlane16_swap(rb4[1], rb4[3], false, false);
+                const unsigned ra0 = ra[0], ra1 = ra[1], rc0 = rc[0], rc1 = rc[1];
+                f0[0] += bflo(ra0); f0[1] += bfhi(ra0); f0[2] += bflo(rc0); f0[3] += bfhi(rc0);
+                f1[0] += bflo(ra1); f1[1] += bfhi(ra1); f1[2] += bflo(rc1); f1[3] += bfhi(rc1);
+              }
+              const unsigned p00 = pack2bf(f0[0], f0[1]), p01 = pack2bf(f0[2], f0[3]);
+              const unsigned p10 = pack2bf(f1[0], f1[1]), p11 = pack2bf(f1[2], f1[3]);
+              const float g0[4] = {bflo(p00), bfhi(p00), bflo(p01), bfhi(p01)}, g1[4] = {bflo(p10), bfhi(p10), bflo(p11), bfhi(p11)};
+              const float u0[4] = {bflo(ua0), bfhi(ua0), bflo(uc0), bfhi(uc0)}, u1[4] = {bflo(ua1), bfhi(ua1), bflo(uc1), bfhi(uc1)};
+              const f32x4 sc = *reinterpret_cast<const f32x4*>(bxs + mi * 16 + 4 * lg), sh = *reinterpret_cast<const f32x4*>(bxs + BN + mi * 16 + 4 * lg);
+#pragma unroll
+              for (int r = 0; r < 4; ++r) {
+                const float scr = sc[r], shr = sh[r];
+                const float gm0 = fmaf(u0[r], scr, shr) > 0.f ? g0[r] : 0.f;
+                const float gm1 = fmaf(u1[r], scr, shr) > 0.f ? g1[r] : 0.f;
+                s1[mi][r] = fmaf(gm1, u1[r], fmaf(gm0, u0[r], s1[mi][r]));
+                s2[mi][r] += gm0 + gm1;
+              }
+              const u32x2 e0 = __builtin_amdgcn_permlane16_swap(p00, p10, false, false);
+              const u32x2 e1 = __builtin_amdgcn_permlane16_swap(p01, p11, false, false);
+              ov[mi] = u32x4{e0[0], e1[0], e0[1], e1[1]};
+              continue;
+            }
+            const u32x2 o0 = u32x2{pack2bf(v0[0], v0[1]), pack2bf(v0[2], v0[3])};
+            const u32x2 o1 = u32x2{pack2bf(v1[0], v1[1]), pack2bf(v1[2], v1[3])};
+            if (p.stats) {
+              const f32x4 w0 = f32x4{bflo(o0[0]), bfhi(o0[0]), bflo(o0[1]), bfhi(o0[1])};
+              const f32x4 w1 = f32x4{bflo(o1[0]), bfhi(o1[0]), bflo(o1[1]), bfhi(o1[1])};
+#pragma unroll
+              for (int r = 0; r < 4; ++r) {
+                s1[mi][r] += w0[r] + w1[r];
+                s2[mi][r] = fmaf(w1[r], w1[r], fmaf(w0[r], w0[r], s2[mi][r]));
+              }
+            }
+            u32x4 o;
+            if (p.res) {
+              float f[8];
+#pragma unroll
+              for (int r = 0; r < 4; ++r) {
+                const float a0 = v0[r], a1 = v1[r];
+                const u32x2 e = __builtin_amdgcn_permlane16_swap(__float_as_uint(a0), __float_as_uint(a1), false, false);
+                const unsigned e0 = e[0], e1 = e[1];
+                f[r] = __uint_as_float(e0); f[4 + r] = __uint_as_float(e1);
+              }
+              const u32x4 old = *reinterpret_cast<const u32x4*>(rsrc + mi * 16);
+#pragma unroll
+              for (int e = 0; e < 4; ++e) o[e] = pack2bf(f[2 * e] + bflo(old[e]), f[2 * e + 1] + bfhi(old[e]));
+            } else {
+              const u32x2 e0 = __builtin_amdgcn_permlane16_swap(o0[0], o1[0], false, false);
+              const u32x2 e1 = __builtin_amdgcn_permlane16_swap(o0[1], o1[1], false, false);
+              o = u32x4{e0[0], e1[0], e0[1], e1[1]};
+            }
+            ov[mi] = o;
+          }
+          if (!(dbg & 8)) {
+#pragma unroll
+            for (int mi = 0; mi < NT_CO; ++mi) *reinterpret_cast<u32x4*>(dst + mi * 16) = ov[mi];
+          }
+        }
+        epi_counted = !(dbg & 8) && (BX || !p.res);
+      } else {
+#pragma unroll
+        for (int ni = 0; ni < NT_PIX; ++ni) {
+          const int oh = coh0 + RPW * wave + (ni >> 1), ow = cow0 + (ni & 1) * 16 + l15;
+          const bool valid = oh < p.Ho && ow < p.Wo;
+          T* dst = yb + ((long)oh * p.Wo + ow) * p.ldy;
+          const T* rsrc = rb + ((long)oh * p.Wo + ow) * p.ldres;
+#pragma unroll
+          for (int mi = 0; mi < NT_CO; ++mi) {
+            const int co = mi * 16 + 4 * lg;
+            float v[4];
+#pragma unroll
+            for (int r = 0; r < 4; ++r) v[r] = acc[mi][ni][r];
+            if (valid && co + 3 < p.Cout) {
+              if (BX ? BXR : p.res != nullptr) {
+                const u32x2 old = *reinterpret_cast<const u32x2*>(rsrc + co);
+                v[0] += bflo(old[0]); v[1] += bfhi(old[0]); v[2] += bflo(old[1]); v[3] += bfhi(old[1]);
+              }
+              const u32x2 o = u32x2{pack2bf(v[0], v[1]), pack2bf(v[2], v[3])};
+              *reinterpret_cast<u32x2*>(dst + co) = o;
+              v[0] = bflo(o[0]); v[1] = bfhi(o[0]); v[2] = bflo(o[1]); v[3] = bfhi(o[1]);
+            } else if (valid && co < p.Cout) {
+#pragma unroll
+              for (int r = 0; r < 4; ++r) {
+                if (co + r < p.Cout) {
+                  if (BX ? BXR : p.res != nullptr) v[r] += Elem<T>::ld(rsrc + co + r);
+                  Elem<T>::st(dst + co + r, v[r]); v[r] = Elem<T>::rnd(v[r]);
+                }
+                else v[r] = 0.f;
+              }
+            } else {
+#pragma unroll
+              for (int r = 0; r < 4; ++r) v[r] = 0.f;
+            }
+            if constexpr (BX) {
+#pragma unroll
+              for (int r = 0; r < 4; ++r) acc[mi][ni][r] = v[r];
+            } else if (p.stats) {
+#pragma unroll
+              for (int r = 0; r < 4; ++r) { s1[mi][r] += v[r]; s2[mi][r] = fmaf(v[r], v[r], s2[mi][r]); }
+            }
+          }
+        }
+        if constexpr (BX) {
+#pragma unroll
+          for (int ni = 0; ni < NT_PIX; ++ni) {
+            const int oh = min(coh0 + RPW * wave + (ni >> 1), p.Ho - 1), ow = min(cow0 + (ni & 1) * 16 + l15, p.Wo - 1);
+            const T* const usrc = (const T*)pbx.bx + ((long)oimg * p.Ho * p.Wo + (long)oh * p.Wo + ow) * pbx.ldbx;
+#pragma unroll
+            for (int mi = 0; mi < NT_CO; ++mi) {
+              const int co = mi * 16 + 4 * lg;
+              const u32x2 uu = *reinterpret_cast<const u32x2*>(usrc + min(co, p.Cout - 4));
+              const unsigned uu0 = uu[0], uu1 = uu[1];
+              const float uf[4] = {bflo(uu0), bfhi(uu0), bflo(uu1), bfhi(uu1)};
+#pragma unroll
+              for (int r = 0; r < 4; ++r) {
+                const float g = acc[mi][ni][r];
+                const float gm = fmaf(uf[r], bxs[co + r], bxs[BN + co + r]) > 0.f ? g : 0.f;
+                s1[mi][r] = fmaf(gm, uf[r], s1[mi][r]); s2[mi][r] += gm;
+              }
+            }
+          }
+        }
+      }
+      if constexpr (BX) bx_fold();
+      if (p.stats) {
+        const int nimg = KD > 1 ? nb * p.Do + nz : nb;
+        const int ngrp = nimg < p.bpg ? 0 : nimg / p.bpg;
+        if (!has_next || ngrp != grp) {
+          flush_stats(grp); epi_counted = false;
+          if constexpr (BX) { if (has_next) bx_scale(ngrp); }
+        }
+      }
+    }
+    cb = nb; coh0 = noh0; cow0 = now0; ch_half = nh; ct = nt; cz = nz;
+  }
diff --git a/pmt_learning_for_semantic_segmentation_and_disparity_amd/csrc/conv_fwd.hip b/pmt_learning_for_semantic_segmentation_and_disparity_amd/csrc/conv_fwd.hip
--- a/pmt_learning_for_semantic_segmentation_and_disparity_amd/csrc/conv_fwd.hip
+++ b/pmt_learning_for_semantic_segmentation_and_disparity_amd/csrc/conv_fwd.hip
@@ -535,8 +535,10 @@
 
 bool band_common_ok(const ConvCall& c) {
   const ConvGeom& g = c.g;
-  return !c.ps && !c.bx && c.omul == 1 && c.dtype == SDHIP_BF16 && g.stride == 1 && g.dil == 1 && !c.in_scale &&
-         !((c.accumulate || c.addend) && c.stats) && !(c.accumulate && c.addend) &&
+  const bool bx_ok = !c.bx || (c.bx_mode == 0 && c.flat() && c.stats && !c.accumulate && !c.bias && c.act == 0 && c.Cout % 4 == 0 &&
+                               c.ldbx % 8 == 0 && ((uintptr_t)c.bx & 15) == 0 && !sdhip_diag().conv_no_band_bx);
+  return !c.ps && bx_ok && c.omul == 1 && c.dtype == SDHIP_BF16 && g.stride == 1 && g.dil == 1 && !c.in_scale &&
+         !((c.accumulate || c.addend) && c.stats && !c.bx) && !(c.accumulate && c.addend) &&
          (!c.addend || (c.ldadd % 8 == 0 && ((uintptr_t)c.addend & 15) == 0)) && c.Cin % 8 == 0 &&
          c.ldx % 8 == 0 && ((uintptr_t)c.x & 15) == 0 && c.ldy % 8 == 0 && ((uintptr_t)c.y & 15) == 0 &&
          (long)g.B * g.D * g.H * g.W * c.ldx * 2 < (long)kBandOob && band_ok(sdhip_cdiv(g.Ho, 16) * sdhip_cdiv(g.Wo, 32) * g.B * g.Do) &&
@@ -560,6 +562,14 @@
   const bool band5 = g.kh == 5 && g.kw == 5 && (c.Cin <= 32 || c.Cin == 64);
   const bool band3 = g.kh == 3 && g.kw == 3 && c.Cin <= 32 && !sdhip_diag().conv_no_band3;
   if (!((band5 || band3) && c.flat() && d.Mpad <= 64 && d.Mpad >= 32 && band_common_ok(c))) return kNotTaken;
+  if (c.bx && !band_bx_form_ok(g.kh, d.Mpad, c.addend != nullptr)) return kNotTaken;
+  if (c.bx) {
+    BandBxArgs f{};
+    static_cast<BandArgs&>(f) = band_args(c, d);
+    f.pad_d = 0;
+    f.bx = c.bx; f.bsc = c.bsc; f.bsh = c.bsh; f.ldbx = c.ldbx;
+    return band5 ? launch_band_bx<5>(f, c.stream) : launch_band_bx<3>(f, c.stream);
+  }
   BandArgs f = band_args(c, d);
   f.pad_d = 0;
   return band5 ? launch_band<5>(f, c.stream) : launch_band<3>(f, c.stream);
@@ -567,7 +577,7 @@
 
 int path_band3d(const ConvCall& c, const ConvPlan& d) {
   const ConvGeom& g = c.g;
-  if (!(g.kh == 3 && g.kw == 3 && g.kd == 3 && g.sd == 1 && c.Cin <= 32 && d.Mpad == 32 && band_common_ok(c) && !sdhip_diag().conv_no_band3))
+  if (!(g.kh == 3 && g.kw == 3 && g.kd == 3 && g.sd == 1 && c.Cin <= 32 && d.Mpad == 32 && !c.bx && band_common_ok(c) && !sdhip_diag().conv_no_band3))
     return kNotTaken;
   BandArgs f = band_args(c, d);
   return launch_band<3, 3>(f, c.stream);
diff --git a/pmt_learning_for_semantic_segmentation_and_disparity_amd/csrc/runtime.hip b/pmt_learning_for_semantic_segmentation_and_disparity_amd/csrc/runtime.hip
--- a/pmt_learning_for_semantic_segmentation_and_disparity_amd/csrc/runtime.hip
+++ b/pmt_learning_for_semantic_segmentation_and_disparity_amd/csrc/runtime.hip
@@ -31,6 +31,7 @@
   g_diag.conv_no_gemm = env_set("SDHIP_CONV_NO_GEMM");
   g_diag.conv_no_band = env_set("SDHIP_CONV_NO_BAND");
   g_diag.conv_no_band3 = env_set("SDHIP_CONV_NO_BAND3");
+  g_diag.conv_no_band_bx = env_set("SDHIP_CONV_NO_BAND_BX");
   g_diag.conv_no_point = env_set("SDHIP_CONV_NO_POINT");
   g_diag.conv_no_grow = env_set("SDHIP_CONV_NO_GROW");
   g_diag.conv_no_mid = env_set("SDHIP_CONV_NO_MID");
diff --git a/pmt_learning_for_semantic_segmentation_and_disparity_amd/csrc/sdhip_common.h b/pmt_learning_for_semantic_segmentation_and_disparity_amd/csrc/sdhip_common.h
--- a/pmt_learning_for_semantic_segmentation_and_disparity_amd/csrc/sdhip_common.h
+++ b/pmt_learning_for_semantic_segmentation_and_disparity_amd/csrc/sdhip_common.h
@@ -28,7 +28,7 @@
 #define SDHIP_LAUNCH_CHECK() SDHIP_LAUNCH_CHECK_AS(__func__)
 
 struct SdhipDiag {
-  bool conv_generic, conv_big, conv_no_thin, conv_no_gemm, conv_no_band, conv_no_band3, wgrad_generic, wgrad_no_pack, wgrad_force_pack, wgrad_no_half, thin_wgrad_reg, corr_no_tiled, wgrad_no_half32, wgrad_split2d, wgrad_no_gemm, conv_no_point, conv_no_grow, conv_no_mid;
+  bool conv_generic, conv_big, conv_no_thin, conv_no_gemm, conv_no_band, conv_no_band3, conv_no_band_bx, wgrad_generic, wgrad_no_pack, wgrad_force_pack, wgrad_no_half, thin_wgrad_reg, corr_no_tiled, wgrad_no_half32, wgrad_split2d, wgrad_no_gemm, conv_no_point, conv_no_grow, conv_no_mid;
   int tune_s2_small;
   int tune_big, tune_split, tune_thin_blocks, tune_fused_blocks, tune_gemm_dbg, tune_band_dbg;
   int tune_mid_min_map, tune_mid_max_map, tune_mid_max_wg;
diff --git a/pmt_learning_for_semantic_segmentation_and_disparity_amd/ops.py b/pmt_learning_for_semantic_segmentation_and_disparity_amd/ops.py
--- a/pmt_learning_for_semantic_segmentation_and_disparity_amd/ops.py
+++ b/pmt_learning_for_semantic_segmentation_and_disparity_amd/ops.py
@@ -710,6 +710,7 @@
 
 
 BN_SLOT_MAX_BYTES = _lib.TUNE_BN_SLOT_MAX_MB << 20
+BAND_BX_FORMS = tuple(f for f in _lib.TUNE_BAND_BX_FORMS.split(",") if f)
 
 
 class BNSlot:
@@ -719,6 +720,27 @@
         self.u = self.scale = self.shift = self.sums = None
         self.ldu = self.groups = self.C = 0
         self.gptr = 0
+
+
+def _band_bx_form(spec, Bimg, H, W, Cin, Cout, has_addend, ldg, bn_slot):
+    env = os.environ
+    if env.get("SDHIP_CONV_NO_BAND_BX") or env.get("SDHIP_CONV_NO_BAND") or env.get("SDHIP_CONV_GENERIC"):
+        return None
+    if spec.stride != 1 or spec.dil != 1 or spec.kh != spec.kw or Cout % 8 or Cin % 8 or ldg % 8:
+        return None
+    if bn_slot is None or bn_slot.u is None or bn_slot.ldu % 8 or bn_slot.u.data_ptr() % 16:
+        return None
+    if Bimg * spec.Ho * spec.Wo * ldg * 2 >= 0x7fffff00:
+        return None
+    mpad = (Cin + 15) & ~15
+    tiles = -(-H // 16) * -(-W // 32) * Bimg
+    if not (32 <= mpad <= 64 and 192 <= tiles < 65536):
+        return None
+    if spec.kh == 5 and (Cout <= 32 or Cout == 64) and not (mpad > 32 and has_addend):
+        return '5x5'
+    if spec.kh == 3 and Cout <= 32 and not env.get("SDHIP_CONV_NO_BAND3"):
+        return '3x3'
+    return None
 
 
 def _conv_backward(ctx_spec, xv, ldx, weight, g, ldg, in_scale, in_shift, in_relu, groups, need_x, need_w, bias=None, acc_into=None,
@@ -732,9 +754,10 @@
     if need_x:
         wd = packed_weight(weight, spec.kind, 'dgrad', xv.dtype)
         fused_bn = False
+        band_form = _band_bx_form(spec, Bimg, H, W, Cin, Cout, acc_into is not None or addend is not None, ldg, bn_slot) if spec.kd == 1 and spec.D == 1 else None
         if (bn_slot is not None and bn_slot.u is not None and bn_slot.C == Cin and xv.dtype == torch.bfloat16 and spec.stride == 1
                 and spec.sd == 1 and spec.kd == 1 and spec.D == 1 and tuple(bn_slot.u.shape) == (Bimg, Cin, H, W)
-                and spec.kh * spec.kw <= 9 and Bimg * H * W * Cin * 2 <= BN_SLOT_MAX_BYTES):
+                and (band_form in BAND_BX_FORMS or (spec.kh * spec.kw <= 9 and Bimg * H * W * Cin * 2 <= BN_SLOT_MAX_BYTES))):
             other = acc_into if acc_into is not None else addend
             gpost, ldgp = alloc_nhwc(Bimg, Cin, H, W, xv.dtype, xv.device)
             sums = _zeros((NREP, bn_slot.groups, 2, Cin), torch.float64, xv.device)[0]
```

New measurement: 439.0 stereo-pairs/s (median of 6 runs). 1.0% higher.
